# Komputerowe-Projektowanie-Lekow/pmarlo

Measured on AMD Instinct MI355X. Metric: frames/sec featurize->TICA->k-means->T-matrix, 1Mx64 synth; ITS rel-err, higher is better.
Workload: dtype f64; 1 GPU; synthetic 1000000 frames x 64 f32 features per GPU (AR(1) latents), TICA->10, k=500 (10 Lloyd iterations), lag=10, row-normalised T; frames_per_gpu=1000000, features=64, tica_dim=10, k=500, lag=10, kmeans_iters=10, parallelism=shards1

## Files before the change

### include/msmhip.h

```cpp
#ifndef MSMHIP_H
#define MSMHIP_H

#include <stddef.h>
#include <stdint.h>

#ifdef __cplusplus
extern "C" {
#endif

typedef struct msm_ctx msm_ctx;
typedef struct msm_event msm_event;
typedef struct msm_graph msm_graph;

typedef enum {
    MSM_OK = 0,
    MSM_ERR_INVALID = 1,
    MSM_ERR_HIP = 2,
    MSM_ERR_NOMEM = 3,
    MSM_ERR_UNSUPPORTED = 4,
    MSM_ERR_NOCONV = 5
} msm_status;

typedef enum { MSM_F32 = 0, MSM_F64 = 1 } msm_dtype;


msm_status msm_ctx_create(int device, void* hip_stream, msm_ctx** out);
void msm_ctx_destroy(msm_ctx* ctx);
const char* msm_last_error(const msm_ctx* ctx);
msm_status msm_device_info(msm_ctx* ctx, char* arch, size_t arch_len,
                           int* n_cu, size_t* total_mem);
const char* msm_version(void);

msm_status msm_malloc(msm_ctx* ctx, size_t bytes, void** d_out);
msm_status msm_free(msm_ctx* ctx, void* d_ptr);
msm_status msm_memcpy_h2d(msm_ctx* ctx, void* d_dst, const void* h_src, size_t bytes);
msm_status msm_memcpy_d2h(msm_ctx* ctx, void* h_dst, const void* d_src, size_t bytes);
msm_status msm_memcpy_d2d(msm_ctx* ctx, void* d_dst, const void* d_src, size_t bytes);
msm_status msm_memset(msm_ctx* ctx, void* d_dst, int value, size_t bytes);
msm_status msm_sync(msm_ctx* ctx);

msm_status msm_event_create(msm_ctx* ctx, msm_event** out);
void msm_event_destroy(msm_event* ev);
msm_status msm_event_record(msm_ctx* ctx, msm_event* ev);
msm_status msm_event_elapsed_ms(msm_event* start, msm_event* stop, float* h_ms);

msm_status msm_graph_begin(msm_ctx* ctx);
msm_status msm_graph_end(msm_ctx* ctx, msm_graph** out);
msm_status msm_graph_launch(msm_ctx* ctx, msm_graph* g);
void msm_graph_destroy(msm_graph* g);


msm_status msm_featurize_distances(msm_ctx* ctx, const float* d_xyz, int64_t n, int A,
                                   const int32_t* d_pairs, int P, float* d_out, int64_t ld, int col_off);
msm_status msm_featurize_contacts(msm_ctx* ctx, const float* d_xyz, int64_t n, int A,
                                  const int32_t* d_pairs, int P, float rcut, float* d_out,
                                  int64_t ld, int col_off);
msm_status msm_featurize_rg(msm_ctx* ctx, const float* d_xyz, int64_t n, int A, float* d_out,
                            int64_t ld, int col_off);
msm_status msm_featurize_angles(msm_ctx* ctx, const float* d_xyz, int64_t n, int A,
                                const int32_t* d_triplets, int Tn, float* d_out, int64_t ld, int col_off);
msm_status msm_featurize_dihedrals(msm_ctx* ctx, const float* d_xyz, int64_t n, int A,
                                   const int32_t* d_quads, int Q, int mode, float* d_out, int64_t ld,
                                   int col_off);

msm_status msm_featurize_sasa(msm_ctx* ctx, const float* d_xyz, int64_t n, int A, const float* d_radii,
                              const float* d_points, int P, float* d_out);
msm_status msm_hbond_presence(msm_ctx* ctx, const float* d_xyz, int64_t n, int A, const int32_t* d_triplets,
                              int Tn, float dist_cutoff, float angle_cutoff, uint64_t* d_counts);
msm_status msm_dssp(msm_ctx* ctx, const float* d_xyz, int64_t n, int A, const int32_t* d_backbone,
                    const int32_t* d_chain, const uint8_t* d_proline, int R, uint8_t* d_codes);


msm_status msm_count_transitions(msm_ctx* ctx, const int32_t* d_labels, int64_t n,
                                 const int64_t* h_seg_start, const int64_t* h_seg_stop,
                                 int n_seg, int lag, int stride, int k,
                                 int64_t* d_counts, int64_t* d_pairs);

msm_status msm_count_transitions_weighted(msm_ctx* ctx, const int32_t* d_labels,
                                          const double* d_weights, int64_t n,
                                          const int64_t* h_seg_start, const int64_t* h_seg_stop,
                                          int n_seg, int lag, int stride, int k,
                                          double* d_counts, int64_t* d_pairs);

msm_status msm_count_transitions_lagscan(msm_ctx* ctx, const int32_t* d_labels, int64_t n,
                                         const int64_t* h_seg_start, const int64_t* h_seg_stop,
                                         int n_seg, const int32_t* h_lags, int n_lag, int k,
                                         int64_t* d_counts, int64_t* d_pairs);

msm_status msm_state_counts(msm_ctx* ctx, const int32_t* d_labels, int64_t n, int k,
                            int64_t* d_visits);

msm_status msm_run_lengths(msm_ctx* ctx, const int32_t* d_labels, int64_t n, int k, int64_t* d_stats,
                           int32_t* d_run_state, int64_t* d_run_len, int64_t capacity, int64_t* d_n_runs);


msm_status msm_column_moments_partial(msm_ctx* ctx, const void* d_x, msm_dtype dtype, int64_t n, int F,
                                      int64_t ld, const double* d_shift, double* d_sums,
                                      double* d_shift_out);
msm_status msm_moments_finalize(msm_ctx* ctx, const double* d_sums, const double* d_shift, int F,
                                int ddof, double* d_mean, double* d_std, double* d_count);
msm_status msm_column_minmax(msm_ctx* ctx, const void* d_x, msm_dtype dtype, int64_t n, int F, int64_t ld,
                             double* d_min, double* d_max, int64_t* d_counts);
msm_status msm_column_moments(msm_ctx* ctx, const void* d_x, msm_dtype dtype, int64_t n, int F,
                              int64_t ld, int ddof, double* d_mean, double* d_std, double* d_count);

msm_status msm_standardise_params(msm_ctx* ctx, const double* d_sums, const double* d_shift, int F,
                                  double n_rows, int with_std, double* d_mean, double* d_scale,
                                  double* d_inv_scale);

msm_status msm_lagged_moments(msm_ctx* ctx, const void* d_x, msm_dtype dtype, int64_t n, int F, int64_t ld,
                              const int64_t* h_seg_start, const int64_t* h_seg_stop, int n_seg, int lag,
                              const double* d_shift, int assume_finite, double* d_moments);

msm_status msm_lagged_moments_reversible(msm_ctx* ctx, const void* d_x, msm_dtype dtype, int64_t n, int F, int64_t ld,
                                         const int64_t* h_seg_start, const int64_t* h_seg_stop, int n_seg, int lag,
                                         const double* d_shift, int assume_finite, double* d_moments);

msm_status msm_lagged_moments_onesided(msm_ctx* ctx, const void* d_x, msm_dtype dtype, int64_t n, int F,
                                       int64_t ld, const int64_t* h_seg_start, const int64_t* h_seg_stop,
                                       int n_seg, int lag, const double* d_shift, int assume_finite,
                                       double* d_moments);

msm_status msm_onesided_tica_eigenvalues(msm_ctx* ctx, const double* d_moments, int F, double clip,
                                         double* d_eigvals);

msm_status msm_moments_from_lagged(msm_ctx* ctx, const void* d_x, msm_dtype dtype, int64_t n, int F, int64_t ld,
                                   const int64_t* h_seg_start, const int64_t* h_seg_stop, int n_seg, int lag,
                                   const double* d_shift, const double* d_moments, double* d_sums);

msm_status msm_tica_solve(msm_ctx* ctx, const double* d_moments, const double* d_scale, int F,
                          double epsilon, int kinetic_map, double* d_eigvals, double* d_coeffs,
                          double* d_mean, int* d_rank);

msm_status msm_project(msm_ctx* ctx, const void* d_x, msm_dtype dtype, int64_t n, int F, int64_t ld,
                       const double* d_mu, const double* d_inv_sigma, const double* d_mean2,
                       const double* d_w, int d, int64_t ldw, double* d_y, int64_t ldy, double* d_absmax);

msm_status msm_project_finite(msm_ctx* ctx, const void* d_x, msm_dtype dtype, int64_t n, int F, int64_t ld,
                              const double* d_mu, const double* d_inv_sigma, const double* d_mean2,
                              const double* d_w, int d, int64_t ldw, double* d_y, int64_t ldy, double* d_absmax);

msm_status msm_eigh(msm_ctx* ctx, const double* d_a, int n, double* d_w, double* d_v, int* d_sweeps);


msm_status msm_kmeans_assign(msm_ctx* ctx, const void* d_x, msm_dtype dtype, int64_t n, int d,
                             int64_t ld, const double* d_centers, int k,
                             const double* d_mean, const double* d_std,
                             int32_t* d_labels, double* d_mindist);

msm_status msm_kmeans_fit(msm_ctx* ctx, const void* d_x, msm_dtype dtype, int64_t n, int d, int64_t ld,
                          const double* d_mean, const double* d_std, int k, uint64_t seed,
                          int init_centers, int max_iter, double tol2, double* d_centers,
                          double* d_state);
msm_status msm_kmeans_init_plusplus(msm_ctx* ctx, const void* d_x, msm_dtype dtype, int64_t n, int d, int64_t ld,
                                    const double* d_mean, const double* d_std, int k, uint64_t seed, double n_total,
                                    double* d_centers, const double* d_state, int64_t* d_picked);
msm_status msm_kmeans_fit_begin(msm_ctx* ctx, const void* d_x, msm_dtype dtype, int64_t n, int d,
                                int64_t ld, const double* d_mean, const double* d_std, int k,
                                uint64_t seed, int init_centers, double n_total, double tol2,
                                double* d_centers, double* d_state, int absmax_ready);
msm_status msm_kmeans_accumulate(msm_ctx* ctx, const void* d_x, msm_dtype dtype, int64_t n, int d,
                                 int64_t ld, const double* d_centers, int k, const double* d_mean,
                                 const double* d_std, const double* d_state, int64_t* d_sums,
                                 int64_t* d_counts);
msm_status msm_kmeans_update(msm_ctx* ctx, int64_t* d_sums, int64_t* d_counts, int k, int d,
                             double* d_centers, double* d_state, int clear);

msm_status msm_kmeans_image_bytes(int64_t n, int d, size_t* out_bytes);
msm_status msm_kmeans_pack(msm_ctx* ctx, const void* d_x, msm_dtype dtype, int64_t n, int d, int64_t ld,
                           const double* d_mean, const double* d_std, void* d_image);
msm_status msm_kmeans_assign_packed(msm_ctx* ctx, const void* d_x, msm_dtype dtype, int64_t n, int d,
                                    int64_t ld, const double* d_centers, int k, const double* d_mean,
                                    const double* d_std, const void* d_image, int32_t* d_labels,
                                    double* d_mindist);
msm_status msm_kmeans_accumulate_packed(msm_ctx* ctx, const void* d_x, msm_dtype dtype, int64_t n, int d,
                                        int64_t ld, const double* d_centers, int k, const double* d_mean,
                                        const double* d_std, const void* d_image, const double* d_state,
                                        int64_t* d_sums, int64_t* d_counts);
msm_status msm_kmeans_accumulate_delta(msm_ctx* ctx, const void* d_x, msm_dtype dtype, int64_t n, int d,
                                       int64_t ld, const double* d_centers, int k, const double* d_mean,
                                       const double* d_std, const void* d_image, const double* d_state,
                                       int32_t* d_prev_labels, int64_t* d_sums, int64_t* d_counts);
msm_status msm_kmeans_lloyd_pass(msm_ctx* ctx, const void* d_x, msm_dtype dtype, int64_t n, int d, int64_t ld,
                                 double* d_centers, int k, const double* d_mean, const double* d_std,
                                 const void* d_image, double* d_state, int32_t* d_prev_labels, int64_t* d_sums,
                                 int64_t* d_counts);
msm_status msm_kmeans_filter_scanned(msm_ctx* ctx, uint64_t* h_out, int reset);
msm_status msm_mfma_bf16_probe(msm_ctx* ctx, const uint16_t* h_a, const uint16_t* h_b, const float* h_c,
                               float* h_d, int n_tiles);

msm_status msm_sum_f64(msm_ctx* ctx, const double* d_v, int64_t n, double* d_out);


msm_status msm_transition_matrix(msm_ctx* ctx, const void* d_counts, int counts_are_f64, int k, int mode,
                                 double alpha, double epsilon, double* d_T, int32_t* d_active,
                                 int32_t* d_inv_map, int32_t* d_n_active, double* d_rowsum,
                                 double* d_diag_mass);

msm_status msm_embed_full(msm_ctx* ctx, const double* d_T_active, const double* d_pi_active,
                          const int32_t* d_inv_map, int k, double* d_T_full, double* d_pi_full);

size_t msm_spectrum_workspace_bytes(int n_max, int p, int batch);
msm_status msm_spectrum(msm_ctx* ctx, const double* d_T, int64_t t_stride, int ld, const int32_t* d_n,
                        int n_max, int batch, int p, int n_iter, int init, uint64_t seed, int n_watch,
                        void* d_workspace, double* d_ritz, double* d_pi, int64_t pi_stride,
                        double* d_change, int32_t* d_status, int n_its, const double* d_lags,
                        double* d_its_eig, double* d_its_ts, double freeze_tol, double* d_vecs, int n_vecs);
msm_status msm_matrix_power(msm_ctx* ctx, const double* d_T, int64_t t_stride, int ld, const int32_t* d_n, int n_max,
                            int batch, int n_squarings, double* d_scratch, double* d_out);
msm_status msm_spectrum_powered(msm_ctx* ctx, const double* d_T, const double* d_T_power, int64_t t_stride, int ld,
                                const int32_t* d_n, int n_max, int batch, int p, int n_iter, int init, uint64_t seed,
                                int n_watch, void* d_workspace, double* d_ritz, double* d_pi, int64_t pi_stride,
                                double* d_change, int32_t* d_status, int n_its, const double* d_lags,
                                double* d_its_eig, double* d_its_ts, double freeze_tol, double* d_vecs, int n_vecs);

msm_status msm_reversible_mle(msm_ctx* ctx, const double* d_counts, int n, int ld, double maxerr, int maxiter,
                              double* d_T, int ldt, double* d_pi, int* h_iterations, double* h_err);

msm_status msm_sample_transition_matrices(msm_ctx* ctx, const void* d_counts, int counts_are_f64, int k,
                                          const int32_t* d_active, const int32_t* d_n_active, double alpha,
                                          uint64_t seed, int first_sample, int n_samples, double* d_T,
                                          int64_t t_stride, int ld);

msm_status msm_philox4x32(msm_ctx* ctx, uint64_t key, const uint32_t counter[4], uint32_t* d_out);

msm_status msm_gemm_f64(msm_ctx* ctx, int m, int n, int k, const double* d_A, int64_t lda,
                        const double* d_B, int64_t ldb, double* d_C, int64_t ldc);
msm_status msm_ck_test(msm_ctx* ctx, const double* d_T1, int64_t ld1, const double* d_Tk,
                       int64_t tk_stride, int64_t ldk, int n, const int32_t* h_factors, int n_factors,
                       const double* d_rowcounts, int64_t rc_stride, double* d_mse, double* d_noise);

msm_status msm_diff_norms(msm_ctx* ctx, const double* d_P, int64_t ldp, const double* d_Q, int64_t ldq, int n, int m,
                          double* d_out);

msm_status msm_order_statistics(msm_ctx* ctx, const double* d_x, int64_t stride, int64_t n, const int64_t* h_ranks,
                                int n_ranks, double* h_out);

msm_status msm_weighted_stats(msm_ctx* ctx, const double* d_x, int64_t stride, int64_t n,
                              const double* d_w, double* d_out6);
msm_status msm_hist2d(msm_ctx* ctx, const double* d_x, int64_t sx, const double* d_y, int64_t sy,
                      int64_t n, const double* d_w, double w_absmax, const double* d_xedges, int nx,
                      const double* d_yedges, int ny, double* d_hist);
msm_status msm_smooth_sparse_bins(msm_ctx* ctx, const double* d_hist, int nx, int ny,
                                  double min_count, double* d_out, int32_t* d_n_smoothed);
msm_status msm_scale_to_total(msm_ctx* ctx, double* d_v, int n, double total);
msm_status msm_fes_finalize(msm_ctx* ctx, const double* d_hist, int n_cells, double kT,
                            double* d_F, int32_t* d_status);
msm_status msm_kde2d(msm_ctx* ctx, const double* d_x, int64_t sx, const double* d_y, int64_t sy,
                     int64_t n, const double* d_w, double w_scale, const double* d_xcenters, int nx,
                     const double* d_ycenters, int ny, double bw_x, double bw_y, int periodic, double* d_density);

msm_status msm_clip_or_wrap(msm_ctx* ctx, const double* d_x, int64_t stride, int64_t n, double lo, double hi, int mode,
                            double* d_out);

msm_status msm_gather_f64(msm_ctx* ctx, const double* d_table, int m, const int32_t* d_idx, int64_t n, double* d_out);

msm_status msm_solve_f64(msm_ctx* ctx, int n, int nrhs, double* d_A, int64_t lda, double* d_B,
                         int64_t ldb, int32_t* d_info);
msm_status msm_reactive_flux(msm_ctx* ctx, const double* d_T, int64_t ldt, const double* d_pi,
                             const int32_t* d_role, int n, double* d_qplus, double* d_qminus,
                             double* d_gross, double* d_net, double* d_totals, int32_t* d_info);
msm_status msm_lump_macro(msm_ctx* ctx, const double* d_T, int64_t ldt, const double* d_pi,
                          const int32_t* d_macro, int n, int n_macro, double* d_T_macro,
                          double* d_pi_macro);
msm_status msm_macro_mfpt(msm_ctx* ctx, const double* d_T, int64_t ldt, int n, double* d_mfpt,
                          int32_t* d_info);

msm_status msm_silhouette(msm_ctx* ctx, const double* d_x, int64_t n, int d, int64_t ld,
                          const int64_t* h_offsets, int k, double* d_samples, double* d_score);

msm_status msm_grid_cells(msm_ctx* ctx, const void* d_x, msm_dtype dtype, int64_t n, int F, int64_t ld,
                          const double* d_edges, int bins, int32_t* d_flat);
msm_status msm_first_occurrence(msm_ctx* ctx, const int32_t* d_flat, int64_t n, int n_cells,
                                int64_t* d_first);
msm_status msm_relabel(msm_ctx* ctx, const int32_t* d_flat, int64_t n, const int32_t* d_map, int n_cells,
                       int32_t* d_labels);


typedef struct msm_comm msm_comm;
#define MSM_COMM_ID_BYTES 128
msm_status msm_comm_unique_id(void* out_id, size_t bytes);
msm_status msm_comm_init(msm_ctx* ctx, int rank, int world, const void* id, size_t id_bytes, msm_comm** out);
void msm_comm_destroy(msm_comm* comm);
msm_status msm_comm_info(msm_comm* comm, int* rank, int* world, uint64_t* n_collectives);
msm_status msm_allreduce_i64(msm_comm* comm, int64_t* d_buf, size_t count);
msm_status msm_allreduce_i64_from(msm_comm* comm, const int64_t* d_src, int64_t* d_dst, size_t count);
msm_status msm_allreduce_f64(msm_comm* comm, double* d_buf, size_t count);
msm_status msm_allreduce_min_f64(msm_comm* comm, double* d_buf, size_t count);
msm_status msm_allreduce_max_f64(msm_comm* comm, double* d_buf, size_t count);
msm_status msm_broadcast(msm_comm* comm, void* d_buf, size_t bytes, int root);
msm_status msm_rcp_f64(msm_ctx* ctx, const double* d_src, size_t n, double* d_dst);

#ifdef __cplusplus
}
#endif
#endif
```

### pmarlo_amd/_lib.py

```python

from __future__ import annotations

import ctypes as C
from pathlib import Path

__all__ = ["lib", "load", "LIB_PATH", "check", "MsmError", "DECLARED_SYMBOLS"]

LIB_PATH = Path(__file__).resolve().parent / "csrc" / "libmsmhip.so"

MSM_OK, MSM_ERR_INVALID, MSM_ERR_HIP, MSM_ERR_NOMEM, MSM_ERR_UNSUPPORTED, MSM_ERR_NOCONV = range(6)
MSM_F32, MSM_F64 = 0, 1


class MsmError(RuntimeError):
    """A HIP-side failure reported through the C ABI."""


_vp = C.c_void_p
_i32 = C.c_int
_i64 = C.c_int64
_sz = C.c_size_t
_f64 = C.c_double
_pp = C.POINTER(C.c_void_p)

_PROTOTYPES: dict[str, tuple] = {
    "msm_version": (C.c_char_p, []),
    "msm_ctx_create": (_i32, [_i32, _vp, _pp]),
    "msm_ctx_destroy": (None, [_vp]),
    "msm_last_error": (C.c_char_p, [_vp]),
    "msm_device_info": (_i32, [_vp, C.c_char_p, _sz, C.POINTER(_i32), C.POINTER(_sz)]),
    "msm_malloc": (_i32, [_vp, _sz, _pp]),
    "msm_free": (_i32, [_vp, _vp]),
    "msm_memcpy_h2d": (_i32, [_vp, _vp, _vp, _sz]),
    "msm_memcpy_d2h": (_i32, [_vp, _vp, _vp, _sz]),
    "msm_memcpy_d2d": (_i32, [_vp, _vp, _vp, _sz]),
    "msm_memset": (_i32, [_vp, _vp, _i32, _sz]),
    "msm_sync": (_i32, [_vp]),
    "msm_event_create": (_i32, [_vp, _pp]),
    "msm_event_destroy": (None, [_vp]),
    "msm_event_record": (_i32, [_vp, _vp]),
    "msm_event_elapsed_ms": (_i32, [_vp, _vp, C.POINTER(C.c_float)]),
    "msm_graph_begin": (_i32, [_vp]),
    "msm_graph_end": (_i32, [_vp, _pp]),
    "msm_graph_launch": (_i32, [_vp, _vp]),
    "msm_graph_destroy": (None, [_vp]),
    "msm_featurize_distances": (_i32, [_vp, _vp, _i64, _i32, _vp, _i32, _vp, _i64, _i32]),
    "msm_featurize_contacts": (_i32, [_vp, _vp, _i64, _i32, _vp, _i32, C.c_float, _vp, _i64, _i32]),
    "msm_featurize_rg": (_i32, [_vp, _vp, _i64, _i32, _vp, _i64, _i32]),
    "msm_featurize_angles": (_i32, [_vp, _vp, _i64, _i32, _vp, _i32, _vp, _i64, _i32]),
    "msm_featurize_dihedrals": (_i32, [_vp, _vp, _i64, _i32, _vp, _i32, _i32, _vp, _i64, _i32]),
    "msm_featurize_sasa": (_i32, [_vp, _vp, _i64, _i32, _vp, _vp, _i32, _vp]),
    "msm_hbond_presence": (_i32, [_vp, _vp, _i64, _i32, _vp, _i32, C.c_float, C.c_float, _vp]),
    "msm_dssp": (_i32, [_vp, _vp, _i64, _i32, _vp, _vp, _vp, _i32, _vp]),
    "msm_count_transitions": (_i32, [_vp, _vp, _i64, _vp, _vp, _i32, _i32, _i32, _i32, _vp, _vp]),
    "msm_count_transitions_weighted": (
        _i32, [_vp, _vp, _vp, _i64, _vp, _vp, _i32, _i32, _i32, _i32, _vp, _vp]),
    "msm_count_transitions_lagscan": (_i32, [_vp, _vp, _i64, _vp, _vp, _i32, _vp, _i32, _i32, _vp, _vp]),
    "msm_state_counts": (_i32, [_vp, _vp, _i64, _i32, _vp]),
    "msm_column_moments_partial": (_i32, [_vp, _vp, _i32, _i64, _i32, _i64, _vp, _vp, _vp]),
    "msm_moments_finalize": (_i32, [_vp, _vp, _vp, _i32, _i32, _vp, _vp, _vp]),
    "msm_column_moments": (_i32, [_vp, _vp, _i32, _i64, _i32, _i64, _i32, _vp, _vp, _vp]),
    "msm_column_minmax": (_i32, [_vp, _vp, _i32, _i64, _i32, _i64, _vp, _vp, _vp]),
    "msm_standardise_params": (_i32, [_vp, _vp, _vp, _i32, _f64, _i32, _vp, _vp, _vp]),
    "msm_lagged_moments": (_i32, [_vp, _vp, _i32, _i64, _i32, _i64, _vp, _vp, _i32, _i32, _vp, _i32, _vp]),
    "msm_tica_solve": (_i32, [_vp, _vp, _vp, _i32, _f64, _i32, _vp, _vp, _vp, _vp]),
    "msm_lagged_moments_reversible": (_i32, [_vp, _vp, _i32, _i64, _i32, _i64, _vp, _vp, _i32, _i32, _vp, _i32, _vp]),
    "msm_lagged_moments_onesided": (_i32, [_vp, _vp, _i32, _i64, _i32, _i64, _vp, _vp, _i32, _i32, _vp, _i32, _vp]),
    "msm_onesided_tica_eigenvalues": (_i32, [_vp, _vp, _i32, _f64, _vp]),
    "msm_moments_from_lagged": (_i32, [_vp, _vp, _i32, _i64, _i32, _i64, _vp, _vp, _i32, _i32, _vp, _vp, _vp]),
    "msm_project": (_i32, [_vp, _vp, _i32, _i64, _i32, _i64, _vp, _vp, _vp, _vp, _i32, _i64, _vp, _i64, _vp]),
    "msm_project_finite": (_i32, [_vp, _vp, _i32, _i64, _i32, _i64, _vp, _vp, _vp, _vp, _i32, _i64, _vp, _i64, _vp]),
    "msm_eigh": (_i32, [_vp, _vp, _i32, _vp, _vp, _vp]),
    "msm_kmeans_assign": (_i32, [_vp, _vp, _i32, _i64, _i32, _i64, _vp, _i32, _vp, _vp, _vp, _vp]),
    "msm_kmeans_fit": (_i32, [_vp, _vp, _i32, _i64, _i32, _i64, _vp, _vp, _i32, C.c_uint64, _i32, _i32, _f64, _vp, _vp]),
    "msm_kmeans_fit_begin": (
        _i32, [_vp, _vp, _i32, _i64, _i32, _i64, _vp, _vp, _i32, C.c_uint64, _i32, _f64, _f64, _vp, _vp, _i32]),
    "msm_kmeans_accumulate": (_i32, [_vp, _vp, _i32, _i64, _i32, _i64, _vp, _i32, _vp, _vp, _vp, _vp, _vp]),
    "msm_kmeans_update": (_i32, [_vp, _vp, _vp, _i32, _i32, _vp, _vp, _i32]),
    "msm_comm_unique_id": (_i32, [_vp, _sz]),
    "msm_comm_init": (_i32, [_vp, _i32, _i32, _vp, _sz, _pp]),
    "msm_comm_destroy": (None, [_vp]),
    "msm_comm_info": (_i32, [_vp, C.POINTER(_i32), C.POINTER(_i32), C.POINTER(C.c_uint64)]),
    "msm_allreduce_i64": (_i32, [_vp, _vp, _sz]),
    "msm_allreduce_i64_from": (_i32, [_vp, _vp, _vp, _sz]),
    "msm_allreduce_f64": (_i32, [_vp, _vp, _sz]),
    "msm_allreduce_min_f64": (_i32, [_vp, _vp, _sz]),
    "msm_allreduce_max_f64": (_i32, [_vp, _vp, _sz]),
    "msm_broadcast": (_i32, [_vp, _vp, _sz, _i32]),
    "msm_rcp_f64": (_i32, [_vp, _vp, _sz, _vp]),
    "msm_kmeans_image_bytes": (_i32, [_i64, _i32, C.POINTER(_sz)]),
    "msm_kmeans_pack": (_i32, [_vp, _vp, _i32, _i64, _i32, _i64, _vp, _vp, _vp]),
    "msm_kmeans_assign_packed": (_i32, [_vp, _vp, _i32, _i64, _i32, _i64, _vp, _i32, _vp, _vp, _vp, _vp, _vp]),
    "msm_kmeans_accumulate_packed": (_i32, [_vp, _vp, _i32, _i64, _i32, _i64, _vp, _i32, _vp, _vp, _vp, _vp, _vp, _vp]),
    "msm_kmeans_lloyd_pass": (_i32, [_vp, _vp, _i32, _i64, _i32, _i64, _vp, _i32, _vp, _vp, _vp, _vp, _vp, _vp, _vp]),
    "msm_kmeans_accumulate_delta": (_i32, [_vp, _vp, _i32, _i64, _i32, _i64, _vp, _i32, _vp, _vp, _vp, _vp, _vp, _vp,
                                           _vp]),
    "msm_kmeans_filter_scanned": (_i32, [_vp, C.POINTER(C.c_uint64), _i32]),
    "msm_kmeans_init_plusplus": (_i32, [_vp, _vp, _i32, _i64, _i32, _i64, _vp, _vp, _i32, C.c_uint64, _f64, _vp, _vp, _vp]),
    "msm_mfma_bf16_probe": (_i32, [_vp, _vp, _vp, _vp, _vp, _i32]),
    "msm_run_lengths": (_i32, [_vp, _vp, _i64, _i32, _vp, _vp, _vp, _i64, _vp]),
    "msm_sum_f64": (_i32, [_vp, _vp, _i64, _vp]),
    "msm_transition_matrix": (_i32, [_vp, _vp, _i32, _i32, _i32, _f64, _f64, _vp, _vp, _vp, _vp, _vp, _vp]),
    "msm_embed_full": (_i32, [_vp, _vp, _vp, _vp, _i32, _vp, _vp]),
    "msm_spectrum_workspace_bytes": (_sz, [_i32, _i32, _i32]),
    "msm_spectrum": (_i32, [_vp, _vp, _i64, _i32, _vp, _i32, _i32, _i32, _i32, _i32, C.c_uint64, _i32, _vp, _vp, _vp,
                            _i64, _vp, _vp, _i32, _vp, _vp, _vp, _f64, _vp, _i32]),
    "msm_matrix_power": (_i32, [_vp, _vp, _i64, _i32, _vp, _i32, _i32, _i32, _vp, _vp]),
    "msm_spectrum_powered": (_i32, [_vp, _vp, _vp, _i64, _i32, _vp, _i32, _i32, _i32, _i32, _i32, C.c_uint64, _i32, _vp, _vp,
                                    _vp, _i64, _vp, _vp, _i32, _vp, _vp, _vp, _f64, _vp, _i32]),
    "msm_sample_transition_matrices": (_i32, [_vp, _vp, _i32, _i32, _vp, _vp, _f64, C.c_uint64, _i32, _i32, _vp, _i64,
                                              _i32]),
    "msm_reversible_mle": (_i32, [_vp, _vp, _i32, _i32, _f64, _i32, _vp, _i32, _vp, _vp, _vp]),
    "msm_philox4x32": (_i32, [_vp, C.c_uint64, _vp, _vp]),
    "msm_gemm_f64": (_i32, [_vp, _i32, _i32, _i32, _vp, _i64, _vp, _i64, _vp, _i64]),
    "msm_diff_norms": (_i32, [_vp, _vp, _i64, _vp, _i64, _i32, _i32, _vp]),
    "msm_gather_f64": (_i32, [_vp, _vp, _i32, _vp, _i64, _vp]),
    "msm_clip_or_wrap": (_i32, [_vp, _vp, _i64, _i64, _f64, _f64, _i32, _vp]),
    "msm_order_statistics": (_i32, [_vp, _vp, _i64, _i64, _vp, _i32, _vp]),
    "msm_weighted_stats": (_i32, [_vp, _vp, _i64, _i64, _vp, _vp]),
    "msm_hist2d": (_i32, [_vp, _vp, _i64, _vp, _i64, _i64, _vp, _f64, _vp, _i32, _vp, _i32, _vp]),
    "msm_smooth_sparse_bins": (_i32, [_vp, _vp, _i32, _i32, _f64, _vp, _vp]),
    "msm_scale_to_total": (_i32, [_vp, _vp, _i32, _f64]),
    "msm_fes_finalize": (_i32, [_vp, _vp, _i32, _f64, _vp, _vp]),
    "msm_kde2d": (_i32, [_vp, _vp, _i64, _vp, _i64, _i64, _vp, _f64, _vp, _i32, _vp, _i32, _f64, _f64, _i32, _vp]),
    "msm_solve_f64": (_i32, [_vp, _i32, _i32, _vp, _i64, _vp, _i64, _vp]),
    "msm_reactive_flux": (_i32, [_vp, _vp, _i64, _vp, _vp, _i32, _vp, _vp, _vp, _vp, _vp, _vp]),
    "msm_lump_macro": (_i32, [_vp, _vp, _i64, _vp, _vp, _i32, _i32, _vp, _vp]),
    "msm_macro_mfpt": (_i32, [_vp, _vp, _i64, _i32, _vp, _vp]),
    "msm_silhouette": (_i32, [_vp, _vp, _i64, _i32, _i64, _vp, _i32, _vp, _vp]),
    "msm_grid_cells": (_i32, [_vp, _vp, _i32, _i64, _i32, _i64, _vp, _i32, _vp]),
    "msm_first_occurrence": (_i32, [_vp, _vp, _i64, _i32, _vp]),
    "msm_relabel": (_i32, [_vp, _vp, _i64, _vp, _i32, _vp]),
    "msm_ck_test": (_i32, [_vp, _vp, _i64, _vp, _i64, _i64, _i32, _vp, _i32, _vp, _i64, _vp, _vp]),
}

DECLARED_SYMBOLS = tuple(_PROTOTYPES)

_lib = None


def load() -> C.CDLL:
    global _lib
    if _lib is not None:
        return _lib
    if not LIB_PATH.exists():
        raise ImportError(
            f"{LIB_PATH} is missing: build it with `python -m pmarlo_amd.csrc.build` "
            "(hipcc, gfx950).  pmarlo_amd has no CPU fallback."
        )
    handle = C.CDLL(str(LIB_PATH))
    for name, (res, args) in _PROTOTYPES.items():
        fn = getattr(handle, name)
        fn.restype = res
        fn.argtypes = args
    _lib = handle
    return handle


class _LazyLib:
    def __getattr__(self, name):
        return getattr(load(), name)


lib = _LazyLib()

_EXC = {
    MSM_ERR_INVALID: ValueError,
    MSM_ERR_HIP: MsmError,
    MSM_ERR_NOMEM: MemoryError,
    MSM_ERR_UNSUPPORTED: NotImplementedError,
    MSM_ERR_NOCONV: MsmError,
}


def check(status: int, ctx_handle=None) -> None:
    if status == MSM_OK:
        return
    msg = ""
    if ctx_handle:
        raw = load().msm_last_error(ctx_handle)
        msg = raw.decode("utf-8", "replace") if raw else ""
    exc = _EXC.get(status, MsmError)
    raise exc(msg or f"libmsmhip call failed with status {status}")
```

### pmarlo_amd/csrc/kmeans.hip

```cpp
#include "common.h"

#include <algorithm>
#include <cstdlib>

namespace {

constexpr int kThreads = 256;

template <typename T>
__device__ __forceinline__ double load_as_f64(const T* p) { return (double)(*p); }

struct FitState {
    double scale;
    double inv_scale;
    double absmax;
    double shift2;
    double tol2;
    double done;
    double n_iter;
    double inertia;
};

__device__ __forceinline__ long long to_fixed(double v, double scale) { return __double2ll_rn(v * scale); }

// ... 448 lines not shown
            const int kt16 = (kt + 15) & ~15;
            if (!single_tile) {
                __syncthreads();
                stage_tile(k0, kt, kt16);
                KSTAMP(5);
            }
            const int n_tiles = kt16 / 16;
            for (int jt = 0; jt < n_tiles; jt += 2) {
                const int jb = min(jt + 1, n_tiles - 1);
                v4f64 acca[NF], accb[NF];
#pragma unroll
                for (int u = 0; u < NF; ++u) { acca[u] = (v4f64){0.0, 0.0, 0.0, 0.0}; accb[u] = acca[u]; }
                if constexpr (KS <= 4) {
#pragma unroll
                    for (int s = 0; s < KS; ++s) {
                        const double afa = cs[jt * TS + s * 64 + lane];
#pragma unroll
                        for (int u = 0; u < NF; ++u)
                            acca[u] = __builtin_amdgcn_mfma_f64_16x16x4f64(afa, zb[u][s], acca[u], 0, 0, 0);
                    }
#pragma unroll
                    for (int s = 0; s < KS; ++s) {
                        const double afb = cs[jb * TS + s * 64 + lane];
#pragma unroll
                        for (int u = 0; u < NF; ++u)
                            accb[u] = __builtin_amdgcn_mfma_f64_16x16x4f64(afb, zb[u][s], accb[u], 0, 0, 0);
                    }
                } else {
                    double fa = cs[jt * TS + lane], fb = cs[jb * TS + lane];
#pragma unroll
                    for (int s = 0; s < KS; ++s) {
                        double na = fa, nb = fb;
                        if (s + 1 < KS) {
                            na = cs[jt * TS + (s + 1) * 64 + lane];
                            nb = cs[jb * TS + (s + 1) * 64 + lane];
                        }
#pragma unroll
                        for (int u = 0; u < NF; ++u) {
                            acca[u] = __builtin_amdgcn_mfma_f64_16x16x4f64(fa, zb[u][s], acca[u], 0, 0, 0);
                            accb[u] = __builtin_amdgcn_mfma_f64_16x16x4f64(fb, zb[u][s], accb[u], 0, 0, 0);
                        }
                        fa = na;
                        fb = nb;
                    }
                }
                if constexpr (!fold) {
#pragma unroll
                    for (int r = 0; r < 4; ++r) {
                        const double ha = chalf[jt * 16 + g + 4 * r], hb = chalf[jb * 16 + g + 4 * r];
#pragma unroll
                        for (int u = 0; u < NF; ++u) { acca[u][r] -= ha; accb[u][r] -= hb; }
                    }
                }
                __builtin_amdgcn_sched_barrier(0);
                if constexpr (KS > 4) asm volatile("s_nop 15\n\ts_nop 3" ::: "memory");
                double ma[NF], mb[NF];
#pragma unroll
                for (int u = 0; u < NF; ++u) ma[u] = max_f64(max_f64(acca[u][0], acca[u][1]), max_f64(acca[u][2], acca[u][3]));
                asm volatile("s_nop 7" ::: "memory");
                __builtin_amdgcn_sched_barrier(0);
#pragma unroll
                for (int u = 0; u < NF; ++u) {
                    mb[u] = max_f64(max_f64(accb[u][0], accb[u][1]), max_f64(accb[u][2], accb[u][3]));
                    const double m = max_f64(ma[u], mb[u]);
                    const bool better = m > best[u];
                    best[u] = better ? m : best[u];
                    const int code = kGlobalRecovery ? (((k0 >> 4) + jt) << 1) | (jb == jt ? 1 : 0) : jt;
                    bpair[u] = better ? code : bpair[u];
                }
            }
            KSTAMP(2);
            if constexpr (!kGlobalRecovery) {
#pragma unroll
            for (int u = 0; u < NF; ++u) {
                double M = best[u];
                M = fmax(M, __shfl_xor(M, 16, 64));
                M = fmax(M, __shfl_xor(M, 32, 64));
                const unsigned long long tied = __ballot(best[u] == M) >> j16;
                unsigned pending = (unsigned)(tied & 1) | (unsigned)((tied >> 15) & 2) | (unsigned)((tied >> 30) & 4) |
                                   (unsigned)((tied >> 45) & 8);
                int found = 0x7fffffff;
                while (__any(pending != 0)) {
                    const int gs = pending ? __builtin_ctz(pending) : 0;
                    const int pj = __shfl(bpair[u], j16 + 16 * gs, 64);
                    const int ta = pj, tb = min(pj + 1, n_tiles - 1);
                    const int crow = gs + 4 * g;
                    const double* ca = cs + ta * TS + crow;
                    const double* cb = cs + tb * TS + crow;
                    double da = 0.0, db = 0.0;
#pragma unroll
                    for (int s = 0; s < KS; ++s)
#pragma unroll
                        for (int gp = 0; gp < 4; ++gp) {
                            const double zv = __shfl(zb[u][s], j16 + 16 * gp, 64);
                            da = fma(ca[s * 64 + gp * 16], zv, da);
                            db = fma(cb[s * 64 + gp * 16], zv, db);
                        }
                    if constexpr (!fold) {
                        da -= chalf[ta * 16 + crow];
                        db -= chalf[tb * 16 + crow];
                    }
                    int cand = 0x7fffffff;
                    if (pending) {
                        if (db == M) cand = k0 + tb * 16 + crow;
                        if (da == M) cand = k0 + ta * 16 + crow;
                    }
                    cand = min(cand, __shfl_xor(cand, 16, 64));
                    cand = min(cand, __shfl_xor(cand, 32, 64));
                    found = min(found, cand);
                    pending &= pending - 1;
                }
                if (found < k) { bm[u] = M; bidx[u] = found; }
            }
            }
        }
        if constexpr (kGlobalRecovery) {
#pragma unroll
            for (int u = 0; u < NF; ++u) {
                double M = best[u];
                M = fmax(M, __shfl_xor(M, 16, 64));
                M = fmax(M, __shfl_xor(M, 32, 64));
                const unsigned long long tied = __ballot(best[u] == M) >> j16;
                unsigned pending = (unsigned)(tied & 1) | (unsigned)((tied >> 15) & 2) | (unsigned)((tied >> 30) & 4) |
                                   (unsigned)((tied >> 45) & 8);
                int found = 0x7fffffff;
                const T* row = x + (fok[u] ? fidx[u] : 0) * ld;
                while (__any(pending != 0)) {
                    const int gs = pending ? __builtin_ctz(pending) : 0;
                    const int pj = __shfl(bpair[u], j16 + 16 * gs, 64);
                    const int ta = pj >> 1, tb = ta + ((pj & 1) ? 0 : 1);
                    const int crow = gs + 4 * g;
                    const int ia = ta * 16 + crow, ib = tb * 16 + crow;
                    const double* ca = centers + (size_t)min(ia, k - 1) * d;
                    const double* cb = centers + (size_t)min(ib, k - 1) * d;
                    double da = 0.0, db = 0.0;
                    int f = 0;
                    for (; f + 8 <= d; f += 8) {
                        double v[8], va[8], vb[8];
#pragma unroll
                        for (int q = 0; q < 8; ++q) {
                            v[q] = load_as_f64(row + f + q);
                            va[q] = ca[f + q];
                            vb[q] = cb[f + q];
                        }
#pragma unroll
                        for (int q = 0; q < 8; ++q) {
                            double z = v[q];
                            if (mean) z = (z - mean[f + q]) / stdv[f + q];
                            da = fma(va[q], z, da);
                            db = fma(vb[q], z, db);
                        }
                    }
                    for (; f < d; ++f) {
                        double v = load_as_f64(row + f);
                        if (mean) v = (v - mean[f]) / stdv[f];
                        da = fma(ca[f], v, da);
                        db = fma(cb[f], v, db);
                    }
                    da -= chalf_g[min(ia, k - 1)];
                    db -= chalf_g[min(ib, k - 1)];
                    int cand = 0x7fffffff;
                    if (pending) {
                        if (ib < k && db == M) cand = ib;
                        if (ia < k && da == M) cand = ia;
                    }
                    cand = min(cand, __shfl_xor(cand, 16, 64));
                    cand = min(cand, __shfl_xor(cand, 32, 64));
                    found = min(found, cand);
                    pending &= pending - 1;
                }
                if (found < k) { bm[u] = M; bidx[u] = found; }
            }
        }
        KSTAMP(3);
#pragma unroll
        for (int u = 0; u < NF; ++u) {
            if (!fok[u]) continue;
            if constexpr (ACCUM) {
                const int old = labels ? labels[fidx[u]] : -1;
                if (!labels || old != bidx[u]) {
                    unsigned long long* base = lds_acc ? lsum : sums;
                    unsigned long long* srow = base + (size_t)bidx[u] * d;
#pragma unroll
                    for (int s = 0; s < KS; ++s) {
                        const int f = 4 * s + g;
                        if (f < d) {
                            const unsigned long long fx = (unsigned long long)to_fixed(zb[u][s], scale);
                            atomicAdd(&srow[f], fx);
                            if (old >= 0) atomicAdd(&base[(size_t)old * d + f], 0ull - fx);
                        }
                    }
                    if (g == 0) {
                        atomicAdd((lds_acc ? lcnt : counts) + bidx[u], 1ull);
                        if (old >= 0) atomicAdd((lds_acc ? lcnt : counts) + old, ~0ull);
                        if (labels) labels[fidx[u]] = bidx[u];
                    }
                }
            } else {
                if (g == 0) {
                    labels[fidx[u]] = bidx[u];
                    if (mindist) {
                        const T* row = x + fidx[u] * ld;
                        double zsq = 0.0;
                        for (int f = 0; f < d; ++f) {
                            double v = load_as_f64(row + f);
                            if (mean) v = (v - mean[f]) / stdv[f];
                            zsq = fma(v, v, zsq);
                        }
                        const double md = -2.0 * bm[u] + zsq;
                        mindist[fidx[u]] = md > 0.0 ? md : 0.0;
                    }
                }
            }
        }
        KSTAMP(4);
    }
    KSTAMP(7);
    if constexpr (ACCUM) {
        if (lds_acc) {
            __syncthreads();
            KSTAMP(5);
            for (int i = tid; i < k * d; i += kMT)
                if (lsum[i]) atomicAdd(&sums[i], lsum[i]);
            for (int i = tid; i < k; i += kMT)
                if (lcnt[i]) atomicAdd(&counts[i], lcnt[i]);
        }
    }
    KSTAMP(6);
    KSTAMP_FLUSH
}

template <typename T, int KS, bool ACCUM>
msm_status launch_mfma(msm_ctx* ctx, const T* x, int64_t n, int d, int64_t ld, const double* centers, int k,
                       const double* mean, const double* stdv, int32_t* labels, double* mindist, const FitState* st,
                       unsigned long long* sums, unsigned long long* counts) {
    constexpr int NF = KS <= 16 ? 2 : 1;
    constexpr int kMT = KS <= 4 ? kMTNarrow : kMTWide;
    constexpr int TS = KS * 64 + 1;
    const size_t acc_bytes = ACCUM ? (size_t)k * (d + 1) * sizeof(unsigned long long) : 0;
    const int lds_acc = ACCUM && acc_bytes <= 64 * 1024;
    const size_t tile_budget = 150 * 1024 - (lds_acc ? acc_bytes : 0);
    int tile_k = (int)(tile_budget / ((TS + 16) * sizeof(double))) * 16;
    const int k16 = (k + 15) & ~15;
    if (tile_k > k16) tile_k = k16;
    if (tile_k < 16) tile_k = 16;
    if (tile_k < k16 && tile_k >= 32) tile_k &= ~31;
    const size_t lds = (size_t)(tile_k / 16) * (TS + 16) * sizeof(double) + (lds_acc ? acc_bytes : 0);
    const int64_t n_units = (n + 16 * NF - 1) / (16 * NF);
    const int waves = kMT / 64;
    const int grid = (int)std::min<int64_t>((n_units + waves - 1) / waves, (int64_t)ctx->n_cu);
    const bool multi = k > tile_k;
    const bool foldm = (d & 3) != 0;
    auto kern = multi ? (foldm ? kmeans_mfma_kernel<T, KS, NF, kMT, ACCUM, true, true>
                               : kmeans_mfma_kernel<T, KS, NF, kMT, ACCUM, false, true>)
                      : (foldm ? kmeans_mfma_kernel<T, KS, NF, kMT, ACCUM, true, false>
                               : kmeans_mfma_kernel<T, KS, NF, kMT, ACCUM, false, false>);
    double* chalf_g = nullptr;
    double* tile_img = nullptr;
    if (multi) {
        const size_t n_tiles_all = (size_t)k16 / 16;
        const size_t img_doubles = (n_tiles_all * TS + 1) & ~(size_t)1;
        msm_status rs = msm_reserve_aux(ctx, (img_doubles + k16) * sizeof(double));
        if (rs != MSM_OK) return rs;
        tile_img = (double*)ctx->aux;
        chalf_g = tile_img + img_doubles;
        if (foldm)
            hipLaunchKernelGGL((pack_tiles_kernel<KS, true>), dim3((unsigned)n_tiles_all), dim3(64), 0, ctx->stream, centers,
                               k, d, tile_img, chalf_g);
        else
            hipLaunchKernelGGL((pack_tiles_kernel<KS, false>), dim3((unsigned)n_tiles_all), dim3(64), 0, ctx->stream, centers,
                               k, d, tile_img, chalf_g);
    } else if (KS > 8) {
        msm_status rs = msm_reserve_aux(ctx, (size_t)k * sizeof(double));
        if (rs != MSM_OK) return rs;
        chalf_g = (double*)ctx->aux;
        hipLaunchKernelGGL(chalf_kernel, dim3((k + 255) / 256), dim3(256), 0, ctx->stream, centers, k, d, chalf_g);
    }
    if (lds > 48 * 1024)
        MSM_HIP(ctx, hipFuncSetAttribute((const void*)kern, hipFuncAttributeMaxDynamicSharedMemorySize, (int)lds));
    hipLaunchKernelGGL(kern, dim3(grid), dim3(kMT), lds, ctx->stream, x, n, d, ld, centers, k, mean, stdv, tile_k,
                       labels, mindist, st, sums, counts, lds_acc, (const double*)chalf_g, (const double*)tile_img);
    MSM_CHECK_LAUNCH(ctx);
    return MSM_OK;
}

__global__ void mfma_bf16_probe_kernel(const uint16_t* __restrict__ A, const uint16_t* __restrict__ B,
                                       const float* __restrict__ C, float* __restrict__ D) {
    const int l = threadIdx.x, i = l & 15, q = l >> 4;
    A += (size_t)blockIdx.x * 512;
    B += (size_t)blockIdx.x * 512;
    C += (size_t)blockIdx.x * 256;
    D += (size_t)blockIdx.x * 256;
    v8bf a, b;
    for (int j = 0; j < 8; ++j) {
        a[j] = __builtin_bit_cast(__bf16, A[i * 32 + 8 * q + j]);
        b[j] = __builtin_bit_cast(__bf16, B[(8 * q + j) * 16 + i]);
    }
    v4f32 c;
    for (int r = 0; r < 4; ++r) c[r] = C[(4 * q + r) * 16 + i];
    c = __builtin_amdgcn_mfma_f32_16x16x32_bf16(a, b, c, 0, 0, 0);
    for (int r = 0; r < 4; ++r) D[(4 * q + r) * 16 + i] = c[r];
}

bool filter_enabled() {
    static const bool on = [] {
        const char* e = getenv("MSM_KMEANS_FILTER");
        return !(e && e[0] == '0');
    }();
    return on;
}

size_t filter_image_bytes(int64_t n, int d) { return (size_t)((n + 63) & ~(int64_t)63) * 16 * filter_rowq(filter_nm(d)); }

template <typename T>
msm_status launch_pack(msm_ctx* ctx, const T* x, int64_t n, int d, int64_t ld, const double* mean, const double* stdv,
                       uint4* image) {
    const unsigned grid = (unsigned)((n + 255) / 256);
    const int dense = ld == d && ((uintptr_t)x & 15) == 0;
#define MSM_PACK_CASE(D)                                                                                              \
    case D:                                                                                                           \
        hipLaunchKernelGGL((kmeans_pack_kernel<T, D>), dim3(grid), dim3(256), 0, ctx->stream, x, n, ld, mean, stdv, image, \
                           dense);                                                                                    \
        break
    switch (d) {
        MSM_PACK_CASE(1); MSM_PACK_CASE(2); MSM_PACK_CASE(3); MSM_PACK_CASE(4); MSM_PACK_CASE(5);
        MSM_PACK_CASE(6); MSM_PACK_CASE(7); MSM_PACK_CASE(8); MSM_PACK_CASE(9); MSM_PACK_CASE(10);
        default: return msm_fail(ctx, MSM_ERR_UNSUPPORTED, "k-means frame images need d <= %d (got %d)", kFilterMaxD, d);
    }
#undef MSM_PACK_CASE
    MSM_CHECK_LAUNCH(ctx);
    return MSM_OK;
}

msm_status filter_stats_buffer(msm_ctx* ctx, unsigned long long** out) {
    static_assert(sizeof(unsigned long long) == 8, "");
    if (!ctx->km_stats) {
        if (ctx->capturing) { *out = nullptr; return MSM_OK; }
        MSM_HIP(ctx, hipMalloc(&ctx->km_stats, 16));
        MSM_HIP(ctx, hipMemsetAsync(ctx->km_stats, 0, 16, ctx->stream));
    }
    *out = (unsigned long long*)ctx->km_stats;
    return MSM_OK;
}

template <typename T, int NM, bool ACCUM>
msm_status launch_filter_nm(msm_ctx* ctx, const T* x, int64_t n, int d, int64_t ld, const double* centers, int k,
                            const double* mean, const double* stdv, const uint4* image, int32_t* labels, double* mindist,
                            const FitState* st, unsigned long long* sums, unsigned long long* counts, double* upd_centers) {
    constexpr int NF = 4;
    const size_t lds = filter_lds_bytes(k, d, ACCUM);
    msm_status rs;
    const int64_t n_units = (n + 16 * NF - 1) / (16 * NF);
    constexpr int kWaves = filter_waves(NM);
    const int grid = (int)std::min<int64_t>((n_units + kWaves - 1) / kWaves, (int64_t)ctx->n_cu);
    unsigned long long* stats = nullptr;
    rs = filter_stats_buffer(ctx, &stats);
    if (rs != MSM_OK) return rs;
    auto kern = mean ? kmeans_filter_kernel<T, NM, NF, ACCUM, true> : kmeans_filter_kernel<T, NM, NF, ACCUM, false>;
    if (lds > 48 * 1024)
        MSM_HIP(ctx, hipFuncSetAttribute((const void*)kern, hipFuncAttributeMaxDynamicSharedMemorySize, (int)lds));
    hipLaunchKernelGGL(kern, dim3(grid), dim3(64 * kWaves), lds, ctx->stream, x, n, d, ld, k, mean, stdv, image, centers,
                       labels, mindist, st, sums, counts, stats, stats ? upd_centers : nullptr,
                       stats ? (unsigned int*)(stats + 1) : nullptr);
    MSM_CHECK_LAUNCH(ctx);
    return MSM_OK;
}

template <typename T, bool ACCUM>
msm_status launch_filter(msm_ctx* ctx, const T* x, int64_t n, int d, int64_t ld, const double* centers, int k,
                         const double* mean, const double* stdv, const uint4* image, int32_t* labels, double* mindist,
                         const FitState* st, unsigned long long* sums, unsigned long long* counts, double* upd_centers) {
    if (filter_nm(d) == 1)
        return launch_filter_nm<T, 1, ACCUM>(ctx, x, n, d, ld, centers, k, mean, stdv, image, labels, mindist, st, sums,
                                             counts, upd_centers);
    return launch_filter_nm<T, 2, ACCUM>(ctx, x, n, d, ld, centers, k, mean, stdv, image, labels, mindist, st, sums, counts,
                                         upd_centers);
}

bool filter_fits(int k, int d, bool accum) { return filter_enabled() && d <= kFilterMaxD && filter_lds_bytes(k, d, accum) != 0; }

template <typename T, bool ACCUM>
msm_status dispatch_mfma(msm_ctx* ctx, const T* x, int64_t n, int d, int64_t ld, const double* centers, int k,
                         const double* mean, const double* stdv, int32_t* labels, double* mindist, const FitState* st,
                         unsigned long long* sums, unsigned long long* counts, const void* image = nullptr,
                         double* upd_centers = nullptr, bool* folded = nullptr) {
    if (folded) *folded = false;
    if (filter_fits(k, d, ACCUM)) {
        if (!image) {
            msm_status rs = msm_reserve_km_image(ctx, filter_image_bytes(n, d));
            if (rs != MSM_OK) return rs;
            rs = launch_pack<T>(ctx, x, n, d, ld, mean, stdv, (uint4*)ctx->km_image);
            if (rs != MSM_OK) return rs;
            image = ctx->km_image;
        }
        if (upd_centers && !(ACCUM && (int64_t)k * d <= kUpdateWide && (ctx->km_stats || !ctx->capturing))) upd_centers = nullptr;
        if (folded) *folded = upd_centers != nullptr;
        return launch_filter<T, ACCUM>(ctx, x, n, d, ld, centers, k, mean, stdv, (const uint4*)image, labels, mindist, st,
                                       sums, counts, upd_centers);
    }
#define MSM_MFMA_CASE(KSV) \
    if (d <= 4 * KSV)      \
        return launch_mfma<T, KSV, ACCUM>(ctx, x, n, d, ld, centers, k, mean, stdv, labels, mindist, st, sums, counts)
    MSM_MFMA_CASE(1);
    MSM_MFMA_CASE(2);
    MSM_MFMA_CASE(3);
    MSM_MFMA_CASE(4);
    MSM_MFMA_CASE(6);
    MSM_MFMA_CASE(8);
    MSM_MFMA_CASE(12);
    MSM_MFMA_CASE(16);
    MSM_MFMA_CASE(24);
    MSM_MFMA_CASE(32);
    MSM_MFMA_CASE(48);
    MSM_MFMA_CASE(64);
#undef MSM_MFMA_CASE
    return msm_fail(ctx, MSM_ERR_UNSUPPORTED, "k-means: d=%d > 256 not supported", d);
}

}

extern "C" {

static msm_status kmeans_assign_impl(msm_ctx* ctx, const void* d_x, msm_dtype dtype, int64_t n, int d, int64_t ld,
                                     const double* d_centers, int k, const double* d_mean, const double* d_std,
                                     const void* d_image, int32_t* d_labels, double* d_mindist) {
    if (!ctx) return MSM_ERR_INVALID;
    MSM_REQUIRE(ctx, n >= 0 && d >= 1 && k >= 1, "msm_kmeans_assign: need n >= 0, d >= 1, k >= 1");
    MSM_REQUIRE(ctx, ld >= d, "msm_kmeans_assign: ld (%lld) < d (%d)", (long long)ld, d);
    MSM_REQUIRE(ctx, (d_mean == nullptr) == (d_std == nullptr),
                "msm_kmeans_assign: mean and std must both be given or both be NULL");
    MSM_REQUIRE(ctx, dtype == MSM_F32 || dtype == MSM_F64, "msm_kmeans_assign: bad dtype");
    if (n == 0) return MSM_OK;
    MSM_REQUIRE(ctx, d_x && d_centers && d_labels, "msm_kmeans_assign: NULL pointer");
    if (dtype == MSM_F32)
        return dispatch_mfma<float, false>(ctx, (const float*)d_x, n, d, ld, d_centers, k, d_mean, d_std, d_labels,
                                           d_mindist, nullptr, nullptr, nullptr, d_image);
    return dispatch_mfma<double, false>(ctx, (const double*)d_x, n, d, ld, d_centers, k, d_mean, d_std, d_labels,
                                        d_mindist, nullptr, nullptr, nullptr, d_image);
}

msm_status msm_kmeans_assign(msm_ctx* ctx, const void* d_x, msm_dtype dtype, int64_t n, int d, int64_t ld,
                             const double* d_centers, int k, const double* d_mean, const double* d_std,
                             int32_t* d_labels, double* d_mindist) {
    return kmeans_assign_impl(ctx, d_x, dtype, n, d, ld, d_centers, k, d_mean, d_std, nullptr, d_labels, d_mindist);
}

msm_status msm_kmeans_assign_packed(msm_ctx* ctx, const void* d_x, msm_dtype dtype, int64_t n, int d, int64_t ld,
                                    const double* d_centers, int k, const double* d_mean, const double* d_std,
                                    const void* d_image, int32_t* d_labels, double* d_mindist) {
    return kmeans_assign_impl(ctx, d_x, dtype, n, d, ld, d_centers, k, d_mean, d_std, d_image, d_labels, d_mindist);
}

msm_status msm_kmeans_image_bytes(int64_t n, int d, size_t* out_bytes) {
    if (!out_bytes || n < 0 || d < 1) return MSM_ERR_INVALID;
    *out_bytes = d <= kFilterMaxD ? filter_image_bytes(n, d) : 0;
    return MSM_OK;
}

msm_status msm_kmeans_pack(msm_ctx* ctx, const void* d_x, msm_dtype dtype, int64_t n, int d, int64_t ld,
                           const double* d_mean, const double* d_std, void* d_image) {
    if (!ctx) return MSM_ERR_INVALID;
    MSM_REQUIRE(ctx, n >= 0 && d >= 1 && d <= kFilterMaxD && ld >= d, "msm_kmeans_pack: need 1 <= d <= %d, ld >= d",
                kFilterMaxD);
    MSM_REQUIRE(ctx, (d_mean == nullptr) == (d_std == nullptr), "msm_kmeans_pack: mean/std must come together");
    MSM_REQUIRE(ctx, dtype == MSM_F32 || dtype == MSM_F64, "msm_kmeans_pack: bad dtype");
    if (n == 0) return MSM_OK;
    MSM_REQUIRE(ctx, d_x && d_image, "msm_kmeans_pack: NULL pointer");
    MSM_REQUIRE(ctx, ((uintptr_t)d_image & 15) == 0, "msm_kmeans_pack: the image must be 16-byte aligned");
    if (dtype == MSM_F32) return launch_pack<float>(ctx, (const float*)d_x, n, d, ld, d_mean, d_std, (uint4*)d_image);
    return launch_pack<double>(ctx, (const double*)d_x, n, d, ld, d_mean, d_std, (uint4*)d_image);
}

msm_status msm_kmeans_filter_scanned(msm_ctx* ctx, uint64_t* h_out, int reset) {
    if (!ctx || !h_out) return MSM_ERR_INVALID;
    *h_out = 0;
    if (!ctx->km_stats) return MSM_OK;
    MSM_HIP(ctx, hipStreamSynchronize(ctx->stream));
    MSM_HIP(ctx, hipMemcpy(h_out, ctx->km_stats, 8, hipMemcpyDeviceToHost));
    if (reset) MSM_HIP(ctx, hipMemset(ctx->km_stats, 0, 8));
    return MSM_OK;
}

msm_status msm_mfma_bf16_probe(msm_ctx* ctx, const uint16_t* h_a, const uint16_t* h_b, const float* h_c, float* h_d,
                               int n_tiles) {
    if (!ctx) return MSM_ERR_INVALID;
    MSM_REQUIRE(ctx, n_tiles >= 1 && h_a && h_b && h_c && h_d, "msm_mfma_bf16_probe: bad arguments");
    const size_t na = (size_t)n_tiles * 512 * sizeof(uint16_t), nc = (size_t)n_tiles * 256 * sizeof(float);
    msm_status rs = msm_reserve_scratch(ctx, 2 * na + 2 * nc);
    if (rs != MSM_OK) return rs;
    unsigned char* base = (unsigned char*)ctx->scratch;
    uint16_t* d_a = (uint16_t*)base;
    uint16_t* d_b = (uint16_t*)(base + na);
    float* d_c = (float*)(base + 2 * na);
    float* d_d = (float*)(base + 2 * na + nc);
    MSM_HIP(ctx, hipMemcpyAsync(d_a, h_a, na, hipMemcpyHostToDevice, ctx->stream));
    MSM_HIP(ctx, hipMemcpyAsync(d_b, h_b, na, hipMemcpyHostToDevice, ctx->stream));
    MSM_HIP(ctx, hipMemcpyAsync(d_c, h_c, nc, hipMemcpyHostToDevice, ctx->stream));
    hipLaunchKernelGGL(mfma_bf16_probe_kernel, dim3((unsigned)n_tiles), dim3(64), 0, ctx->stream, d_a, d_b, d_c, d_d);
    MSM_CHECK_LAUNCH(ctx);
    MSM_HIP(ctx, hipMemcpyAsync(h_d, d_d, nc, hipMemcpyDeviceToHost, ctx->stream));
    MSM_HIP(ctx, hipStreamSynchronize(ctx->stream));
    return MSM_OK;
}

msm_status msm_kmeans_fit_begin(msm_ctx* ctx, const void* d_x, msm_dtype dtype, int64_t n, int d, int64_t ld,
                                const double* d_mean, const double* d_std, int k, uint64_t seed, int init_centers,
                                double n_total, double tol2, double* d_centers, double* d_state, int absmax_ready) {
    if (!ctx) return MSM_ERR_INVALID;
    MSM_REQUIRE(ctx, n >= 1 && d >= 1 && d <= 256 && k >= 1 && ld >= d, "msm_kmeans_fit_begin: bad shape");
    MSM_REQUIRE(ctx, !absmax_ready || !d_mean, "msm_kmeans_fit_begin: a precomputed max |x| excludes whitening");
    MSM_REQUIRE(ctx, !init_centers || n >= k, "msm_kmeans_fit_begin: fewer frames (%lld) than centres (%d)",
                (long long)n, k);
    MSM_REQUIRE(ctx, (d_mean == nullptr) == (d_std == nullptr), "msm_kmeans_fit_begin: mean/std must come together");
    MSM_REQUIRE(ctx, d_x && d_centers && d_state, "msm_kmeans_fit_begin: NULL pointer");
    MSM_REQUIRE(ctx, dtype == MSM_F32 || dtype == MSM_F64, "msm_kmeans_fit_begin: bad dtype");
    MSM_REQUIRE(ctx, n_total >= (double)n && tol2 >= 0.0, "msm_kmeans_fit_begin: bad n_total / tol2");
    unsigned long long* bits = (unsigned long long*)(d_state + 2);
    if (!absmax_ready) {
        MSM_HIP(ctx, hipMemsetAsync(bits, 0, sizeof(unsigned long long), ctx->stream));
        const int grid = (int)std::min<int64_t>((n * d + kThreads * 8 - 1) / (kThreads * 8), (int64_t)ctx->n_cu * 8);
        if (dtype == MSM_F32)
            hipLaunchKernelGGL(absmax_kernel<float>, dim3(grid), dim3(kThreads), 0, ctx->stream, (const float*)d_x, n, d,
                               ld, d_mean, d_std, bits);
        else
            hipLaunchKernelGGL(absmax_kernel<double>, dim3(grid), dim3(kThreads), 0, ctx->stream, (const double*)d_x, n,
                               d, ld, d_mean, d_std, bits);
        MSM_CHECK_LAUNCH(ctx);
    }
    if (!init_centers) {
        hipLaunchKernelGGL(fit_scale_kernel, dim3(1), dim3(64), 0, ctx->stream, bits, n_total, tol2, (FitState*)d_state);
        MSM_CHECK_LAUNCH(ctx);
    }
    if (init_centers) {
        const int g2 = msm_ceil_div((int64_t)k * d, 256);
        if (dtype == MSM_F32)
            hipLaunchKernelGGL(init_centers_kernel<float>, dim3(g2), dim3(256), 0, ctx->stream, (const float*)d_x, n, d,
                               ld, d_mean, d_std, k, (unsigned long long)seed, d_centers, bits, n_total, tol2,
                               (FitState*)d_state);
        else
            hipLaunchKernelGGL(init_centers_kernel<double>, dim3(g2), dim3(256), 0, ctx->stream, (const double*)d_x, n,
                               d, ld, d_mean, d_std, k, (unsigned long long)seed, d_centers, bits, n_total, tol2,
                               (FitState*)d_state);
        MSM_CHECK_LAUNCH(ctx);
    }
    return MSM_OK;
}

static msm_status kmeans_accumulate_impl(msm_ctx* ctx, const void* d_x, msm_dtype dtype, int64_t n, int d, int64_t ld,
                                         const double* d_centers, int k, const double* d_mean, const double* d_std,
                                         const void* d_image, const double* d_state, int64_t* d_sums, int64_t* d_counts,
                                         int32_t* d_prev_labels = nullptr, double* d_update_centers = nullptr,
                                         bool* folded = nullptr) {
    if (folded) *folded = false;
    if (!ctx) return MSM_ERR_INVALID;
    MSM_REQUIRE(ctx, n >= 0 && d >= 1 && k >= 1 && ld >= d, "msm_kmeans_accumulate: bad shape");
    MSM_REQUIRE(ctx, (d_mean == nullptr) == (d_std == nullptr), "msm_kmeans_accumulate: mean/std must come together");
    MSM_REQUIRE(ctx, dtype == MSM_F32 || dtype == MSM_F64, "msm_kmeans_accumulate: bad dtype");
    if (n == 0) return MSM_OK;
    MSM_REQUIRE(ctx, d_x && d_centers && d_state && d_sums && d_counts, "msm_kmeans_accumulate: NULL pointer");
    if (dtype == MSM_F32)
        return dispatch_mfma<float, true>(ctx, (const float*)d_x, n, d, ld, d_centers, k, d_mean, d_std, d_prev_labels,
                                          nullptr, (const FitState*)d_state, (unsigned long long*)d_sums,
                                          (unsigned long long*)d_counts, d_image, d_update_centers, folded);
    return dispatch_mfma<double, true>(ctx, (const double*)d_x, n, d, ld, d_centers, k, d_mean, d_std, d_prev_labels,
                                       nullptr, (const FitState*)d_state, (unsigned long long*)d_sums,
                                       (unsigned long long*)d_counts, d_image, d_update_centers, folded);
}

msm_status msm_kmeans_lloyd_pass(msm_ctx* ctx, const void* d_x, msm_dtype dtype, int64_t n, int d, int64_t ld,
                                 double* d_centers, int k, const double* d_mean, const double* d_std, const void* d_image,
                                 double* d_state, int32_t* d_prev_labels, int64_t* d_sums, int64_t* d_counts) {
    bool folded = false;
    msm_status rs = kmeans_accumulate_impl(ctx, d_x, dtype, n, d, ld, d_centers, k, d_mean, d_std, d_image, d_state, d_sums,
                                           d_counts, d_prev_labels, d_centers, &folded);
    if (rs != MSM_OK || folded) return rs;
    return msm_kmeans_update(ctx, d_sums, d_counts, k, d, d_centers, d_state, 0);
}

msm_status msm_kmeans_accumulate_delta(msm_ctx* ctx, const void* d_x, msm_dtype dtype, int64_t n, int d, int64_t ld,
                                       const double* d_centers, int k, const double* d_mean, const double* d_std,
                                       const void* d_image, const double* d_state, int32_t* d_prev_labels,
                                       int64_t* d_sums, int64_t* d_counts) {
    if (!ctx) return MSM_ERR_INVALID;
    MSM_REQUIRE(ctx, d_prev_labels || n == 0, "msm_kmeans_accumulate_delta: NULL label buffer");
    return kmeans_accumulate_impl(ctx, d_x, dtype, n, d, ld, d_centers, k, d_mean, d_std, d_image, d_state, d_sums,
                                  d_counts, d_prev_labels);
}

msm_status msm_kmeans_accumulate(msm_ctx* ctx, const void* d_x, msm_dtype dtype, int64_t n, int d, int64_t ld,
                                 const double* d_centers, int k, const double* d_mean, const double* d_std,
                                 const double* d_state, int64_t* d_sums, int64_t* d_counts) {
    return kmeans_accumulate_impl(ctx, d_x, dtype, n, d, ld, d_centers, k, d_mean, d_std, nullptr, d_state, d_sums,
                                  d_counts);
}

msm_status msm_kmeans_accumulate_packed(msm_ctx* ctx, const void* d_x, msm_dtype dtype, int64_t n, int d, int64_t ld,
                                        const double* d_centers, int k, const double* d_mean, const double* d_std,
                                        const void* d_image, const double* d_state, int64_t* d_sums,
                                        int64_t* d_counts) {
    return kmeans_accumulate_impl(ctx, d_x, dtype, n, d, ld, d_centers, k, d_mean, d_std, d_image, d_state, d_sums,
                                  d_counts);
}

msm_status msm_kmeans_update(msm_ctx* ctx, int64_t* d_sums, int64_t* d_counts, int k, int d, double* d_centers,
                             double* d_state, int clear) {
    if (!ctx) return MSM_ERR_INVALID;
    MSM_REQUIRE(ctx, k >= 1 && d >= 1, "msm_kmeans_update: bad shape");
    MSM_REQUIRE(ctx, d_sums && d_counts && d_centers && d_state, "msm_kmeans_update: NULL pointer");
    if ((int64_t)k * d > kUpdateWide) {
        const int nb = std::min(k, ctx->n_cu);
        const int cpb = (k + nb - 1) / nb;
        const int nblocks = (k + cpb - 1) / cpb;
        msm_status rs = msm_reserve_aux(ctx, (size_t)nblocks * sizeof(double));
        if (rs != MSM_OK) return rs;
        hipLaunchKernelGGL(kmeans_update_wide_kernel, dim3(nblocks), dim3(1024), 0, ctx->stream, (unsigned long long*)d_sums,
                           (unsigned long long*)d_counts, k, d, cpb, d_centers, (const FitState*)d_state, clear,
                           (double*)ctx->aux);
        MSM_CHECK_LAUNCH(ctx);
        hipLaunchKernelGGL(kmeans_update_finish_kernel, dim3(1), dim3(64), 0, ctx->stream, (const double*)ctx->aux, nblocks,
                           (FitState*)d_state);
        MSM_CHECK_LAUNCH(ctx);
        return MSM_OK;
    }
    hipLaunchKernelGGL(kmeans_update_kernel, dim3(1), dim3(1024), 0, ctx->stream, (unsigned long long*)d_sums,
                       (unsigned long long*)d_counts, k, d, d_centers, (FitState*)d_state, clear);
    MSM_CHECK_LAUNCH(ctx);
    return MSM_OK;
}

msm_status msm_kmeans_fit(msm_ctx* ctx, const void* d_x, msm_dtype dtype, int64_t n, int d, int64_t ld,
                          const double* d_mean, const double* d_std, int k, uint64_t seed, int init_centers,
                          int max_iter, double tol2, double* d_centers, double* d_state) {
    if (!ctx) return MSM_ERR_INVALID;
    MSM_REQUIRE(ctx, max_iter >= 0, "msm_kmeans_fit: max_iter must be >= 0");
    msm_status rs = msm_kmeans_fit_begin(ctx, d_x, dtype, n, d, ld, d_mean, d_std, k, seed, init_centers, (double)n,
                                         tol2, d_centers, d_state, 0);
    if (rs != MSM_OK) return rs;
    const size_t acc_bytes = ((size_t)k * (d + 1) * sizeof(unsigned long long) + 15) & ~(size_t)15;
    rs = msm_reserve_scratch(ctx, acc_bytes + (size_t)n * sizeof(int32_t));
    if (rs != MSM_OK) return rs;
    int64_t* sums = (int64_t*)ctx->scratch;
    int64_t* counts = sums + (size_t)k * d;
    int32_t* prev = (int32_t*)((char*)ctx->scratch + acc_bytes);
    MSM_HIP(ctx, hipMemsetAsync(sums, 0, acc_bytes, ctx->stream));
    MSM_HIP(ctx, hipMemsetAsync(prev, 0xFF, (size_t)n * sizeof(int32_t), ctx->stream));
    const void* image = nullptr;
    if (max_iter > 0 && filter_fits(k, d, true)) {
        rs = msm_reserve_km_image(ctx, filter_image_bytes(n, d));
        if (rs != MSM_OK) return rs;
        rs = msm_kmeans_pack(ctx, d_x, dtype, n, d, ld, d_mean, d_std, ctx->km_image);
        if (rs != MSM_OK) return rs;
        image = ctx->km_image;
    }
    for (int it = 0; it < max_iter; ++it) {
        rs = msm_kmeans_lloyd_pass(ctx, d_x, dtype, n, d, ld, d_centers, k, d_mean, d_std, image, d_state, prev, sums, counts);
        if (rs != MSM_OK) return rs;
    }
    return MSM_OK;
}

msm_status msm_sum_f64(msm_ctx* ctx, const double* d_v, int64_t n, double* d_out) {
    if (!ctx) return MSM_ERR_INVALID;
    MSM_REQUIRE(ctx, n >= 0 && d_out && (d_v || n == 0), "msm_sum_f64: bad arguments");
    const int nb = (int)std::min<int64_t>(256, std::max<int64_t>(1, n / 4096));
    msm_status rs = msm_reserve_scratch(ctx, (size_t)nb * sizeof(double));
    if (rs != MSM_OK) return rs;
    hipLaunchKernelGGL(sum_partial_kernel, dim3(nb), dim3(1024), 0, ctx->stream, d_v, n, (double*)ctx->scratch);
    MSM_CHECK_LAUNCH(ctx);
    hipLaunchKernelGGL(sum_final_kernel, dim3(1), dim3(64), 0, ctx->stream, (const double*)ctx->scratch, nb, d_out);
    MSM_CHECK_LAUNCH(ctx);
    return MSM_OK;
}

}
```

### pmarlo_amd/csrc/kmeans_filter.h

```cpp
#pragma once

typedef __bf16 v8bf __attribute__((ext_vector_type(8)));
typedef float v4f32 __attribute__((ext_vector_type(4)));

#ifdef MSM_KMF_WAVES
__host__ __device__ constexpr int filter_waves(int) { return MSM_KMF_WAVES; }
#else
__host__ __device__ constexpr int filter_waves(int nm) { return nm == 1 ? 16 : 12; }
#endif
constexpr int kFilterMaxD = 10;
constexpr double kFilterTiny = 1e-14, kFilterHi = 1e18;
constexpr float kPickEps = 20.0f * 5.9604644775390625e-08f;
constexpr float kPickFloor = 1e-30f;
constexpr float kUp20 = 1.0f + 9.5367431640625e-07f;

__host__ __device__ constexpr int filter_nm(int d) { return 6 * d + 4 <= 32 ? 1 : 2; }
__host__ __device__ constexpr int filter_rowq(int nm) { return nm == 1 ? 4 : 5; }
__host__ __device__ constexpr double filter_kappa(int nm) { return (nm == 1 ? 44.0 : 80.0) * 5.9604644775390625e-08; }

__device__ __forceinline__ unsigned bf16_rn(float f) {
    unsigned u = __float_as_uint(f);
    u += 0x7FFFu + ((u >> 16) & 1u);
    return u >> 16;
}
__device__ __forceinline__ float bf16_f32(unsigned h) { return __uint_as_float(h << 16); }
__device__ __forceinline__ unsigned bf16_up(float f) {
    unsigned h = bf16_rn(f);
    if (bf16_f32(h) < f) ++h;
    return h;
}
__device__ __forceinline__ void bf16_split3(double v, unsigned (&out)[3]) {
    float r = (float)v;
#pragma unroll
    for (int t = 0; t < 3; ++t) {
        out[t] = bf16_rn(r);
        r -= bf16_f32(out[t]);
    }
}
__device__ __forceinline__ int filter_part_c(int t) { return t == 1 || t == 3 ? 1 : (t == 4 ? 2 : 0); }
__device__ __forceinline__ int filter_part_x(int t) { return t == 2 || t == 3 ? 1 : (t == 5 ? 2 : 0); }

template <int NM>
__host__ __device__ constexpr int filter_slot(int t, int f, int d) {
    if (NM == 1) return t * d + f;
    constexpr int lo8[6] = {0, 8, 24, 32, 16, 40};
    constexpr int hi2[6] = {48, 50, 54, 56, 52, 58};
    return f < 8 ? lo8[t] + f : hi2[t] + (f - 8);
}
template <int NM>
__host__ __device__ constexpr int filter_slot_h(int d) { return NM == 1 ? 6 * d : 60; }
template <int NM>
__host__ __device__ constexpr int filter_slot_norm() { return 32 * NM - 1; }
template <int NM>
__device__ __forceinline__ int filter_piece(int q, int m) {
    if (NM == 1) return q;
    return m == 0 ? (q < 3 ? 0 : 1) : q + 1;
}

__device__ __forceinline__ float max3_f32(float a, float b, float c) { return __builtin_fmaxf(__builtin_fmaxf(a, b), c); }
__device__ __forceinline__ float med3_f32(float a, float b, float c) { return __builtin_amdgcn_fmed3f(a, b, c); }
__device__ __forceinline__ float hw_max_f32(float a, float b) {
    float r;
    asm("v_max_f32 %0, %1, %2" : "=v"(r) : "v"(a), "v"(b));
    return r;
}

template <typename T, int D>
__global__ __launch_bounds__(256) void kmeans_pack_kernel(const T* __restrict__ x, int64_t n, int64_t ld,
                                                         const double* __restrict__ mean,
                                                         const double* __restrict__ stdv, uint4* __restrict__ image,
                                                         int dense) {
    constexpr int NM = filter_nm(D);
    constexpr int RQ = filter_rowq(NM);
    constexpr int kOutStride = 5;
    constexpr int kInBytes = 256 * D * (int)sizeof(T);
    constexpr int kOutBytes = 256 * kOutStride * 16;
    __shared__ __attribute__((aligned(16))) unsigned char stage[kOutBytes > kInBytes ? kOutBytes : kInBytes];
    const int64_t t0 = (int64_t)blockIdx.x * 256;
    const int64_t t = t0 + threadIdx.x;
    const int rows = (int)(n - t0 < 256 ? n - t0 : 256);
    const int64_t n_pad = (n + 63) & ~(int64_t)63;
    const int rows_out = (int)(n_pad - t0 < 256 ? n_pad - t0 : 256);
    double v[D];
    if (dense) {
        const unsigned char* src = reinterpret_cast<const unsigned char*>(x + t0 * D);
        const int nbytes = rows * D * (int)sizeof(T);
        for (int b = threadIdx.x * 16; b + 16 <= nbytes; b += 256 * 16)
            *reinterpret_cast<uint4*>(stage + b) = *reinterpret_cast<const uint4*>(src + b);
        if (threadIdx.x < (nbytes & 15) / (int)sizeof(T)) {
            const int e = (nbytes & ~15) / (int)sizeof(T) + threadIdx.x;
            reinterpret_cast<T*>(stage)[e] = reinterpret_cast<const T*>(src)[e];
        }
        __syncthreads();
        const T* row = reinterpret_cast<const T*>(stage) + threadIdx.x * D;
#pragma unroll
        for (int f = 0; f < D; ++f) v[f] = threadIdx.x < rows ? (double)row[f] : 0.0;
        __syncthreads();
    } else {
        const T* row = x + (t < n ? t : n - 1) * ld;
#pragma unroll
        for (int f = 0; f < D; ++f) v[f] = load_as_f64(row + f);
    }
    unsigned part[D][3];
    double q = 0.0, tiny = 0.0;
    bool ok = t < n;
#pragma unroll
    for (int f = 0; f < D; ++f) {
        if (mean) v[f] = (v[f] - mean[f]) / stdv[f];
        ok = ok && fabs(v[f]) <= kFilterHi;
    }
#pragma unroll
    for (int f = 0; f < D; ++f) {
        const double a = fabs(v[f]);
        const bool keep = ok && a >= kFilterTiny;
        if (ok && !keep) tiny += a;
        const double w = keep ? v[f] : 0.0;
        q = fma(w, w, q);
        bf16_split3(w, part[f]);
    }
    const unsigned xn = ok ? bf16_up((float)((sqrt(q) + tiny / filter_kappa(NM)) * (1.0 + 9.5367431640625e-07))) : 0x7F80u;
    unsigned slots[8 * RQ];
#pragma unroll
    for (int s = 0; s < 8 * RQ; ++s) slots[s] = 0;
    if constexpr (NM == 1) {
#pragma unroll
        for (int tt = 0; tt < 6; ++tt)
#pragma unroll
            for (int f = 0; f < D; ++f) slots[tt * D + f] = part[f][tt == 2 || tt == 3 ? 1 : (tt == 5 ? 2 : 0)];
        slots[6 * D] = slots[6 * D + 1] = slots[6 * D + 2] = 0x3F80u;
        slots[31] = xn;
    } else {
#pragma unroll
        for (int f = 0; f < D; ++f) {
            if (f < 8) {
                slots[f] = part[f][0];
                slots[8 + f] = part[f][1];
                slots[16 + f] = part[f][2];
            } else {
                const int g = f - 8;
                slots[24 + g] = slots[26 + g] = slots[28 + g] = part[f][0];
                slots[30 + g] = part[f][1];
                slots[32 + g] = part[f][1];
                slots[34 + g] = part[f][2];
            }
        }
        slots[36] = slots[37] = slots[38] = 0x3F80u;
        slots[39] = xn;
    }
    uint4* mine = reinterpret_cast<uint4*>(stage) + threadIdx.x * kOutStride;
#pragma unroll
    for (int c = 0; c < RQ; ++c)
        mine[c] = make_uint4(slots[8 * c + 0] | (slots[8 * c + 1] << 16), slots[8 * c + 2] | (slots[8 * c + 3] << 16),
                             slots[8 * c + 4] | (slots[8 * c + 5] << 16), slots[8 * c + 6] | (slots[8 * c + 7] << 16));
    __syncthreads();
    uint4* dst = image + t0 * RQ;
    for (int c = threadIdx.x; c < rows_out * RQ; c += 256)
        dst[c] = reinterpret_cast<const uint4*>(stage)[(c / RQ) * kOutStride + (c % RQ)];
}

template <int NM>
struct FilterShape {
    static constexpr int DP = NM == 1 ? 4 : 10;
    static constexpr int RF = NM == 1 ? 8 : 12;
    static constexpr int kTileBytes = NM * 1024 + 16 * RF * 4 + 16 * 8;
};

constexpr int kStageRegs = (16 * kFilterMaxD + 63) / 64;
__device__ __forceinline__ int stage_row(int i, int d) { return (int)(((float)i + 0.5f) * (1.0f / (float)d)); }
template <int DP>
__device__ __forceinline__ void filter_stage_fetch(int tile, int lane, const double* __restrict__ centers, int k, int d,
                                                   double (&c)[kStageRegs], double (&rc)[DP]) {
#pragma unroll
    for (int u = 0; u < kStageRegs; ++u) {
        const int i = lane + 64 * u;
        const int r = stage_row(i, d), j = tile * 16 + r;
        c[u] = (i < 16 * d && j < k) ? centers[(size_t)tile * 16 * d + i] : 0.0;
    }
    const int jr = tile * 16 + lane;
#pragma unroll
    for (int f = 0; f < DP; ++f) rc[f] = (lane < 16 && jr < k && f < d) ? centers[(size_t)jr * d + f] : 0.0;
}
template <int NM>
__device__ __forceinline__ void filter_stage_build(int tile, int lane, unsigned short* simg, const double (&c)[kStageRegs],
                                                   const double (&rc)[FilterShape<NM>::DP], int k, int d,
                                                   float* __restrict__ tab, double* __restrict__ hs, int* __restrict__ any_bad) {
    using S = FilterShape<NM>;
    constexpr double kappa = filter_kappa(NM);
    for (int i = lane; i < NM * 64 * 4; i += 64) reinterpret_cast<unsigned*>(simg)[i] = 0u;
    for (int i = lane; i < 16 * S::RF; i += 64) tab[(size_t)tile * 16 * S::RF + i] = 0.0f;
    __builtin_amdgcn_fence(__ATOMIC_ACQ_REL, "wavefront");
    auto slot_addr = [&](int i, int sl) {
        const int m = sl >> 5, qq = (sl & 31) >> 3, e = sl & 7;
        return ((m * 64) + qq * 16 + i) * 8 + e;
    };
#pragma unroll
    for (int u = 0; u < kStageRegs; ++u) {
        const int i = lane + 64 * u;
        const int r = stage_row(i, d), f = i - r * d, j = tile * 16 + r;
        if (i < 16 * d && j < k) {
            tab[(size_t)j * S::RF + f] = (float)c[u];
            if (fabs(c[u]) >= kFilterTiny) {
                unsigned cp[3];
                bf16_split3(c[u], cp);
#pragma unroll
                for (int t = 0; t < 6; ++t) simg[slot_addr(r, filter_slot<NM>(t, f, d))] = (unsigned short)cp[filter_part_c(t)];
            }
        }
    }
    __builtin_amdgcn_fence(__ATOMIC_ACQ_REL, "wavefront");
    int bad_row = 0;
    if (lane < 16) {
        const int j = tile * 16 + lane;
        float* row = tab + (size_t)j * S::RF;
        double h = __builtin_inf();
        if (j < k) {
            double a = 0.0, akeep = 0.0, tiny = 0.0;
            bool ok = true;
#pragma unroll
            for (int f = 0; f < S::DP; ++f) {
                const double cf = rc[f];
                a = fma(cf, cf, a);
                const double ac = fabs(cf);
                ok = ok && ac <= kFilterHi;
                if (ac >= kFilterTiny) akeep = fma(cf, cf, akeep);
                else tiny += ac;
            }
            h = 0.5 * a;
            if (!ok) bad_row = 1;
            unsigned hsp[3];
            bf16_split3(-(h - kappa * h), hsp);
            const int sh = filter_slot_h<NM>(d);
            simg[slot_addr(lane, sh)] = (unsigned short)hsp[0];
            simg[slot_addr(lane, sh + 1)] = (unsigned short)hsp[1];
            simg[slot_addr(lane, sh + 2)] = (unsigned short)hsp[2];
            simg[slot_addr(lane, filter_slot_norm<NM>())] =
                (unsigned short)bf16_up((float)((kappa * sqrt(akeep) + tiny) * (1.0 + 9.5367431640625e-07)));
            row[S::DP] = (float)h;
            row[S::DP + 1] = (float)(sqrt(a) * (1.0 + 9.5367431640625e-07));
        } else {
            simg[slot_addr(lane, filter_slot_h<NM>(d))] = 0xFF7F;
            row[S::DP] = 3.0e38f;
            row[S::DP + 1] = -3.0e38f;
        }
        hs[j] = h;
    }
    const bool bad = __any(bad_row != 0);
    if (bad && lane == 0) atomicOr(any_bad, 1);
}

typedef unsigned v2u32 __attribute__((ext_vector_type(2)));
template <typename Op>
__device__ __forceinline__ unsigned xrow_reduce_u32(unsigned x, Op op) {
    v2u32 r = __builtin_amdgcn_permlane16_swap(x, x, false, false);
    x = op(r[0], r[1]);
    r = __builtin_amdgcn_permlane32_swap(x, x, false, false);
    return op(r[0], r[1]);
}
__device__ __forceinline__ float xrow_max_f32(float x) {
    return __uint_as_float(xrow_reduce_u32(__float_as_uint(x), [](unsigned a, unsigned b) {
        return __float_as_uint(hw_max_f32(__uint_as_float(a), __uint_as_float(b)));
    }));
}
__device__ __forceinline__ int xrow_min_i32(int x) {
    return (int)xrow_reduce_u32((unsigned)x, [](unsigned a, unsigned b) { return (unsigned)min((int)a, (int)b); });
}
template <typename Op>
__device__ __forceinline__ unsigned row_reduce_u32(unsigned x, Op op) {
    x = op(x, (unsigned)__builtin_amdgcn_update_dpp(0, (int)x, 0xB1, 0xF, 0xF, false));
    x = op(x, (unsigned)__builtin_amdgcn_update_dpp(0, (int)x, 0x4E, 0xF, 0xF, false));
    x = op(x, (unsigned)__builtin_amdgcn_update_dpp(0, (int)x, 0x141, 0xF, 0xF, false));
    x = op(x, (unsigned)__builtin_amdgcn_update_dpp(0, (int)x, 0x140, 0xF, 0xF, false));
    return x;
}
__device__ __forceinline__ float wave_max_f32(float x) {
    const unsigned r = row_reduce_u32(__float_as_uint(x), [](unsigned a, unsigned b) {
        return __float_as_uint(hw_max_f32(__uint_as_float(a), __uint_as_float(b)));
    });
    return xrow_max_f32(__uint_as_float(r));
}
__device__ __forceinline__ int wave_min_i32(int x) {
    return xrow_min_i32((int)row_reduce_u32((unsigned)x, [](unsigned a, unsigned b) { return (unsigned)min((int)a, (int)b); }));
}
__device__ __forceinline__ double wave_max_f64(double x) {
    auto mx = [](double a, double b) {
        double r;
        asm volatile("v_max_f64 %0, %1, %2" : "=v"(r) : "v"(a), "v"(b));
        return r;
    };
    auto dpp = [&](double v, auto ctrl) {
        const long long bits = __double_as_longlong(v);
        const int lo = __builtin_amdgcn_update_dpp(0, (int)bits, decltype(ctrl)::value, 0xF, 0xF, false);
        const int hi = __builtin_amdgcn_update_dpp(0, (int)(bits >> 32), decltype(ctrl)::value, 0xF, 0xF, false);
        return __longlong_as_double((long long)(((unsigned long long)(unsigned)hi << 32) | (unsigned)lo));
    };
    x = mx(x, dpp(x, std::integral_constant<int, 0xB1>{}));
    x = mx(x, dpp(x, std::integral_constant<int, 0x4E>{}));
    x = mx(x, dpp(x, std::integral_constant<int, 0x141>{}));
    x = mx(x, dpp(x, std::integral_constant<int, 0x140>{}));
#pragma unroll
    for (int step = 0; step < 2; ++step) {
        const unsigned lo = (unsigned)__double_as_longlong(x), hi = (unsigned)(__double_as_longlong(x) >> 32);
        v2u32 rl, rh;
        if (step == 0) {
            rl = __builtin_amdgcn_permlane16_swap(lo, lo, false, false);
            rh = __builtin_amdgcn_permlane16_swap(hi, hi, false, false);
        } else {
            rl = __builtin_amdgcn_permlane32_swap(lo, lo, false, false);
            rh = __builtin_amdgcn_permlane32_swap(hi, hi, false, false);
        }
        x = mx(__longlong_as_double((long long)(((unsigned long long)rh[0] << 32) | rl[0])),
               __longlong_as_double((long long)(((unsigned long long)rh[1] << 32) | rl[1])));
    }
    return x;
}

template <typename T, int DP, bool WHITEN>
__device__ __forceinline__ void filter_load_frame(const T* __restrict__ x, int64_t ld, int d, bool vec_rows,
                                                  const double* __restrict__ mean, const double* __restrict__ stdv,
                                                  int64_t t, double (&z)[DP]) {
    const T* row = x + t * ld;
    if (vec_rows) {
        const double2* r2 = reinterpret_cast<const double2*>(row);
#pragma unroll
        for (int f2 = 0; f2 < DP / 2; ++f2) {
            const double2 v = r2[f2];
            z[2 * f2] = v.x;
            z[2 * f2 + 1] = v.y;
        }
    } else {
#pragma unroll
        for (int f = 0; f < DP; ++f) {
            const double v = load_as_f64(row + (f < d ? f : d - 1));
            z[f] = f < d ? v : 0.0;
        }
    }
    if constexpr (WHITEN) {
#pragma unroll
        for (int f = 0; f < DP; ++f) {
            const int fc = f < d ? f : d - 1;
            const double w = (z[f] - mean[fc]) / stdv[fc];
            z[f] = f < d ? w : 0.0;
        }
    }
}

template <int MT>
__device__ __forceinline__ void filter_close_iteration(const unsigned long long* sums, const unsigned long long* counts, int k,
                                                       int d, double* centers, FitState* st) {
    __shared__ double red[16];
    const int tid = threadIdx.x;
    const double inv_scale = st->inv_scale;
    for (int v0 = 0; v0 < 1024; v0 += MT) {
        const int v = v0 + tid;
        if (v < 1024) {
            double acc = 0.0;
            constexpr int CH = 4;
            for (int i0 = v; i0 < k * d; i0 += 1024 * CH) {
                long long cnt[CH], sm[CH];
                double old[CH];
#pragma unroll
                for (int c = 0; c < CH; ++c) {
                    const int i = i0 + c * 1024;
                    cnt[c] = 0;
                    if (i < k * d) {
                        cnt[c] = (long long)__hip_atomic_load(&counts[i / d], __ATOMIC_RELAXED, __HIP_MEMORY_SCOPE_AGENT);
                        sm[c] = (long long)__hip_atomic_load(&sums[i], __ATOMIC_RELAXED, __HIP_MEMORY_SCOPE_AGENT);
                        old[c] = centers[i];
                    }
                }
#pragma unroll
                for (int c = 0; c < CH; ++c)
                    if (cnt[c] > 0) {
                        const double c_new = (double)sm[c] * inv_scale / (double)cnt[c];
                        const double dlt = c_new - old[c];
                        acc = fma(dlt, dlt, acc);
                        centers[i0 + c * 1024] = c_new;
                    }
            }
            for (int off = 32; off > 0; off >>= 1) acc += __shfl_down(acc, off, 64);
            if ((v & 63) == 0) red[v >> 6] = acc;
        }
    }
    __syncthreads();
    if (tid == 0) {
        double t = 0.0;
        for (int i = 0; i < 16; ++i) t += red[i];
        st->shift2 = t;
        st->n_iter += 1.0;
        if (t <= st->tol2) st->done = 1.0;
    }
}

template <typename T, int NM, int NF, bool ACCUM, bool WHITEN>
__global__ __launch_bounds__(64 * filter_waves(NM)) void kmeans_filter_kernel(
    const T* __restrict__ x, int64_t n, int d, int64_t ld, int k, const double* __restrict__ mean,
    const double* __restrict__ stdv, const uint4* __restrict__ image, const double* __restrict__ centers,
    int32_t* __restrict__ labels,
    double* __restrict__ mindist, const FitState* __restrict__ st, unsigned long long* __restrict__ sums,
    unsigned long long* __restrict__ counts, unsigned long long* __restrict__ n_scanned, double* upd_centers,
    unsigned int* __restrict__ ticket) {
    using S = FilterShape<NM>;
    constexpr int kFilterWaves = filter_waves(NM);
    constexpr int kMT = 64 * kFilterWaves, DP = S::DP, RF = S::RF, RQ = filter_rowq(NM);
    static_assert(NF == 4, "one frame group per lane quarter: a unit is 64 frames, one per lane in the candidate pick");
    extern __shared__ __attribute__((aligned(16))) unsigned char smem_raw[];
    if constexpr (ACCUM) {
        if (st->done != 0.0) return;
    }
    const int k16 = (k + 15) & ~15;
    const int n_tiles = ((k16 / 16) + 1) & ~1;
    uint4* img = reinterpret_cast<uint4*>(smem_raw);
    float* tab = reinterpret_cast<float*>(img + (size_t)n_tiles * NM * 64);
    double* hs = reinterpret_cast<double*>(tab + (size_t)n_tiles * 16 * RF);
    unsigned long long* lsum = reinterpret_cast<unsigned long long*>(hs + (size_t)n_tiles * 16);
    unsigned long long* lcnt = lsum + (ACCUM ? (size_t)k * d : 0);
    __shared__ int unit_ctr;
    __shared__ int any_bad;
    const int tid = threadIdx.x, lane = tid & 63, wave = __builtin_amdgcn_readfirstlane(tid >> 6);
    const int j16 = lane & 15, q = lane >> 4;
    const double scale = ACCUM ? st->scale : 0.0;
    if (tid == 0) {
        unit_ctr = kFilterWaves;
        any_bad = 0;
    }
    KSTAMP_INIT
    if constexpr (ACCUM) {
        for (int i = tid; i < k * (d + 1); i += kMT) lsum[i] = 0ull;
    }
    __syncthreads();
    constexpr int kUnit = 16 * NF;
    const int64_t n_units = (n + kUnit - 1) / kUnit;
    const int64_t units_per_block = (n_units + gridDim.x - 1) / gridDim.x;
    const int64_t u_begin = (int64_t)blockIdx.x * units_per_block;
    const int64_t u_end = min(n_units, u_begin + units_per_block);
    int voff[NM];
#pragma unroll
    for (int m = 0; m < NM; ++m) voff[m] = j16 * RQ + filter_piece<NM>(q, m);

    int64_t unit = u_begin + wave;
    v8bf b[NF][NM];
    auto load_images = [&](int64_t un) {
        const uint4* ub = image + un * (kUnit * RQ);
#pragma unroll
        for (int u = 0; u < NF; ++u)
#pragma unroll
            for (int m = 0; m < NM; ++m) b[u][m] = __builtin_bit_cast(v8bf, ub[voff[m] + u * 16 * RQ]);
    };
    if (unit < u_end) load_images(unit);

    for (int t = wave; t < n_tiles; t += 2 * kFilterWaves) {
        const int t2 = t + kFilterWaves;
        double c0[kStageRegs], c1[kStageRegs], r0[DP], r1[DP];
        filter_stage_fetch<DP>(t, lane, centers, k, d, c0, r0);
        if (t2 < n_tiles) filter_stage_fetch<DP>(t2, lane, centers, k, d, c1, r1);
        filter_stage_build<NM>(t, lane, reinterpret_cast<unsigned short*>(img + (size_t)t * NM * 64), c0, r0, k, d, tab, hs,
                               &any_bad);
        if (t2 < n_tiles)
            filter_stage_build<NM>(t2, lane, reinterpret_cast<unsigned short*>(img + (size_t)t2 * NM * 64), c1, r1, k, d, tab, hs,
                                   &any_bad);
    }
    __syncthreads();
    const bool all_scan = any_bad != 0;
    KSTAMP(0);

    unsigned long long my_scans = 0;
    const bool vec_rows = sizeof(T) == 8 && d == DP && ((ld * sizeof(T)) & 15) == 0 && (((uintptr_t)x) & 15) == 0;
    const int iters = n_tiles / 2;
    constexpr int kNone = 0x7fffffff;

    auto load_frame = [&](int64_t t, double (&z)[DP]) { filter_load_frame<T, DP, WHITEN>(x, ld, d, vec_rows, mean, stdv, t, z); };
    auto score64 = [&](const double* crow, int c, const double (&z)[DP]) {
        double a = 0.0;
#pragma unroll
        for (int f = 0; f < DP; ++f)
            if (f < d) a = fma(crow[f], z[f], a);
        return a - hs[c];
    };
    auto write_label = [&](int64_t t, int bidx, double bm, const double (&z)[DP]) {
        labels[t] = bidx;
        if (mindist) {
            double zsq = 0.0;
#pragma unroll
            for (int f = 0; f < DP; ++f) zsq = fma(z[f], z[f], zsq);
            const double md = -2.0 * bm + zsq;
            mindist[t] = md > 0.0 ? md : 0.0;
        }
    };
    auto commit_scan = [&](int64_t t, int sbi, double sbest, const double (&zz)[DP], int old_s) {
        if constexpr (ACCUM) {
            if (!labels || old_s != sbi) {
#pragma unroll
                for (int f = 0; f < DP; ++f) {
                    if (f < d && lane == f) {
                        const unsigned long long fx = (unsigned long long)to_fixed(zz[f], scale);
                        atomicAdd(&lsum[(size_t)sbi * d + f], fx);
                        if (old_s >= 0) atomicAdd(&lsum[(size_t)old_s * d + f], 0ull - fx);
                    }
                }
                if (lane == 0) {
                    atomicAdd(&lcnt[sbi], 1ull);
                    if (old_s >= 0) atomicAdd(&lcnt[old_s], ~0ull);
                    if (labels) labels[t] = sbi;
                }
            }
        } else {
            if (lane == 0) write_label(t, sbi, sbest, zz);
        }
    };
    auto scan_frame = [&](int64_t t) {
        double zz[DP];
        load_frame(t, zz);
        double sbest = -__builtin_inf();
        int sbi = kNone;
        for (int c = lane; c < k; c += 64) {
            const double sc = score64(centers + (size_t)c * d, c, zz);
            if (sc > sbest) { sbest = sc; sbi = c; }
        }
#pragma unroll
        for (int off = 1; off < 64; off <<= 1) {
            const double ob = __shfl_xor(sbest, off, 64);
            const int oi = __shfl_xor(sbi, off, 64);
            if (ob > sbest || (ob == sbest && oi < sbi)) { sbest = ob; sbi = oi; }
        }
        if (sbi >= k) { sbi = 0; sbest = -__builtin_inf(); }
        int old_s = -1;
        if constexpr (ACCUM) {
            if (labels) old_s = labels[t];
        }
        commit_scan(t, sbi, sbest, zz, old_s);
#ifdef MSM_KMF_DIAG_COUNT
        if (MSM_KMF_DIAG_COUNT == 1) ++my_scans;
#else
        ++my_scans;
#endif
    };

    while (unit < u_end) {
        int nt = 0;
        if (lane == 0) nt = atomicAdd(&unit_ctr, 1);
        const int64_t nxt = u_begin + __builtin_amdgcn_readfirstlane(nt);
        KSTAMP_VM(1);
        float b1[NF], b2[NF];
        int bp[NF];
#pragma unroll
        for (int u = 0; u < NF; ++u) { b1[u] = -__builtin_inff(); b2[u] = -__builtin_inff(); bp[u] = 0; }
#ifdef MSM_KMF_DIAG_NOTILE
        for (int it = 0; it < (iters < 9 ? iters : 9); ++it) {
#else
        for (int it = 0; it < iters; ++it) {
#endif
            const int jt = 2 * it;
            v8bf aa[NM], ab[NM];
#pragma unroll
            for (int m = 0; m < NM; ++m) {
                aa[m] = __builtin_bit_cast(v8bf, img[((jt + 0) * NM + m) * 64 + lane]);
                ab[m] = __builtin_bit_cast(v8bf, img[((jt + 1) * NM + m) * 64 + lane]);
            }
            v4f32 acca[NF], accb[NF];
#pragma unroll
            for (int u = 0; u < NF; ++u) {
                acca[u] = __builtin_amdgcn_mfma_f32_16x16x32_bf16(aa[0], b[u][0], (v4f32){0.f, 0.f, 0.f, 0.f}, 0, 0, 0);
                accb[u] = __builtin_amdgcn_mfma_f32_16x16x32_bf16(ab[0], b[u][0], (v4f32){0.f, 0.f, 0.f, 0.f}, 0, 0, 0);
            }
            if constexpr (NM == 2) {
#pragma unroll
                for (int u = 0; u < NF; ++u) {
                    acca[u] = __builtin_amdgcn_mfma_f32_16x16x32_bf16(aa[1], b[u][1], acca[u], 0, 0, 0);
                    accb[u] = __builtin_amdgcn_mfma_f32_16x16x32_bf16(ab[1], b[u][1], accb[u], 0, 0, 0);
                }
            }
#pragma unroll
            for (int u = 0; u < NF; ++u) {
                float m = max3_f32(b2[u], acca[u][0], acca[u][1]);
                m = max3_f32(m, acca[u][2], acca[u][3]);
                m = max3_f32(m, accb[u][0], accb[u][1]);
                m = max3_f32(m, accb[u][2], accb[u][3]);
                const bool better = m > b1[u];
                b2[u] = med3_f32(b1[u], b2[u], m);
                b1[u] = hw_max_f32(b1[u], m);
                bp[u] = better ? jt : bp[u];
            }
        }
        KSTAMP(2);
        bool guard[NF];
#pragma unroll
        for (int u = 0; u < NF; ++u) guard[u] = q == 3 && __builtin_bit_cast(unsigned short, b[u][NM - 1][7]) == 0x7F80;
        if (nxt < u_end) load_images(nxt);
        const int64_t f0 = unit * kUnit + lane;
        const bool fok = f0 < n;
        const int64_t fr = fok ? f0 : n - 1;
        int old = -1;
        if constexpr (ACCUM) {
            if (labels) old = labels[fr];
        }
        double z[DP];
        load_frame(fr, z);
        int cd = kNone;
        float Ru = __builtin_inff();
#ifdef MSM_KMF_DIAG_NOCROSS
        cd = bp[0] | (q << 16);
        Ru = b2[0] + b1[1] + b1[2] + b1[3] + b2[1] + b2[2] + b2[3] + (guard[0] | guard[1] | guard[2] | guard[3] ? 1.f : 0.f) + (float)(bp[1] + bp[2] + bp[3]);
#else
#pragma unroll
        for (int u = 0; u < NF; ++u) {
            const float M1 = xrow_max_f32(b1[u]);
            const int code_u = xrow_min_i32(b1[u] == M1 ? ((q << 16) | bp[u]) : kNone);
            const int gs = code_u >> 16;
            float r = q == gs ? b2[u] : b1[u];
            if (guard[u]) r = __builtin_inff();
            const float R_u = xrow_max_f32(r);
            cd = q == u ? code_u : cd;
            Ru = q == u ? R_u : Ru;
        }
#endif
        KSTAMP(3);
        const int gs = cd >> 16, pstar = cd & 0xffff;
        const int base = min(pstar * 16 + 4 * gs, n_tiles * 16 - 20);
        float pz[DP];
        float qz = 0.f;
#pragma unroll
        for (int f = 0; f < DP; ++f) {
            pz[f] = (float)z[f];
            qz = __builtin_fmaf(pz[f], pz[f], qz);
        }
        const bool z_bad = !(qz < __builtin_inff());
        const float zn = hw_max_f32(__builtin_amdgcn_sqrtf(qz) * kUp20, 1.0f);
        float s1 = -__builtin_inff(), s2 = -__builtin_inff(), sbmax = 0.f;
        int i1 = 0;
#ifndef MSM_KMF_DIAG_NOPICK
        const float* p_row = tab + (size_t)base * RF;
#pragma unroll
        for (int c = 0; c < 8; ++c) {
            const float4* r4 = reinterpret_cast<const float4*>(p_row + ((c & 3) + 16 * (c >> 2)) * RF);
            float a = 0.f, h, cn;
            if constexpr (NM == 1) {
                const float4 r0 = r4[0], r1 = r4[1];
                a = __builtin_fmaf(r0.x, pz[0], a);
                a = __builtin_fmaf(r0.y, pz[1], a);
                a = __builtin_fmaf(r0.z, pz[2], a);
                a = __builtin_fmaf(r0.w, pz[3], a);
                h = r1.x;
                cn = r1.y;
            } else {
                const float4 r0 = r4[0], r1 = r4[1], r2 = r4[2];
                a = __builtin_fmaf(r0.x, pz[0], a);
                a = __builtin_fmaf(r0.y, pz[1], a);
                a = __builtin_fmaf(r0.z, pz[2], a);
                a = __builtin_fmaf(r0.w, pz[3], a);
                a = __builtin_fmaf(r1.x, pz[4], a);
                a = __builtin_fmaf(r1.y, pz[5], a);
                a = __builtin_fmaf(r1.z, pz[6], a);
                a = __builtin_fmaf(r1.w, pz[7], a);
                a = __builtin_fmaf(r2.x, pz[8], a);
                a = __builtin_fmaf(r2.y, pz[9], a);
                h = r2.z;
                cn = r2.w;
            }
            const float s = a - h;
            sbmax = hw_max_f32(sbmax, __builtin_fmaf(zn, cn, h));
            const bool better = s > s1;
            s2 = med3_f32(s1, s2, s);
            s1 = hw_max_f32(s1, s);
            i1 = better ? c : i1;
        }
#endif
        const float e = __builtin_fmaf(kPickEps, sbmax, kPickFloor);
        const int jw = base + (i1 & 3) + 16 * (i1 >> 2);
        const bool certified = !all_scan && !z_bad && cd != kNone && jw < k && s1 - s2 > 2.0f * e && s1 - e > Ru;
        const int lab = jw;
#if defined(MSM_KMF_DIAG_NOSCAN) || defined(MSM_KMF_DIAG_NOQUEUE)
        unsigned long long todo = 0;
#else
        unsigned long long todo = __ballot(fok && !certified);
#endif
        KSTAMP(4);
#ifdef MSM_KMF_DIAG_NOCOMMIT
        if (fok && certified && cd == 12345) {
#else
        if (fok && certified) {
#endif
            if constexpr (ACCUM) {
                if (!labels || old != lab) {
#pragma unroll
                    for (int f = 0; f < DP; ++f) {
                        if (f < d) {
                            const unsigned long long fx = (unsigned long long)to_fixed(z[f], scale);
                            atomicAdd(&lsum[(size_t)lab * d + f], fx);
                            if (old >= 0) atomicAdd(&lsum[(size_t)old * d + f], 0ull - fx);
                        }
                    }
                    atomicAdd(&lcnt[lab], 1ull);
                    if (old >= 0) atomicAdd(&lcnt[old], ~0ull);
                    if (labels) labels[f0] = lab;
                }
            } else {
                if (mindist) write_label(f0, lab, score64(centers + (size_t)lab * d, lab, z), z);
                else labels[f0] = lab;
            }
        }
        KSTAMP(5);
        while (todo) {
            const int jf = __builtin_ctzll(todo);
            todo &= todo - 1;
            const int64_t t = ((int64_t)__builtin_amdgcn_readlane((int)(f0 >> 32), jf) << 32) |
                              (unsigned)__builtin_amdgcn_readlane((int)f0, jf);
            const bool plain = all_scan || __builtin_amdgcn_readlane((int)(z_bad || !(Ru < __builtin_inff())), jf) != 0;
            if (plain) {
                scan_frame(t);
                continue;
            }
            float zf[DP];
#pragma unroll
            for (int f = 0; f < DP; ++f) zf[f] = __int_as_float(__builtin_amdgcn_readlane(__float_as_int(pz[f]), jf));
            const float znj = __int_as_float(__builtin_amdgcn_readlane(__float_as_int(zn), jf));
            float t1 = -__builtin_inff(), t2 = -__builtin_inff(), t3 = -__builtin_inff(), sbl = 0.f;
            int c1 = 0, c2 = 0;
            for (int c = lane; c < n_tiles * 16; c += 64) {
                const float4* r4 = reinterpret_cast<const float4*>(tab + (size_t)c * RF);
                float a = 0.f, h, cn;
                if constexpr (NM == 1) {
                    const float4 r0 = r4[0], r1 = r4[1];
                    a = __builtin_fmaf(r0.x, zf[0], a);
                    a = __builtin_fmaf(r0.y, zf[1], a);
                    a = __builtin_fmaf(r0.z, zf[2], a);
                    a = __builtin_fmaf(r0.w, zf[3], a);
                    h = r1.x;
                    cn = r1.y;
                } else {
                    const float4 r0 = r4[0], r1 = r4[1], r2 = r4[2];
                    a = __builtin_fmaf(r0.x, zf[0], a);
                    a = __builtin_fmaf(r0.y, zf[1], a);
                    a = __builtin_fmaf(r0.z, zf[2], a);
                    a = __builtin_fmaf(r0.w, zf[3], a);
                    a = __builtin_fmaf(r1.x, zf[4], a);
                    a = __builtin_fmaf(r1.y, zf[5], a);
                    a = __builtin_fmaf(r1.z, zf[6], a);
                    a = __builtin_fmaf(r1.w, zf[7], a);
                    a = __builtin_fmaf(r2.x, zf[8], a);
                    a = __builtin_fmaf(r2.y, zf[9], a);
                    h = r2.z;
                    cn = r2.w;
                }
                const float sc = a - h;
                sbl = hw_max_f32(sbl, __builtin_fmaf(znj, cn, h));
                if (sc > t1) { t3 = t2; t2 = t1; c2 = c1; t1 = sc; c1 = c; }
                else if (sc > t2) { t3 = t2; t2 = sc; c2 = c; }
                else t3 = hw_max_f32(t3, sc);
            }
            double rowa[DP], rowb[DP];
            {
                const double* ca = centers + (size_t)(c1 < k ? c1 : 0) * d;
                const double* cb = centers + (size_t)(c2 < k ? c2 : 0) * d;
#pragma unroll
                for (int f = 0; f < DP; ++f) {
                    rowa[f] = f < d ? ca[f] : 0.0;
                    rowb[f] = f < d ? cb[f] : 0.0;
                }
            }
            const float top = wave_max_f32(t1), sbw = wave_max_f32(sbl);
            const float band = top - 2.0f * __builtin_fmaf(kPickEps, sbw, kPickFloor);
            const unsigned long long in1 = __ballot(t1 >= band);
            if (__any(t3 >= band) || in1 == 0ull) {
                scan_frame(t);
                continue;
            }
            double zz[DP];
#pragma unroll
            for (int f = 0; f < DP; ++f) {
                const long long bits = __double_as_longlong(z[f]);
                zz[f] = __longlong_as_double((long long)(((unsigned long long)(unsigned)__builtin_amdgcn_readlane((int)(bits >> 32), jf) << 32) |
                                                         (unsigned)__builtin_amdgcn_readlane((int)bits, jf)));
            }
            const int old_t = __builtin_amdgcn_readlane(old, jf);
            int sbi;
            double sbest = 0.0;
            const bool two = __any(t2 >= band) || __builtin_popcountll(in1) > 1;
            if (!two && !(mindist && !ACCUM)) {
                sbi = __builtin_amdgcn_readlane(c1, __builtin_ctzll(in1));
            } else {
                double m1 = -__builtin_inf();
                int i1b = kNone;
                auto chain = [&](const double (&row)[DP], int c) {
                    double a = 0.0;
#pragma unroll
                    for (int f = 0; f < DP; ++f) a = fma(row[f], zz[f], a);
                    return a - hs[c];
                };
                if (t1 >= band && c1 < k) { m1 = chain(rowa, c1); i1b = c1; }
                if (t2 >= band && c2 < k) {
                    const double m2 = chain(rowb, c2);
                    if (m2 > m1 || (m2 == m1 && c2 < i1b)) { m1 = m2; i1b = c2; }
                }
                sbest = wave_max_f64(m1);
                sbi = wave_min_i32(m1 == sbest ? i1b : kNone);
                if (sbi >= k) {
                    scan_frame(t);
                    continue;
                }
            }
            commit_scan(t, sbi, sbest, zz, old_t);
#ifdef MSM_KMF_DIAG_COUNT
            if (MSM_KMF_DIAG_COUNT == 2 && two) ++my_scans;
#else
            ++my_scans;
#endif
        }
        KSTAMP(6);
        unit = nxt;
    }
    KSTAMP(7);
    if (n_scanned && lane == 0 && my_scans) atomicAdd(n_scanned, my_scans);
    if constexpr (ACCUM) {
        __syncthreads();
        for (int i = tid; i < k * d; i += kMT)
            if (lsum[i]) atomicAdd(&sums[i], lsum[i]);
        for (int i = tid; i < k; i += kMT)
            if (lcnt[i]) atomicAdd(&counts[i], lcnt[i]);
        if (upd_centers) {
            __shared__ int is_last;
            asm volatile("s_waitcnt vmcnt(0)" ::: "memory");
            __syncthreads();
            if (tid == 0) {
                const unsigned t = __hip_atomic_fetch_add(ticket, 1u, __ATOMIC_RELAXED, __HIP_MEMORY_SCOPE_AGENT);
                is_last = t == gridDim.x - 1;
                if (is_last) __hip_atomic_store(ticket, 0u, __ATOMIC_RELAXED, __HIP_MEMORY_SCOPE_AGENT);
            }
            __syncthreads();
            if (is_last) filter_close_iteration<kMT>(sums, counts, k, d, upd_centers, const_cast<FitState*>(st));
        }
    }
    KSTAMP_FLUSH
}

static inline size_t filter_lds_bytes(int k, int d, bool accum) {
    if (d > kFilterMaxD) return 0;
    const int nm = filter_nm(d);
    const int k16 = (k + 15) & ~15;
    const int n_tiles = ((k16 / 16) + 1) & ~1;
    const size_t tile_bytes = nm == 1 ? FilterShape<1>::kTileBytes : FilterShape<2>::kTileBytes;
    const size_t total = (size_t)n_tiles * tile_bytes + (accum ? (size_t)k * (d + 1) * sizeof(unsigned long long) : 0);
    const size_t cap = 160 * 1024 - 64;
    return total <= cap ? total : 0;
}
```

### pmarlo_amd/device.py

```python

from __future__ import annotations

import ctypes as C
import os
import sys
from typing import Iterable, Sequence

import numpy as np

from . import _lib
from ._lib import check, lib

__all__ = ["Engine", "DeviceArray", "get_engine", "segments_to_bounds"]


def _dtype_code(dtype: np.dtype) -> int:
    dtype = np.dtype(dtype)
    if dtype == np.float32:
        return _lib.MSM_F32
    if dtype == np.float64:
        return _lib.MSM_F64
    raise TypeError(f"feature matrices must be float32 or float64, got {dtype}")


# ... 283 lines not shown
        width = P + Tn + (Q if dihedral_mode == 0 else 2 * Q)
        out = out if out is not None else self.empty((n, width), np.float32)
        ld = out.shape[1]
        if P:
            check(lib.msm_featurize_distances(self.handle, xyz.ptr, n, A, dp.ptr, P, out.ptr, ld, 0), self.handle)
        if Tn:
            check(lib.msm_featurize_angles(self.handle, xyz.ptr, n, A, dt.ptr, Tn, out.ptr, ld, P), self.handle)
        if Q:
            check(lib.msm_featurize_dihedrals(self.handle, xyz.ptr, n, A, dq.ptr, Q, int(dihedral_mode), out.ptr, ld,
                                              P + Tn), self.handle)
        self.sync()
        return out

    def featurize_distances_into(self, xyz: DeviceArray, pairs: DeviceArray, out: DeviceArray, col0: int = 0) -> DeviceArray:
        n, A, _ = xyz.shape
        check(lib.msm_featurize_distances(self.handle, xyz.ptr, n, A, pairs.ptr, pairs.shape[0], out.ptr, out.shape[1],
                                          int(col0)), self.handle)
        return out

    @staticmethod
    def _seg_ptrs(starts: np.ndarray, stops: np.ndarray):
        starts = np.ascontiguousarray(starts, np.int64)
        stops = np.ascontiguousarray(stops, np.int64)
        if starts.shape != stops.shape:
            raise ValueError("segment starts/stops differ in length")
        return starts, stops

    def count_transitions(self, labels: DeviceArray, k: int, lag: int, *, starts=None, stops=None,
                          stride: int = 1, out: DeviceArray | None = None,
                          pairs: DeviceArray | None = None) -> tuple[DeviceArray, DeviceArray]:
        n = labels.size
        if starts is None:
            starts, stops = segments_to_bounds(None, n)
        starts, stops = self._seg_ptrs(starts, stops)
        out = out if out is not None else self.empty((k, k), np.int64)
        pairs = pairs if pairs is not None else self.empty((1,), np.int64)
        check(lib.msm_count_transitions(self.handle, labels.ptr, n, starts.ctypes.data, stops.ctypes.data,
                                        len(starts), int(lag), int(stride), int(k), out.ptr, pairs.ptr),
              self.handle)
        return out, pairs

    def count_transitions_weighted(self, labels: DeviceArray, weights: DeviceArray, k: int, lag: int, *,
                                   starts=None, stops=None, stride: int = 1,
                                   out: DeviceArray | None = None, pairs: DeviceArray | None = None):
        n = labels.size
        if weights.size != n or weights.dtype != np.float64:
            raise ValueError("weights must be float64 with one entry per label")
        if starts is None:
            starts, stops = segments_to_bounds(None, n)
        starts, stops = self._seg_ptrs(starts, stops)
        out = out if out is not None else self.empty((k, k), np.float64)
        pairs = pairs if pairs is not None else self.empty((1,), np.int64)
        check(lib.msm_count_transitions_weighted(self.handle, labels.ptr, weights.ptr, n, starts.ctypes.data,
                                                 stops.ctypes.data, len(starts), int(lag), int(stride),
                                                 int(k), out.ptr, pairs.ptr), self.handle)
        return out, pairs

    def count_transitions_lagscan(self, labels: DeviceArray, k: int, lags: Sequence[int], *, starts=None,
                                  stops=None, out: DeviceArray | None = None,
                                  pairs: DeviceArray | None = None):
        n = labels.size
        lags_arr = np.ascontiguousarray(lags, np.int32)
        if starts is None:
            starts, stops = segments_to_bounds(None, n)
        starts, stops = self._seg_ptrs(starts, stops)
        L = len(lags_arr)
        out = out if out is not None else self.empty((L, k, k), np.int64)
        pairs = pairs if pairs is not None else self.empty((L,), np.int64)
        check(lib.msm_count_transitions_lagscan(self.handle, labels.ptr, n, starts.ctypes.data,
                                                stops.ctypes.data, len(starts), lags_arr.ctypes.data, L,
                                                int(k), out.ptr, pairs.ptr), self.handle)
        return out, pairs

    def state_counts(self, labels: DeviceArray, k: int, out: DeviceArray | None = None) -> DeviceArray:
        out = out if out is not None else self.empty((k,), np.int64)
        check(lib.msm_state_counts(self.handle, labels.ptr, labels.size, int(k), out.ptr), self.handle)
        return out

    def run_lengths(self, labels: DeviceArray, k: int):
        n = labels.size
        stats = self.empty((4, int(k)), np.int64)
        rs, rl = self.empty((max(n, 1),), np.int32), self.empty((max(n, 1),), np.int64)
        cnt = self.empty((1,), np.int64)
        check(lib.msm_run_lengths(self.handle, labels.ptr, n, int(k), stats.ptr, rs.ptr, rl.ptr, n, cnt.ptr), self.handle)
        r = int(cnt.to_host()[0])
        return stats.to_host(), rs.to_host()[:r], rl.to_host()[:r]

    def column_moments(self, x: DeviceArray, ddof: int = 0):
        n, F = x.shape
        mean, std, cnt = (self.empty((F,), np.float64) for _ in range(3))
        check(lib.msm_column_moments(self.handle, x.ptr, _dtype_code(x.dtype), n, F, F, int(ddof), mean.ptr,
                                     std.ptr, cnt.ptr), self.handle)
        return mean, std, cnt

    def column_minmax(self, x: DeviceArray):
        n, F = x.shape
        mn, mx, cnt = self.empty((F,), np.float64), self.empty((F,), np.float64), self.empty((2,), np.int64)
        check(lib.msm_column_minmax(self.handle, x.ptr, _dtype_code(x.dtype), n, F, F, mn.ptr, mx.ptr, cnt.ptr), self.handle)
        return mn, mx, cnt

    def column_moments_partial(self, x: DeviceArray, shift: DeviceArray | None = None,
                               sums: DeviceArray | None = None):
        n, F = x.shape
        sums = sums if sums is not None else self.empty((3 * F,), np.float64)
        shift_out = self.empty((F,), np.float64) if shift is None else None
        check(lib.msm_column_moments_partial(self.handle, x.ptr, _dtype_code(x.dtype), n, F, F,
                                             shift.ptr if shift is not None else None, sums.ptr,
                                             shift_out.ptr if shift_out is not None else None), self.handle)
        return sums, (shift_out if shift_out is not None else shift)

    def moments_finalize(self, sums: DeviceArray, shift: DeviceArray, F: int, ddof: int = 0):
        mean, std, cnt = (self.empty((F,), np.float64) for _ in range(3))
        check(lib.msm_moments_finalize(self.handle, sums.ptr, shift.ptr, F, int(ddof), mean.ptr, std.ptr,
                                       cnt.ptr), self.handle)
        return mean, std, cnt

    def standardise_params(self, sums: DeviceArray, shift: DeviceArray, F: int, n_rows: float, with_std: bool = True,
                           out=None):
        mean, scale, inv = out if out is not None else tuple(self.empty((F,), np.float64) for _ in range(3))
        check(lib.msm_standardise_params(self.handle, sums.ptr, shift.ptr, F, float(n_rows), int(bool(with_std)),
                                         mean.ptr, scale.ptr, inv.ptr), self.handle)
        return mean, scale, inv

    def lagged_moments(self, x: DeviceArray, lag: int, shift: DeviceArray, *, starts=None, stops=None,
                       assume_finite: bool = False, out: DeviceArray | None = None,
                       one_sided: bool = False, symmetric: bool = False) -> DeviceArray:
        if one_sided and symmetric:
            raise ValueError("one_sided and symmetric moments exclude each other")
        n, F = x.shape
        if starts is None:
            starts, stops = segments_to_bounds(None, n)
        starts, stops = self._seg_ptrs(starts, stops)
        out = out if out is not None else self.empty((2 * F * F + 2 * F + 1,), np.float64)
        fn = (lib.msm_lagged_moments_onesided if one_sided
              else lib.msm_lagged_moments_reversible if symmetric else lib.msm_lagged_moments)
        check(fn(self.handle, x.ptr, _dtype_code(x.dtype), n, F, F, starts.ctypes.data, stops.ctypes.data, len(starts),
                 int(lag), shift.ptr, int(bool(assume_finite)), out.ptr), self.handle)
        return out

    def onesided_tica_eigenvalues(self, moments: DeviceArray, F: int, clip: float = 1e-12) -> DeviceArray:
        out = self.empty((F,), np.float64)
        check(lib.msm_onesided_tica_eigenvalues(self.handle, moments.ptr, int(F), float(clip), out.ptr), self.handle)
        return out

    def moments_from_lagged(self, x: DeviceArray, lag: int, shift: DeviceArray, moments: DeviceArray, *, starts=None,
                            stops=None, out: DeviceArray | None = None) -> DeviceArray:
        n, F = x.shape
        if starts is None:
            starts, stops = segments_to_bounds(None, n)
        starts, stops = self._seg_ptrs(starts, stops)
        out = out if out is not None else self.empty((3 * F,), np.float64)
        check(lib.msm_moments_from_lagged(self.handle, x.ptr, _dtype_code(x.dtype), n, F, F, starts.ctypes.data,
                                          stops.ctypes.data, len(starts), int(lag), shift.ptr, moments.ptr, out.ptr),
              self.handle)
        return out

    def tica_solve(self, moments: DeviceArray, F: int, *, scale: DeviceArray | None = None,
                   epsilon: float = 1e-6, kinetic_map: bool = True, out=None):
        if out is not None:
            eig, W, mean, rank = out
        else:
            eig = self.empty((F,), np.float64)
            W = self.empty((F, F), np.float64)
            mean = self.empty((F,), np.float64)
            rank = self.empty((1,), np.int32)
        check(lib.msm_tica_solve(self.handle, moments.ptr, scale.ptr if scale is not None else None, F,
                                 float(epsilon), int(bool(kinetic_map)), eig.ptr, W.ptr, mean.ptr, rank.ptr),
              self.handle)
        return eig, W, mean, rank

    def project(self, x: DeviceArray, mu: DeviceArray, inv_sigma: DeviceArray, W: DeviceArray, d: int, *,
                mean2: DeviceArray | None = None, out: DeviceArray | None = None,
                absmax: DeviceArray | None = None, assume_finite: bool = False) -> DeviceArray:
        n, F = x.shape
        ldw = W.shape[1]
        out = out if out is not None else self.empty((n, d), np.float64)
        fn = lib.msm_project_finite if assume_finite else lib.msm_project
        check(fn(self.handle, x.ptr, _dtype_code(x.dtype), n, F, F, mu.ptr, inv_sigma.ptr,
                 mean2.ptr if mean2 is not None else None, W.ptr, int(d), ldw, out.ptr,
                 out.shape[1], absmax.ptr if absmax is not None else None), self.handle)
        return out

    def eigh(self, a: DeviceArray, want_vectors: bool = True):
        n = a.shape[0]
        w = self.empty((n,), np.float64)
        v = self.empty((n, n), np.float64) if want_vectors else None
        sweeps = self.empty((1,), np.int32)
        check(lib.msm_eigh(self.handle, a.ptr, n, w.ptr, v.ptr if v is not None else None, sweeps.ptr),
              self.handle)
        return w, v, sweeps

    def kmeans_assign(self, x: DeviceArray, centers: DeviceArray, *, mean: DeviceArray | None = None,
                      std: DeviceArray | None = None, labels: DeviceArray | None = None,
                      mindist: DeviceArray | None = None, image: DeviceArray | None = None) -> DeviceArray:
        n, d = x.shape
        k, dc = centers.shape
        if dc != d:
            raise ValueError(f"centres have {dc} features, data has {d}")
        if centers.dtype != np.float64:
            raise TypeError("centres must be float64")
        labels = labels if labels is not None else self.empty((n,), np.int32)
        check(lib.msm_kmeans_assign_packed(self.handle, x.ptr, _dtype_code(x.dtype), n, d, d, centers.ptr, k,
                                           mean.ptr if mean is not None else None,
                                           std.ptr if std is not None else None,
                                           image.ptr if image is not None else None, labels.ptr,
                                           mindist.ptr if mindist is not None else None), self.handle)
        return labels


    FIT_STATE_FIELDS = ("scale", "inv_scale", "absmax", "shift2", "tol2", "done", "n_iter", "inertia")

    def kmeans_fit(self, x: DeviceArray, k: int, *, seed: int = 0, max_iter: int = 50, tol2: float = 0.0,
                   mean: DeviceArray | None = None, std: DeviceArray | None = None,
                   centers: DeviceArray | None = None) -> tuple[DeviceArray, DeviceArray]:
        n, d = x.shape
        init = centers is None
        centers = centers if centers is not None else self.empty((k, d), np.float64)
        state = self.zeros((8,), np.float64)
        check(lib.msm_kmeans_fit(self.handle, x.ptr, _dtype_code(x.dtype), n, d, d,
                                 mean.ptr if mean is not None else None, std.ptr if std is not None else None,
                                 int(k), int(seed) & (2**64 - 1), int(init), int(max_iter), float(tol2), centers.ptr,
                                 state.ptr), self.handle)
        return centers, state

    def kmeans_init_plusplus(self, x: DeviceArray, k: int, *, seed: int = 0, mean: DeviceArray | None = None,
                             std: DeviceArray | None = None, n_total: int | None = None,
                             centers: DeviceArray | None = None, return_picked: bool = False):
        n, d = x.shape
        n_total = n if n_total is None else int(n_total)
        centers, state = self.kmeans_fit_begin(x, k, seed=seed, n_total=n_total, tol2=0.0, mean=mean, std=std,
                                               centers=centers, init_centers=False)
        picked = self.empty((k,), np.int64) if return_picked else None
        check(lib.msm_kmeans_init_plusplus(self.handle, x.ptr, _dtype_code(x.dtype), n, d, d,
                                           mean.ptr if mean is not None else None, std.ptr if std is not None else None,
                                           int(k), int(seed) & (2**64 - 1), float(n_total), centers.ptr, state.ptr,
                                           picked.ptr if picked is not None else None), self.handle)
        return (centers, picked) if return_picked else centers

    def kmeans_fit_minibatch(self, x: DeviceArray, k: int, *, seed: int = 0, batch_size: int = 100, max_iter: int = 5,
                             init: str = "kmeans++", centers: DeviceArray | None = None,
                             max_batches: int = 4096) -> tuple[DeviceArray, DeviceArray]:
        n, d = x.shape
        if batch_size < 1 or max_iter < 0:
            raise ValueError("batch_size must be >= 1 and max_iter >= 0")
        given = centers is not None
        n_terms = n * max(1, int(max_iter))
        centers, state = self.kmeans_fit_begin(x, k, seed=seed, n_total=n_terms, tol2=0.0, centers=centers,
                                               init_centers=not given and init != "kmeans++")
        if not given and init == "kmeans++":
            check(lib.msm_kmeans_init_plusplus(self.handle, x.ptr, _dtype_code(x.dtype), n, d, d, None, None, int(k),
                                               int(seed) & (2**64 - 1), float(n_terms), centers.ptr, state.ptr, None),
                  self.handle)
        nb = max(1, min(int(max_batches), -(-n // int(batch_size))))
        sums, counts = self.zeros((k * d,), np.int64), self.zeros((k,), np.int64)
        item = x.dtype.itemsize
        for _ in range(int(max_iter)):
            for b in range(nb):
                rows = (n - b + nb - 1) // nb
                if rows <= 0:
                    continue
                check(lib.msm_kmeans_accumulate(self.handle, x.ptr + b * d * item, _dtype_code(x.dtype), rows, d, nb * d,
                                                centers.ptr, k, None, None, state.ptr, sums.ptr, counts.ptr), self.handle)
                check(lib.msm_kmeans_update(self.handle, sums.ptr, counts.ptr, k, d, centers.ptr, state.ptr, 0), self.handle)
        return centers, state

    def kmeans_fit_begin(self, x: DeviceArray, k: int, *, seed: int, n_total: int, tol2: float,
                         mean: DeviceArray | None = None, std: DeviceArray | None = None,
                         centers: DeviceArray | None = None, init_centers: bool = True,
                         state: DeviceArray | None = None, absmax_ready: bool = False):
        n, d = x.shape
        centers = centers if centers is not None else self.empty((k, d), np.float64)
        state = state if state is not None else self.zeros((8,), np.float64)
        check(lib.msm_kmeans_fit_begin(self.handle, x.ptr, _dtype_code(x.dtype), n, d, d,
                                       mean.ptr if mean is not None else None,
                                       std.ptr if std is not None else None, int(k), int(seed) & (2**64 - 1),
                                       int(bool(init_centers)), float(n_total), float(tol2), centers.ptr, state.ptr,
                                       int(bool(absmax_ready))), self.handle)
        return centers, state

    def kmeans_accumulate(self, x: DeviceArray, centers: DeviceArray, state: DeviceArray, sums: DeviceArray,
                          counts: DeviceArray, *, mean: DeviceArray | None = None, std: DeviceArray | None = None,
                          image: DeviceArray | None = None, prev_labels: DeviceArray | None = None):
        n, d = x.shape
        k = centers.shape[0]
        if prev_labels is not None:
            check(lib.msm_kmeans_accumulate_delta(self.handle, x.ptr, _dtype_code(x.dtype), n, d, d, centers.ptr, k,
                                                  mean.ptr if mean is not None else None,
                                                  std.ptr if std is not None else None,
                                                  image.ptr if image is not None else None, state.ptr,
                                                  prev_labels.ptr, sums.ptr, counts.ptr), self.handle)
            return
        check(lib.msm_kmeans_accumulate_packed(self.handle, x.ptr, _dtype_code(x.dtype), n, d, d, centers.ptr, k,
                                               mean.ptr if mean is not None else None,
                                               std.ptr if std is not None else None,
                                               image.ptr if image is not None else None, state.ptr, sums.ptr,
                                               counts.ptr), self.handle)

    def kmeans_image_bytes(self, n: int, d: int) -> int:
        out = C.c_size_t(0)
        check(lib.msm_kmeans_image_bytes(int(n), int(d), C.byref(out)), self.handle)
        return int(out.value)

    def kmeans_pack(self, x: DeviceArray, *, mean: DeviceArray | None = None, std: DeviceArray | None = None,
                    image: DeviceArray | None = None) -> DeviceArray | None:
        n, d = x.shape
        nbytes = self.kmeans_image_bytes(n, d)
        if nbytes == 0:
            return None
        image = image if image is not None else self.empty((nbytes,), np.uint8)
        if image.nbytes < nbytes:
            raise ValueError(f"image buffer holds {image.nbytes} bytes, {nbytes} needed")
        check(lib.msm_kmeans_pack(self.handle, x.ptr, _dtype_code(x.dtype), n, d, d,
                                  mean.ptr if mean is not None else None, std.ptr if std is not None else None,
                                  image.ptr), self.handle)
        return image

    def kmeans_filter_scanned(self, reset: bool = False) -> int:
        out = C.c_uint64(0)
        check(lib.msm_kmeans_filter_scanned(self.handle, C.byref(out), int(reset)), self.handle)
        return int(out.value)

    def mfma_bf16_probe(self, a_bits: np.ndarray, b_bits: np.ndarray, c: np.ndarray) -> np.ndarray:
        a = np.ascontiguousarray(a_bits, np.uint16)
        b = np.ascontiguousarray(b_bits, np.uint16)
        cc = np.ascontiguousarray(c, np.float32)
        t = a.shape[0]
        if a.shape != (t, 16, 32) or b.shape != (t, 32, 16) or cc.shape != (t, 16, 16):
            raise ValueError("mfma_bf16_probe: shapes must be [t,16,32], [t,32,16], [t,16,16]")
        out = np.empty((t, 16, 16), np.float32)
        check(lib.msm_mfma_bf16_probe(self.handle, a.ctypes.data, b.ctypes.data, cc.ctypes.data, out.ctypes.data, t),
              self.handle)
        return out

    def kmeans_lloyd_pass(self, x: DeviceArray, centers: DeviceArray, state: DeviceArray, sums: DeviceArray,
                          counts: DeviceArray, *, mean: DeviceArray | None = None, std: DeviceArray | None = None,
                          image: DeviceArray | None = None, prev_labels: DeviceArray | None = None):
        n, d = x.shape
        k = centers.shape[0]
        check(lib.msm_kmeans_lloyd_pass(self.handle, x.ptr, _dtype_code(x.dtype), n, d, d, centers.ptr, k,
                                        mean.ptr if mean is not None else None, std.ptr if std is not None else None,
                                        image.ptr if image is not None else None, state.ptr,
                                        prev_labels.ptr if prev_labels is not None else None, sums.ptr, counts.ptr),
              self.handle)

    def kmeans_update(self, sums: DeviceArray, counts: DeviceArray, centers: DeviceArray, state: DeviceArray,
                      clear: bool = True):
        k, d = centers.shape
        check(lib.msm_kmeans_update(self.handle, sums.ptr, counts.ptr, k, d, centers.ptr, state.ptr, int(clear)),
              self.handle)

    def sum_f64(self, v: DeviceArray, out: DeviceArray | None = None) -> DeviceArray:
        out = out if out is not None else self.empty((1,), np.float64)
        check(lib.msm_sum_f64(self.handle, v.ptr, v.size, out.ptr), self.handle)
        return out


    def transition_matrix(self, counts: DeviceArray, *, mode: int = 0, alpha: float = 1e-3,
                          epsilon: float = 1e-12) -> dict:
        k = counts.shape[0]
        if counts.dtype not in (np.dtype(np.int64), np.dtype(np.float64)):
            raise TypeError("counts must be int64 or float64")
        T = self.empty((k, k), np.float64)
        rowsum = self.empty((k,), np.float64)
        out = {"T": T, "rowsum": rowsum}
        if mode == 0:
            dm = self.empty((1,), np.float64)
            check(lib.msm_transition_matrix(self.handle, counts.ptr, int(counts.dtype == np.float64), k, 0, 0.0, 0.0,
                                            T.ptr, None, None, None, rowsum.ptr, dm.ptr), self.handle)
            out["diag_mass"] = dm
        else:
            active, inv = self.empty((k,), np.int32), self.empty((k,), np.int32)
            na = self.empty((1,), np.int32)
            check(lib.msm_transition_matrix(self.handle, counts.ptr, int(counts.dtype == np.float64), k, 1,
                                            float(alpha), float(epsilon), T.ptr, active.ptr, inv.ptr, na.ptr,
                                            rowsum.ptr, None), self.handle)
            out.update(active=active, inv_map=inv, n_active=na)
        return out

    def row_normalise_into(self, counts: DeviceArray, T: DeviceArray, rowsum: DeviceArray, diag_mass: DeviceArray):
        k = counts.shape[0]
        check(lib.msm_transition_matrix(self.handle, counts.ptr, int(counts.dtype == np.float64), k, 0, 0.0, 0.0,
                                        T.ptr, None, None, None, rowsum.ptr, diag_mass.ptr), self.handle)

    def rcp(self, src: DeviceArray, dst: DeviceArray) -> None:
        check(lib.msm_rcp_f64(self.handle, src.ptr, src.size, dst.ptr), self.handle)

    def embed_full(self, T_active: DeviceArray, inv_map: DeviceArray, pi_active: DeviceArray | None = None):
        k = T_active.shape[0]
        T_full = self.empty((k, k), np.float64)
        pi_full = self.empty((k,), np.float64)
        check(lib.msm_embed_full(self.handle, T_active.ptr, pi_active.ptr if pi_active is not None else None,
                                 inv_map.ptr, k, T_full.ptr, pi_full.ptr), self.handle)
        return T_full, pi_full

    def silhouette(self, x_sorted: DeviceArray, offsets) -> tuple[float, DeviceArray]:
        n, d = x_sorted.shape
        off = np.ascontiguousarray(offsets, np.int64)
        samples = self.empty((n,), np.float64)
        score = self.empty((1,), np.float64)
        check(lib.msm_silhouette(self.handle, x_sorted.ptr, n, d, d, off.ctypes.data, len(off) - 1, samples.ptr, score.ptr),
              self.handle)
        return float(score.to_host()[0]), samples

    def grid_cells(self, x: DeviceArray, edges: np.ndarray) -> DeviceArray:
        n, F = x.shape
        e = np.ascontiguousarray(edges, np.float64)
        if e.shape[0] != F:
            raise ValueError("edges must have one row per feature")
        flat = self.empty((n,), np.int32)
        dt = _lib.MSM_F32 if x.dtype == np.float32 else _lib.MSM_F64
        ed = self.to_device(e)
        check(lib.msm_grid_cells(self.handle, x.ptr, dt, n, F, F, ed.ptr, e.shape[1] - 1, flat.ptr), self.handle)
        self.sync()
        return flat

    def first_occurrence(self, flat: DeviceArray, n_cells: int) -> np.ndarray:
        first = self.empty((int(n_cells),), np.int64)
        check(lib.msm_first_occurrence(self.handle, flat.ptr, flat.size, int(n_cells), first.ptr), self.handle)
        return first.to_host()

    def relabel(self, flat: DeviceArray, cell_map: np.ndarray) -> DeviceArray:
        m = self.to_device(np.ascontiguousarray(cell_map, np.int32))
        labels = self.empty((flat.size,), np.int32)
        check(lib.msm_relabel(self.handle, flat.ptr, flat.size, m.ptr, m.size, labels.ptr), self.handle)
        self.sync()
        return labels

    def solve(self, A: DeviceArray, B: DeviceArray) -> int:
        n = A.shape[0]
        nrhs = 1 if len(B.shape) == 1 else B.shape[1]
        info = self.empty((1,), np.int32)
        check(lib.msm_solve_f64(self.handle, n, nrhs, A.ptr, A.shape[1], B.ptr, nrhs, info.ptr), self.handle)
        return int(info.to_host()[0])

    def reactive_flux(self, T: DeviceArray, pi: DeviceArray, role: np.ndarray, want_flux: bool = True) -> dict:
        n = T.shape[0]
        rd = self.to_device(np.ascontiguousarray(role, np.int32))
        qp, qm = self.empty((n,), np.float64), self.empty((n,), np.float64)
        info = self.empty((2,), np.int32)
        gross = net = tot = None
        if want_flux:
            gross, net, tot = self.empty((n, n), np.float64), self.empty((n, n), np.float64), self.empty((4,), np.float64)
        check(lib.msm_reactive_flux(self.handle, T.ptr, n, pi.ptr, rd.ptr, n, qp.ptr, qm.ptr,
                                    gross.ptr if gross is not None else None, net.ptr if net is not None else None,
                                    tot.ptr if tot is not None else None, info.ptr), self.handle)
        return {"qplus": qp, "qminus": qm, "gross": gross, "net": net, "totals": tot, "info": info.to_host()}

    def lump_macro(self, T: DeviceArray, pi: DeviceArray, macro: np.ndarray, n_macro: int):
        n = T.shape[0]
        md = self.to_device(np.ascontiguousarray(macro, np.int32))
        Tm, pm = self.empty((n_macro, n_macro), np.float64), self.empty((n_macro,), np.float64)
        check(lib.msm_lump_macro(self.handle, T.ptr, n, pi.ptr, md.ptr, n, int(n_macro), Tm.ptr, pm.ptr), self.handle)
        return Tm, pm

    def macro_mfpt(self, T: DeviceArray):
        n = T.shape[0]
        out = self.empty((n, n), np.float64)
        info = self.empty((n,), np.int32)
        check(lib.msm_macro_mfpt(self.handle, T.ptr, n, n, out.ptr, info.ptr), self.handle)
        return out, info.to_host()

    def weighted_stats(self, x: DeviceArray, col: int = 0, weights: DeviceArray | None = None) -> np.ndarray:
        if len(x.shape) == 1:
            n, stride, off = x.shape[0], 1, 0
        else:
            n, stride, off = x.shape[0], x.shape[1], int(col)
        out = self.empty((6,), np.float64)
        check(lib.msm_weighted_stats(self.handle, x.ptr + off * 8, stride, n, weights.ptr if weights is not None else None,
                                     out.ptr), self.handle)
        return out.to_host()

    def gather(self, table: DeviceArray, idx: DeviceArray) -> DeviceArray:
        out = self.empty((idx.size,), np.float64)
        check(lib.msm_gather_f64(self.handle, table.ptr, table.size, idx.ptr, idx.size, out.ptr), self.handle)
        return out

    def hist2d_xy(self, x, y, xedges: np.ndarray, yedges: np.ndarray) -> DeviceArray:
        def col(a):
            if isinstance(a, tuple):
                arr, c = a
                return arr.ptr + int(c) * 8, arr.shape[1], arr.shape[0]
            return a.ptr, 1, a.size
        (px, sx, n), (py, sy, _) = col(x), col(y)
        nx, ny = len(xedges) - 1, len(yedges) - 1
        xe = self.to_device(np.ascontiguousarray(xedges, np.float64))
        ye = self.to_device(np.ascontiguousarray(yedges, np.float64))
        h = self.empty((nx, ny), np.float64)
        check(lib.msm_hist2d(self.handle, px, sx, py, sy, n, None, 0.0, xe.ptr, nx, ye.ptr, ny, h.ptr), self.handle)
        return h

    def clip_or_wrap(self, x: DeviceArray, lo: float, hi: float, *, wrap: bool, col: int = 0) -> DeviceArray:
        if len(x.shape) == 1:
            n, stride, off = x.shape[0], 1, 0
        else:
            n, stride, off = x.shape[0], x.shape[1], int(col)
        out = self.empty((n,), np.float64)
        check(lib.msm_clip_or_wrap(self.handle, x.ptr + off * 8, stride, n, float(lo), float(hi), 2 if wrap else 1,
                                   out.ptr), self.handle)
        return out

    def order_statistics(self, x: DeviceArray, ranks, col: int = 0) -> np.ndarray:
        if len(x.shape) == 1:
            n, stride, off = x.shape[0], 1, 0
        else:
            n, stride, off = x.shape[0], x.shape[1], int(col)
        r = np.ascontiguousarray(ranks, dtype=np.int64).ravel()
        out = np.empty(r.size, dtype=np.float64)
        check(lib.msm_order_statistics(self.handle, x.ptr + off * 8, stride, n, r.ctypes.data, r.size, out.ctypes.data),
              self.handle)
        return out

    def hist2d(self, x: DeviceArray, cols, xedges: np.ndarray, yedges: np.ndarray,
               weights: DeviceArray | None = None, w_absmax: float = 0.0) -> DeviceArray:
        n, d = x.shape
        nx, ny = len(xedges) - 1, len(yedges) - 1
        xe, ye = self.to_device(np.ascontiguousarray(xedges, np.float64)), self.to_device(np.ascontiguousarray(yedges, np.float64))
        h = self.empty((nx, ny), np.float64)
        check(lib.msm_hist2d(self.handle, x.ptr + int(cols[0]) * 8, d, x.ptr + int(cols[1]) * 8, d, n,
                             weights.ptr if weights is not None else None, float(w_absmax), xe.ptr, nx, ye.ptr, ny, h.ptr),
              self.handle)
        return h

    def smooth_sparse_bins(self, hist: DeviceArray, min_count: float) -> tuple[DeviceArray, int]:
        nx, ny = hist.shape
        out = self.empty((nx, ny), np.float64)
        cnt = self.empty((1,), np.int32)
        check(lib.msm_smooth_sparse_bins(self.handle, hist.ptr, nx, ny, float(min_count), out.ptr, cnt.ptr), self.handle)
        return out, int(cnt.to_host()[0])

    def scale_to_total(self, v: DeviceArray, total: float) -> None:
        check(lib.msm_scale_to_total(self.handle, v.ptr, v.size, float(total)), self.handle)

    def fes_finalize(self, hist: DeviceArray, kT: float) -> tuple[DeviceArray, int]:
        F = self.empty(hist.shape, np.float64)
        st = self.empty((1,), np.int32)
        check(lib.msm_fes_finalize(self.handle, hist.ptr, hist.size, float(kT), F.ptr, st.ptr), self.handle)
        return F, int(st.to_host()[0])

    def kde2d(self, x: DeviceArray, cols, xcenters: np.ndarray, ycenters: np.ndarray, bw_x: float, bw_y: float,
              weights: DeviceArray | None, w_scale: float, periodic: int = 0) -> DeviceArray:
        n, d = x.shape
        xc, yc = self.to_device(np.ascontiguousarray(xcenters, np.float64)), self.to_device(np.ascontiguousarray(ycenters, np.float64))
        dens = self.empty((len(xcenters), len(ycenters)), np.float64)
        check(lib.msm_kde2d(self.handle, x.ptr + int(cols[0]) * 8, d, x.ptr + int(cols[1]) * 8, d, n,
                            weights.ptr if weights is not None else None, float(w_scale), xc.ptr, len(xcenters), yc.ptr,
                            len(ycenters), float(bw_x), float(bw_y), int(periodic), dens.ptr), self.handle)
        return dens

    def gemm(self, A: DeviceArray, B: DeviceArray, out: DeviceArray | None = None) -> DeviceArray:
        m, k = A.shape
        k2, n = B.shape
        if k != k2:
            raise ValueError(f"gemm: inner dimensions differ ({k} vs {k2})")
        C = out if out is not None else self.empty((m, n), np.float64)
        check(lib.msm_gemm_f64(self.handle, m, n, k, A.ptr, k, B.ptr, n, C.ptr, n), self.handle)
        return C

    def ck_test(self, T1: DeviceArray, Tk: DeviceArray, factors, rowcounts: DeviceArray | None = None):
        n = T1.shape[0]
        fac = np.ascontiguousarray(factors, dtype=np.int32)
        F = int(fac.size)
        if tuple(Tk.shape) != (F, n, n):
            raise ValueError(f"ck_test: Tk must have shape ({F}, {n}, {n}), got {tuple(Tk.shape)}")
        mse = self.empty((max(F, 1),), np.float64)
        noise = self.empty((max(F, 1),), np.float64) if rowcounts is not None else None
        check(lib.msm_ck_test(self.handle, T1.ptr, n, Tk.ptr, n * n, n, n, fac.ctypes.data, F,
                              rowcounts.ptr if rowcounts is not None else None, n, mse.ptr,
                              noise.ptr if noise is not None else None), self.handle)
        return mse.to_host()[:F], (noise.to_host()[:F] if noise is not None else None)

    def matrix_power(self, T: DeviceArray, squarings: int, *, n: DeviceArray | None = None) -> DeviceArray:
        B = T.shape[0] if len(T.shape) == 3 else 1
        k = T.shape[-1]
        out = self.empty(T.shape, np.float64)
        tmp = self.empty(T.shape, np.float64) if squarings > 1 else None
        check(lib.msm_matrix_power(self.handle, T.ptr, k * k, k, n.ptr if n is not None else None, k, B, int(squarings),
                                   tmp.ptr if tmp is not None else None, out.ptr), self.handle)
        return out

    def spectrum(self, T: DeviceArray, *, n: DeviceArray | None = None, n_its: int = 0, lags=None,
                 p: int | None = None, want_pi: bool = True, tol: float = 1e-9, n_iter: int = 24,
                 max_launches: int = 100, seed: int = 0, allow_unconverged: bool = False, n_vecs: int = 0,
                 n_watch: int | None = None, squarings: int | None = None) -> dict:
        if squarings is None:
            squarings = int(os.environ.get("MSM_SPEC_SQUARINGS", "2")) if T.shape[-1] >= 32 else 0
        if squarings > 0:
            B = T.shape[0] if len(T.shape) == 3 else 1
            it_pow = int(os.environ.get("MSM_SPEC_NITER", -n_iter if B == 1 else max(6, (2 * n_iter) // 3)))
            try:
                return self._spectrum(T, self.matrix_power(T, squarings, n=n), it_pow, n=n, n_its=n_its, lags=lags, p=p,
                                      want_pi=want_pi, tol=tol, max_launches=max(8, max_launches // 2), seed=seed,
                                      allow_unconverged=False, n_vecs=n_vecs, n_watch=n_watch)
            except _lib.MsmError:
                pass
        return self._spectrum(T, None, n_iter, n=n, n_its=n_its, lags=lags, p=p, want_pi=want_pi, tol=tol,
                              max_launches=max_launches, seed=seed, allow_unconverged=allow_unconverged, n_vecs=n_vecs,
                              n_watch=n_watch)

    def _spectrum(self, T: DeviceArray, Tpow: DeviceArray | None, n_iter: int, *, n, n_its, lags, p, want_pi, tol,
                  max_launches, seed, allow_unconverged, n_vecs, n_watch) -> dict:
        batched = len(T.shape) == 3
        B = T.shape[0] if batched else 1
        k = T.shape[-1]
        n_vecs = int(min(n_vecs, 32, k))
        watch = int(n_watch) if n_watch is not None else max(n_its + 1, n_vecs, 1)
        if p is None:
            p = min(32, max(watch + 6, 8))
        p = int(min(p, 32, k))
        ws_bytes = int(lib.msm_spectrum_workspace_bytes(k, p, B))
        cache = getattr(self, "_spec_cache", None)
        key = (k, B, max(n_its, 1))
        m_its = max(n_its, 1)
        if cache is None or cache[0] != key or cache[1].size < ws_bytes:
            outs = self.empty((B * (129 + 2 * m_its) + (B + 1) // 2,), np.float64)
            cache = (key, self.empty((ws_bytes,), np.uint8), outs)
            self._spec_cache = cache
        _, ws, outs = cache
        o_change, o_eig, o_ts, o_status = B * 128, B * 129, B * (129 + m_its), B * (129 + 2 * m_its)
        ritz = self.wrap(outs.ptr, (B, 128), np.float64)
        change = self.wrap(outs.ptr + 8 * o_change, (B,), np.float64)
        its_eig = self.wrap(outs.ptr + 8 * o_eig, (B, m_its), np.float64)
        its_ts = self.wrap(outs.ptr + 8 * o_ts, (B, m_its), np.float64)
        status = self.wrap(outs.ptr + 8 * o_status, (B,), np.int32)
        pi = self.empty((B, k), np.float64) if want_pi else None
        vecs = self.empty((B, n_vecs, k), np.float64) if n_vecs else None
        lag_d = self.to_device(np.asarray(lags if lags is not None else np.ones(B), np.float64).reshape(B))
        launches = 0
        restart = True
        since_restart = 0
        worst = prev = float("inf")
        ramp = n_iter < 0
        n_iter_max = abs(int(n_iter))
        for launch in range(max_launches):
            n_iter = min(n_iter_max, 6 << max(0, launch - 1)) if ramp else n_iter_max
# ... 97 lines not shown
```

### pmarlo_amd/dist.py

```python

from __future__ import annotations

import ctypes as C
import os
import time
from dataclasses import dataclass
from pathlib import Path

import numpy as np

from .device import DeviceArray, Engine

__all__ = ["Comm", "NativeComm", "TorchComm", "ShardedMSM", "ShardConfig", "exchange_shapes", "exchange_aliases",
           "torch_exchange_buffers", "bootstrap_id"]


class Comm:

    world = 1
    rank = 0

    def allreduce_sum(self, name: str) -> None: ...
    def allreduce_sum_from(self, name: str, src) -> None: ...
    def allreduce_min(self, name: str) -> None: ...
# ... 52 lines not shown

    def __init__(self, engine: Engine, bufs: dict[str, DeviceArray], rank: int, world: int, uid: bytes,
                 id_file: str | os.PathLike | None = None):
        from ._lib import check, lib

        self.eng, self.b, self.rank, self.world = engine, bufs, int(rank), int(world)
        self._lib, self._check = lib, check
        handle = C.c_void_p()
        idbuf = (C.c_ubyte * 128).from_buffer_copy(uid)
        check(lib.msm_comm_init(engine.handle, self.rank, self.world, idbuf, 128, C.byref(handle)), engine.handle)
        self.handle = handle
        self._id_file = id_file
        self.timing = False
        self.events: dict[str, list] = {}

    @classmethod
    def from_env(cls, engine: Engine, bufs: dict[str, DeviceArray]) -> "NativeComm":
        rank, world = int(os.environ.get("RANK", "0")), int(os.environ.get("WORLD_SIZE", "1"))
        path = _resolve_id_path(world)
        if rank == 0:
            try:
                os.unlink(path)
            except OSError:
                pass
        self = cls(engine, bufs, rank, world, bootstrap_id(rank, world, path), id_file=path)
        if "timing" in bufs:
            self.allreduce_max("timing")
            engine.sync()
            if rank == 0:
                try:
                    os.unlink(path)
                except OSError:
                    pass
        return self

    def comm_info(self) -> tuple[int, int]:
        r, w = C.c_int32(0), C.c_int32(0)
        self._check(self._lib.msm_comm_info(self.handle, C.byref(r), C.byref(w), None), self.eng.handle)
        return int(r.value), int(w.value)

    def _timed(self, name, call):
        if not self.timing:
            return call()
        e0, e1 = self.eng.event(), self.eng.event()
        e0.record()
        call()
        e1.record()
        self.events.setdefault(name, []).append((e0, e1))

    def exchange_ms(self) -> dict[str, float]:
        return {nm: float(sum(a.elapsed_ms(b) for a, b in evs)) for nm, evs in self.events.items()}

    def close(self) -> None:
        if getattr(self, "handle", None):
            self._lib.msm_comm_destroy(self.handle)
            self.handle = None

    def __del__(self):
        try:
            self.close()
        except Exception:
            pass

    @property
    def n_collectives(self) -> int:
        n = C.c_uint64(0)
        self._check(self._lib.msm_comm_info(self.handle, None, None, C.byref(n)), self.eng.handle)
        return int(n.value)

    def allreduce_sum(self, name):
        a = self.b[name]
        fn = self._lib.msm_allreduce_i64 if a.dtype == np.int64 else self._lib.msm_allreduce_f64
        if a.dtype not in (np.dtype(np.int64), np.dtype(np.float64)):
            raise TypeError(f"exchange buffer {name!r} must be int64 or float64")
        self._timed(name, lambda: self._check(fn(self.handle, a.ptr, a.size), self.eng.handle))

    def allreduce_sum_from(self, name, src):
        a = self.b[name]
        if a.dtype != np.dtype(np.int64) or src.dtype != a.dtype or src.size != a.size:
            raise TypeError(f"exchange buffer {name!r}: the out-of-place sum takes int64 arrays of one size")
        self._timed(name, lambda: self._check(self._lib.msm_allreduce_i64_from(self.handle, src.ptr, a.ptr, a.size),
                                              self.eng.handle))

    def allreduce_min(self, name):
        a = self.b[name]
        self._timed(name, lambda: self._check(self._lib.msm_allreduce_min_f64(self.handle, a.ptr, a.size), self.eng.handle))

    def allreduce_max(self, name):
        a = self.b[name]
        self._timed(name, lambda: self._check(self._lib.msm_allreduce_max_f64(self.handle, a.ptr, a.size), self.eng.handle))

    def broadcast(self, name, src=0):
        a = self.b[name]
        self._timed(name, lambda: self._check(self._lib.msm_broadcast(self.handle, a.ptr, a.nbytes, int(src)),
                                              self.eng.handle))

    def reciprocal(self, dst, src):
        self.eng.rcp(self.b[src], self.b[dst])


class TorchComm(Comm):

    def __init__(self, tensors: dict, views: dict | None = None):
        import torch.distributed as dist

        self.dist = dist
        self.t = tensors
        self.v = views
        self.world = dist.get_world_size()
        self.rank = dist.get_rank()
        self._gather: dict = {}
        self._into_tensor = dist.get_backend() == "nccl"
        self.n_collectives = 0

    def allreduce_sum(self, name):
        t = self.t[name]
        self.n_collectives += 1
        if not t.dtype.is_floating_point:
            self.dist.all_reduce(t, op=self.dist.ReduceOp.SUM)
            return
        import torch

        buf = self._gather.get(name)
        if buf is None:
            buf = torch.empty((self.world,) + tuple(t.shape), dtype=t.dtype, device=t.device)
            self._gather[name] = buf
        if self._into_tensor:
            self.dist.all_gather_into_tensor(buf, t)
        else:
            self.dist.all_gather([buf[r] for r in range(self.world)], t)
        acc = buf[0].clone()
        for r in range(1, self.world):
            acc += buf[r]
        t.copy_(acc)

    def allreduce_sum_from(self, name, src):
        if self.v is None:
            raise RuntimeError("TorchComm needs the engine's views of the exchange buffers for an out-of-place sum")
        self.v[name].copy_from(src)
        self.n_collectives += 1
        self.dist.all_reduce(self.t[name], op=self.dist.ReduceOp.SUM)

    def allreduce_min(self, name):
        self.n_collectives += 1
        self.dist.all_reduce(self.t[name], op=self.dist.ReduceOp.MIN)

    def allreduce_max(self, name):
        self.n_collectives += 1
        self.dist.all_reduce(self.t[name], op=self.dist.ReduceOp.MAX)

    def broadcast(self, name, src=0):
        self.n_collectives += 1
        self.dist.broadcast(self.t[name], src=src)

    def reciprocal(self, dst, src):
        import torch

        torch.reciprocal(self.t[src], out=self.t[dst])


@dataclass
class ShardConfig:
    n_frames: int
    n_features: int
    tica_dim: int
    k: int
    lag: int
    kmeans_iters: int = 10
    seed: int = 0
    n_total: int | None = None
    lags: tuple | None = None
    n_atoms: int = 0
    pairs: np.ndarray | None = None

    @property
    def cluster_dim(self) -> int:
        return self.tica_dim if self.tica_dim > 0 else self.n_features


def exchange_shapes(cfg: ShardConfig) -> dict[str, tuple[tuple[int, ...], str]]:
    F, d, k = cfg.n_features, cfg.cluster_dim, cfg.k
    L = len(cfg.lags) if cfg.lags else 1
    return {
        "shift": ((F,), "float64"),
        "moments": ((2 * F * F + 2 * F + 1 + 3 * F,), "float64"),
        "fit_state": ((8,), "float64"),
        "start": ((k * d + 1,), "float64"),
        "km_acc": ((k * d + k,), "int64"),
        "counts": ((L * k * k + L,), "int64"),
    }


def exchange_aliases(cfg: ShardConfig) -> dict[str, tuple[str, int, int]]:
    F, d, k = cfg.n_features, cfg.cluster_dim, cfg.k
    L = 2 * F * F + 2 * F + 1
    return {"lagged": ("moments", 0, L), "mom_sums": ("moments", L, 3 * F),
            "fit_scale": ("fit_state", 0, 1), "fit_inv_scale": ("fit_state", 1, 1),
            "centers": ("start", 0, k * d), "start_scale": ("start", k * d, 1)}


class ShardedMSM:

    def __init__(self, engine: Engine, cfg: ShardConfig, x: DeviceArray, comm: Comm | None = None,
                 shared: dict[str, DeviceArray] | None = None, always_exchange: bool = False):
        self.eng, self.cfg = engine, cfg
        self.comm = comm
        self.always_exchange = bool(always_exchange) and comm is not None
        self.world = comm.world if comm else 1
        self.n_total = cfg.n_total if cfg.n_total is not None else cfg.n_frames * self.world
        eng = engine
        F, d, k, n = cfg.n_features, cfg.cluster_dim, cfg.k, cfg.n_frames
        self.buf = shared if shared is not None else {
            nm: eng.zeros(shape, np.dtype(dt)) for nm, (shape, dt) in exchange_shapes(cfg).items()}
        b = self.buf
        for name, (parent, first, length) in exchange_aliases(cfg).items():
            if name not in b:
                b[name] = b[parent].view((length,), offset_elems=first)
        b["centers"] = b["start"].view((k, d))
        if cfg.n_atoms > 0:
            if cfg.pairs is None or len(cfg.pairs) != F:
                raise ValueError("ShardConfig.pairs must list n_features atom pairs")
            self.xyz = x
            self.pairs_d = eng.to_device(np.ascontiguousarray(cfg.pairs, np.int32).reshape(F, 2))
            self.x = eng.empty((n, F), np.float32)
            eng.featurize_distances_into(self.xyz, self.pairs_d, self.x)
        else:
            self.xyz = None
            self.x = x
        if cfg.tica_dim > 0:
            self.mean, self.scale, self.inv_scale = (eng.empty((F,), np.float64) for _ in range(3))
            self.eig = eng.empty((F,), np.float64)
            self.W = eng.empty((F, F), np.float64)
            self.m2 = eng.empty((F,), np.float64)
            self.rank_d = eng.empty((1,), np.int32)
            self.Y = eng.empty((n, d), np.float64)
        else:
            self.Y = self.x
        self.labels = eng.empty((n,), np.int32)
        self.T = eng.empty((k, k), np.float64)
        self.rowsum = eng.empty((k,), np.float64)
        self.diag = eng.empty((1,), np.float64)
        self.km_sums = b["km_acc"].view((k * d,), np.int64)
        self.km_counts = b["km_acc"].view((k,), np.int64, offset_elems=k * d)
        multi_shard = self.comm is not None and (self.comm.world > 1 or self.always_exchange)
        self.km_local = eng.empty((k * d + k,), np.int64) if multi_shard else None
        nbytes = eng.kmeans_image_bytes(n, d)
        self.km_image = eng.empty((nbytes,), np.uint8) if nbytes else None
        self.accum_events: list = []
        self.stage_events: dict = {}
        self.time_accum = False
        self.time_stages = False
        if cfg.tica_dim > 0:
            _, first = eng.column_moments_partial(self.x)
            b["shift"].copy_from_host(first.to_host())
            if comm and (comm.world > 1 or self.always_exchange):
                comm.broadcast("shift", 0)

    @property
    def collectives_per_step(self) -> int:
        return (3 if self.cfg.tica_dim > 0 else 2) + self.cfg.kmeans_iters

    def _stamp(self, name: str):
        if self.time_stages:
            ev = self.eng.event()
            ev.record()
            self.stage_events.setdefault(name, []).append(ev)

    def step(self) -> None:
        eng, cfg, b, comm = self.eng, self.cfg, self.buf, self.comm
        multi = comm is not None and (comm.world > 1 or self.always_exchange)
        F, d, k = cfg.n_features, cfg.cluster_dim, cfg.k
        self._stamp("begin")
        if self.xyz is not None:
            eng.featurize_distances_into(self.xyz, self.pairs_d, self.x)
            self._stamp("featurize")
        if cfg.tica_dim > 0:
            eng.lagged_moments(self.x, cfg.lag, b["shift"], assume_finite=True, out=b["lagged"], symmetric=True)
            eng.moments_from_lagged(self.x, cfg.lag, b["shift"], b["lagged"], out=b["mom_sums"])
            if multi:
                comm.allreduce_sum("moments")
            eng.standardise_params(b["mom_sums"], b["shift"], F, float(self.n_total), True,
                                   out=(self.mean, self.scale, self.inv_scale))
            self._stamp("moments")
            eng.tica_solve(b["lagged"], F, scale=self.scale, epsilon=1e-6, kinetic_map=True,
                           out=(self.eig, self.W, self.m2, self.rank_d))
            self._stamp("tica_solve")
            eng.project(self.x, b["shift"], self.inv_scale, self.W, d, mean2=self.m2, out=self.Y,
                        absmax=b["fit_state"].view((1,), offset_elems=2), assume_finite=True)
            self._stamp("project")
        eng.kmeans_fit_begin(self.Y, k, seed=cfg.seed, n_total=self.n_total, tol2=0.0, centers=b["centers"],
                             state=b["fit_state"], absmax_ready=cfg.tica_dim > 0)
        if multi:
            if comm.rank != 0:
                b["centers"].fill_bytes_(0x7F)
            b["start_scale"].copy_from(b["fit_scale"])
            comm.allreduce_min("start")
            b["fit_scale"].copy_from(b["start_scale"])
            comm.reciprocal("fit_inv_scale", "fit_scale")
        acc = self.km_local if self.km_local is not None else b["km_acc"]
        acc.zero_()
        acc_sums, acc_counts = acc.view((k * d,), np.int64), acc.view((k,), np.int64, offset_elems=k * d)
        self.labels.fill_bytes_(0xFF)
        if self.km_image is not None:
            eng.kmeans_pack(self.Y, image=self.km_image)
        for _ in range(cfg.kmeans_iters):
            if self.time_accum:
                e0, e1 = eng.event(), eng.event()
                e0.record()
            if not multi:
                eng.kmeans_lloyd_pass(self.Y, b["centers"], b["fit_state"], acc_sums, acc_counts,
                                      image=self.km_image, prev_labels=self.labels)
            else:
                eng.kmeans_accumulate(self.Y, b["centers"], b["fit_state"], acc_sums, acc_counts,
                                      image=self.km_image, prev_labels=self.labels)
            if self.time_accum:
                e1.record()
                self.accum_events.append((e0, e1))
            if multi:
                comm.allreduce_sum_from("km_acc", self.km_local)
                eng.kmeans_update(self.km_sums, self.km_counts, b["centers"], b["fit_state"], clear=False)
        eng.kmeans_assign(self.Y, b["centers"], labels=self.labels, image=self.km_image)
        self._stamp("kmeans")
        if cfg.lags:
            L = len(cfg.lags)
            eng.count_transitions_lagscan(self.labels, k, cfg.lags, out=b["counts"].view((L, k, k)),
                                          pairs=b["counts"].view((L,), offset_elems=L * k * k))
            if multi:
                comm.allreduce_sum("counts")
            li = list(cfg.lags).index(cfg.lag) if cfg.lag in cfg.lags else 0
            eng.row_normalise_into(b["counts"].view((k, k), offset_elems=li * k * k), self.T, self.rowsum, self.diag)
        else:
            eng.count_transitions(self.labels, k, cfg.lag, out=b["counts"].view((k, k)),
                                  pairs=b["counts"].view((1,), offset_elems=k * k))
            if multi:
                comm.allreduce_sum("counts")
            eng.row_normalise_into(b["counts"].view((k, k)), self.T, self.rowsum, self.diag)
        self._stamp("counts")

    def lagscan_counts(self) -> np.ndarray:
        L, k = len(self.cfg.lags), self.cfg.k
        return self.buf["counts"].view((L, k, k)).to_host()


def torch_exchange_buffers(engine: Engine, cfg: ShardConfig, device) -> tuple[dict, dict]:
    import torch

    tensors, views = {}, {}
    for name, (shape, dt) in exchange_shapes(cfg).items():
        t = torch.zeros(shape, dtype=getattr(torch, dt), device=device)
        tensors[name] = t
        views[name] = engine.wrap(t.data_ptr(), shape, np.dtype(dt))
    for name, (parent, first, length) in exchange_aliases(cfg).items():
        tensors[name] = tensors[parent][first:first + length]
        views[name] = views[parent].view((length,), offset_elems=first)
    return tensors, views
```

Measured before the change: 659.4 million frames/s.

## Switch k-means filter from split-bf16 MFMA to scaled single-f16 MFMA

Replaces the multi-piece bf16 split encoding of points and centers in the k-means distance filter with a single scaled f16 encoding. The scale comes from a global absmax, so each tile needs one f16 MFMA per 16x16x32 block instead of one or two bf16 MFMAs, and the center-norm term is folded into the accumulator init. The packed image shrinks to a fixed three quads per row. The pack step now takes the absmax already computed by projection, or computes it with an extra kernel when none is given. Lower f16 precision is covered by a widened error bound (kappa) and the existing rescan fallback, which may trigger more exact rescans.

```diff
diff --git a/include/msmhip.h b/include/msmhip.h
--- a/include/msmhip.h
+++ b/include/msmhip.h
@@ -169,6 +169,8 @@
 msm_status msm_kmeans_image_bytes(int64_t n, int d, size_t* out_bytes);
 msm_status msm_kmeans_pack(msm_ctx* ctx, const void* d_x, msm_dtype dtype, int64_t n, int d, int64_t ld,
                            const double* d_mean, const double* d_std, void* d_image);
+msm_status msm_kmeans_pack_bounded(msm_ctx* ctx, const void* d_x, msm_dtype dtype, int64_t n, int d, int64_t ld,
+                                   const double* d_mean, const double* d_std, const double* d_absmax, void* d_image);
 msm_status msm_kmeans_assign_packed(msm_ctx* ctx, const void* d_x, msm_dtype dtype, int64_t n, int d,
                                     int64_t ld, const double* d_centers, int k, const double* d_mean,
                                     const double* d_std, const void* d_image, int32_t* d_labels,
@@ -188,6 +190,8 @@
 msm_status msm_kmeans_filter_scanned(msm_ctx* ctx, uint64_t* h_out, int reset);
 msm_status msm_mfma_bf16_probe(msm_ctx* ctx, const uint16_t* h_a, const uint16_t* h_b, const float* h_c,
                                float* h_d, int n_tiles);
+msm_status msm_mfma_f16_probe(msm_ctx* ctx, const uint16_t* h_a, const uint16_t* h_b, const float* h_c,
+                              float* h_d, int n_tiles);
 
 msm_status msm_sum_f64(msm_ctx* ctx, const double* d_v, int64_t n, double* d_out);
 
diff --git a/pmarlo_amd/_lib.py b/pmarlo_amd/_lib.py
--- a/pmarlo_amd/_lib.py
+++ b/pmarlo_amd/_lib.py
@@ -90,6 +90,7 @@
     "msm_rcp_f64": (_i32, [_vp, _vp, _sz, _vp]),
     "msm_kmeans_image_bytes": (_i32, [_i64, _i32, C.POINTER(_sz)]),
     "msm_kmeans_pack": (_i32, [_vp, _vp, _i32, _i64, _i32, _i64, _vp, _vp, _vp]),
+    "msm_kmeans_pack_bounded": (_i32, [_vp, _vp, _i32, _i64, _i32, _i64, _vp, _vp, _vp, _vp]),
     "msm_kmeans_assign_packed": (_i32, [_vp, _vp, _i32, _i64, _i32, _i64, _vp, _i32, _vp, _vp, _vp, _vp, _vp]),
     "msm_kmeans_accumulate_packed": (_i32, [_vp, _vp, _i32, _i64, _i32, _i64, _vp, _i32, _vp, _vp, _vp, _vp, _vp, _vp]),
     "msm_kmeans_lloyd_pass": (_i32, [_vp, _vp, _i32, _i64, _i32, _i64, _vp, _i32, _vp, _vp, _vp, _vp, _vp, _vp, _vp]),
@@ -98,6 +99,7 @@
     "msm_kmeans_filter_scanned": (_i32, [_vp, C.POINTER(C.c_uint64), _i32]),
     "msm_kmeans_init_plusplus": (_i32, [_vp, _vp, _i32, _i64, _i32, _i64, _vp, _vp, _i32, C.c_uint64, _f64, _vp, _vp, _vp]),
     "msm_mfma_bf16_probe": (_i32, [_vp, _vp, _vp, _vp, _vp, _i32]),
+    "msm_mfma_f16_probe": (_i32, [_vp, _vp, _vp, _vp, _vp, _i32]),
     "msm_run_lengths": (_i32, [_vp, _vp, _i64, _i32, _vp, _vp, _vp, _i64, _vp]),
     "msm_sum_f64": (_i32, [_vp, _vp, _i64, _vp]),
     "msm_transition_matrix": (_i32, [_vp, _vp, _i32, _i32, _i32, _f64, _f64, _vp, _vp, _vp, _vp, _vp, _vp]),
diff --git a/pmarlo_amd/csrc/kmeans.hip b/pmarlo_amd/csrc/kmeans.hip
--- a/pmarlo_amd/csrc/kmeans.hip
+++ b/pmarlo_amd/csrc/kmeans.hip
@@ -774,6 +774,24 @@
     for (int r = 0; r < 4; ++r) D[(4 * q + r) * 16 + i] = c[r];
 }
 
+__global__ void mfma_f16_probe_kernel(const uint16_t* __restrict__ A, const uint16_t* __restrict__ B,
+                                      const float* __restrict__ C, float* __restrict__ D) {
+    const int l = threadIdx.x, i = l & 15, q = l >> 4;
+    A += (size_t)blockIdx.x * 512;
+    B += (size_t)blockIdx.x * 512;
+    C += (size_t)blockIdx.x * 256;
+    D += (size_t)blockIdx.x * 256;
+    v8h a, b;
+    for (int j = 0; j < 8; ++j) {
+        a[j] = __builtin_bit_cast(_Float16, A[i * 32 + 8 * q + j]);
+        b[j] = __builtin_bit_cast(_Float16, B[(8 * q + j) * 16 + i]);
+    }
+    v4f32 c;
+    for (int r = 0; r < 4; ++r) c[r] = C[(4 * q + r) * 16 + i];
+    c = __builtin_amdgcn_mfma_f32_16x16x32_f16(a, b, c, 0, 0, 0);
+    for (int r = 0; r < 4; ++r) D[(4 * q + r) * 16 + i] = c[r];
+}
+
 bool filter_enabled() {
     static const bool on = [] {
         const char* e = getenv("MSM_KMEANS_FILTER");
@@ -782,17 +800,26 @@
     return on;
 }
 
-size_t filter_image_bytes(int64_t n, int d) { return (size_t)((n + 63) & ~(int64_t)63) * 16 * filter_rowq(filter_nm(d)); }
+size_t filter_image_bytes(int64_t n, int) { return (size_t)((n + 63) & ~(int64_t)63) * 16 * kFilterRowQ + 16; }
 
 template <typename T>
 msm_status launch_pack(msm_ctx* ctx, const T* x, int64_t n, int d, int64_t ld, const double* mean, const double* stdv,
-                       uint4* image) {
+                       const double* absmax, uint4* image) {
     const unsigned grid = (unsigned)((n + 255) / 256);
+    if (!absmax) {
+        uint4* tail = image + (size_t)((n + 63) & ~(int64_t)63) * kFilterRowQ;
+        MSM_HIP(ctx, hipMemsetAsync(tail, 0, 8, ctx->stream));
+        const int g = (int)std::min<int64_t>((n * d + 256 * 8 - 1) / (256 * 8), (int64_t)ctx->n_cu * 8);
+        hipLaunchKernelGGL(filter_absmax_kernel<T>, dim3(g), dim3(256), 0, ctx->stream, x, n, d, ld, mean, stdv,
+                           (unsigned long long*)tail);
+        MSM_CHECK_LAUNCH(ctx);
+        absmax = (const double*)tail;
+    }
     const int dense = ld == d && ((uintptr_t)x & 15) == 0;
 #define MSM_PACK_CASE(D)                                                                                              \
     case D:                                                                                                           \
-        hipLaunchKernelGGL((kmeans_pack_kernel<T, D>), dim3(grid), dim3(256), 0, ctx->stream, x, n, ld, mean, stdv, image, \
-                           dense);                                                                                    \
+        hipLaunchKernelGGL((kmeans_pack_kernel<T, D>), dim3(grid), dim3(256), 0, ctx->stream, x, n, ld, mean, stdv, absmax, \
+                           image, dense);                                                                             \
         break
     switch (d) {
         MSM_PACK_CASE(1); MSM_PACK_CASE(2); MSM_PACK_CASE(3); MSM_PACK_CASE(4); MSM_PACK_CASE(5);
@@ -815,20 +842,20 @@
     return MSM_OK;
 }
 
-template <typename T, int NM, bool ACCUM>
-msm_status launch_filter_nm(msm_ctx* ctx, const T* x, int64_t n, int d, int64_t ld, const double* centers, int k,
+template <typename T, int DP, bool ACCUM>
+msm_status launch_filter_dp(msm_ctx* ctx, const T* x, int64_t n, int d, int64_t ld, const double* centers, int k,
                             const double* mean, const double* stdv, const uint4* image, int32_t* labels, double* mindist,
                             const FitState* st, unsigned long long* sums, unsigned long long* counts, double* upd_centers) {
     constexpr int NF = 4;
     const size_t lds = filter_lds_bytes(k, d, ACCUM);
     msm_status rs;
     const int64_t n_units = (n + 16 * NF - 1) / (16 * NF);
-    constexpr int kWaves = filter_waves(NM);
+    const int kWaves = filter_waves(DP, ACCUM);
     const int grid = (int)std::min<int64_t>((n_units + kWaves - 1) / kWaves, (int64_t)ctx->n_cu);
     unsigned long long* stats = nullptr;
     rs = filter_stats_buffer(ctx, &stats);
     if (rs != MSM_OK) return rs;
-    auto kern = mean ? kmeans_filter_kernel<T, NM, NF, ACCUM, true> : kmeans_filter_kernel<T, NM, NF, ACCUM, false>;
+    auto kern = mean ? kmeans_filter_kernel<T, DP, NF, ACCUM, true> : kmeans_filter_kernel<T, DP, NF, ACCUM, false>;
     if (lds > 48 * 1024)
         MSM_HIP(ctx, hipFuncSetAttribute((const void*)kern, hipFuncAttributeMaxDynamicSharedMemorySize, (int)lds));
     hipLaunchKernelGGL(kern, dim3(grid), dim3(64 * kWaves), lds, ctx->stream, x, n, d, ld, k, mean, stdv, image, centers,
@@ -842,11 +869,11 @@
 msm_status launch_filter(msm_ctx* ctx, const T* x, int64_t n, int d, int64_t ld, const double* centers, int k,
                          const double* mean, const double* stdv, const uint4* image, int32_t* labels, double* mindist,
                          const FitState* st, unsigned long long* sums, unsigned long long* counts, double* upd_centers) {
-    if (filter_nm(d) == 1)
-        return launch_filter_nm<T, 1, ACCUM>(ctx, x, n, d, ld, centers, k, mean, stdv, image, labels, mindist, st, sums,
+    if (filter_dp(d) == 4)
+        return launch_filter_dp<T, 4, ACCUM>(ctx, x, n, d, ld, centers, k, mean, stdv, image, labels, mindist, st, sums,
                                              counts, upd_centers);
-    return launch_filter_nm<T, 2, ACCUM>(ctx, x, n, d, ld, centers, k, mean, stdv, image, labels, mindist, st, sums, counts,
-                                         upd_centers);
+    return launch_filter_dp<T, 10, ACCUM>(ctx, x, n, d, ld, centers, k, mean, stdv, image, labels, mindist, st, sums, counts,
+                                          upd_centers);
 }
 
 bool filter_fits(int k, int d, bool accum) { return filter_enabled() && d <= kFilterMaxD && filter_lds_bytes(k, d, accum) != 0; }
@@ -861,7 +888,7 @@
         if (!image) {
             msm_status rs = msm_reserve_km_image(ctx, filter_image_bytes(n, d));
             if (rs != MSM_OK) return rs;
-            rs = launch_pack<T>(ctx, x, n, d, ld, mean, stdv, (uint4*)ctx->km_image);
+            rs = launch_pack<T>(ctx, x, n, d, ld, mean, stdv, nullptr, (uint4*)ctx->km_image);
             if (rs != MSM_OK) return rs;
             image = ctx->km_image;
         }
@@ -889,6 +916,31 @@
     return msm_fail(ctx, MSM_ERR_UNSUPPORTED, "k-means: d=%d > 256 not supported", d);
 }
 
+msm_status mfma_probe(msm_ctx* ctx, bool f16, const uint16_t* h_a, const uint16_t* h_b, const float* h_c, float* h_d,
+                      int n_tiles) {
+    if (!ctx) return MSM_ERR_INVALID;
+    MSM_REQUIRE(ctx, n_tiles >= 1 && h_a && h_b && h_c && h_d, "msm_mfma_probe: bad arguments");
+    const size_t na = (size_t)n_tiles * 512 * sizeof(uint16_t), nc = (size_t)n_tiles * 256 * sizeof(float);
+    msm_status rs = msm_reserve_scratch(ctx, 2 * na + 2 * nc);
+    if (rs != MSM_OK) return rs;
+    unsigned char* base = (unsigned char*)ctx->scratch;
+    uint16_t* d_a = (uint16_t*)base;
+    uint16_t* d_b = (uint16_t*)(base + na);
+    float* d_c = (float*)(base + 2 * na);
+    float* d_d = (float*)(base + 2 * na + nc);
+    MSM_HIP(ctx, hipMemcpyAsync(d_a, h_a, na, hipMemcpyHostToDevice, ctx->stream));
+    MSM_HIP(ctx, hipMemcpyAsync(d_b, h_b, na, hipMemcpyHostToDevice, ctx->stream));
+    MSM_HIP(ctx, hipMemcpyAsync(d_c, h_c, nc, hipMemcpyHostToDevice, ctx->stream));
+    if (f16)
+        hipLaunchKernelGGL(mfma_f16_probe_kernel, dim3((unsigned)n_tiles), dim3(64), 0, ctx->stream, d_a, d_b, d_c, d_d);
+    else
+        hipLaunchKernelGGL(mfma_bf16_probe_kernel, dim3((unsigned)n_tiles), dim3(64), 0, ctx->stream, d_a, d_b, d_c, d_d);
+    MSM_CHECK_LAUNCH(ctx);
+    MSM_HIP(ctx, hipMemcpyAsync(h_d, d_d, nc, hipMemcpyDeviceToHost, ctx->stream));
+    MSM_HIP(ctx, hipStreamSynchronize(ctx->stream));
+    return MSM_OK;
+}
+
 }
 
 extern "C" {
@@ -931,6 +983,11 @@
 
 msm_status msm_kmeans_pack(msm_ctx* ctx, const void* d_x, msm_dtype dtype, int64_t n, int d, int64_t ld,
                            const double* d_mean, const double* d_std, void* d_image) {
+    return msm_kmeans_pack_bounded(ctx, d_x, dtype, n, d, ld, d_mean, d_std, nullptr, d_image);
+}
+
+msm_status msm_kmeans_pack_bounded(msm_ctx* ctx, const void* d_x, msm_dtype dtype, int64_t n, int d, int64_t ld,
+                                   const double* d_mean, const double* d_std, const double* d_absmax, void* d_image) {
     if (!ctx) return MSM_ERR_INVALID;
     MSM_REQUIRE(ctx, n >= 0 && d >= 1 && d <= kFilterMaxD && ld >= d, "msm_kmeans_pack: need 1 <= d <= %d, ld >= d",
                 kFilterMaxD);
@@ -939,8 +996,9 @@
     if (n == 0) return MSM_OK;
     MSM_REQUIRE(ctx, d_x && d_image, "msm_kmeans_pack: NULL pointer");
     MSM_REQUIRE(ctx, ((uintptr_t)d_image & 15) == 0, "msm_kmeans_pack: the image must be 16-byte aligned");
-    if (dtype == MSM_F32) return launch_pack<float>(ctx, (const float*)d_x, n, d, ld, d_mean, d_std, (uint4*)d_image);
-    return launch_pack<double>(ctx, (const double*)d_x, n, d, ld, d_mean, d_std, (uint4*)d_image);
+    if (dtype == MSM_F32)
+        return launch_pack<float>(ctx, (const float*)d_x, n, d, ld, d_mean, d_std, d_absmax, (uint4*)d_image);
+    return launch_pack<double>(ctx, (const double*)d_x, n, d, ld, d_mean, d_std, d_absmax, (uint4*)d_image);
 }
 
 msm_status msm_kmeans_filter_scanned(msm_ctx* ctx, uint64_t* h_out, int reset) {
@@ -955,24 +1013,12 @@
 
 msm_status msm_mfma_bf16_probe(msm_ctx* ctx, const uint16_t* h_a, const uint16_t* h_b, const float* h_c, float* h_d,
                                int n_tiles) {
-    if (!ctx) return MSM_ERR_INVALID;
-    MSM_REQUIRE(ctx, n_tiles >= 1 && h_a && h_b && h_c && h_d, "msm_mfma_bf16_probe: bad arguments");
-    const size_t na = (size_t)n_tiles * 512 * sizeof(uint16_t), nc = (size_t)n_tiles * 256 * sizeof(float);
-    msm_status rs = msm_reserve_scratch(ctx, 2 * na + 2 * nc);
-    if (rs != MSM_OK) return rs;
-    unsigned char* base = (unsigned char*)ctx->scratch;
-    uint16_t* d_a = (uint16_t*)base;
-    uint16_t* d_b = (uint16_t*)(base + na);
-    float* d_c = (float*)(base + 2 * na);
-    float* d_d = (float*)(base + 2 * na + nc);
-    MSM_HIP(ctx, hipMemcpyAsync(d_a, h_a, na, hipMemcpyHostToDevice, ctx->stream));
-    MSM_HIP(ctx, hipMemcpyAsync(d_b, h_b, na, hipMemcpyHostToDevice, ctx->stream));
-    MSM_HIP(ctx, hipMemcpyAsync(d_c, h_c, nc, hipMemcpyHostToDevice, ctx->stream));
-    hipLaunchKernelGGL(mfma_bf16_probe_kernel, dim3((unsigned)n_tiles), dim3(64), 0, ctx->stream, d_a, d_b, d_c, d_d);
-    MSM_CHECK_LAUNCH(ctx);
-    MSM_HIP(ctx, hipMemcpyAsync(h_d, d_d, nc, hipMemcpyDeviceToHost, ctx->stream));
-    MSM_HIP(ctx, hipStreamSynchronize(ctx->stream));
-    return MSM_OK;
+    return mfma_probe(ctx, false, h_a, h_b, h_c, h_d, n_tiles);
+}
+
+msm_status msm_mfma_f16_probe(msm_ctx* ctx, const uint16_t* h_a, const uint16_t* h_b, const float* h_c, float* h_d,
+                              int n_tiles) {
+    return mfma_probe(ctx, true, h_a, h_b, h_c, h_d, n_tiles);
 }
 
 msm_status msm_kmeans_fit_begin(msm_ctx* ctx, const void* d_x, msm_dtype dtype, int64_t n, int d, int64_t ld,
diff --git a/pmarlo_amd/csrc/kmeans_filter.h b/pmarlo_amd/csrc/kmeans_filter.h
--- a/pmarlo_amd/csrc/kmeans_filter.h
+++ b/pmarlo_amd/csrc/kmeans_filter.h
@@ -1,61 +1,68 @@
 #pragma once
 
 typedef __bf16 v8bf __attribute__((ext_vector_type(8)));
+typedef _Float16 v8h __attribute__((ext_vector_type(8)));
 typedef float v4f32 __attribute__((ext_vector_type(4)));
 
 #ifdef MSM_KMF_WAVES
-__host__ __device__ constexpr int filter_waves(int) { return MSM_KMF_WAVES; }
+__host__ __device__ constexpr int filter_waves(int, bool) { return MSM_KMF_WAVES; }
 #else
-__host__ __device__ constexpr int filter_waves(int nm) { return nm == 1 ? 16 : 12; }
+__host__ __device__ constexpr int filter_waves(int dp, bool heavy) { return dp == 10 && heavy ? 12 : 16; }
 #endif
 constexpr int kFilterMaxD = 10;
-constexpr double kFilterTiny = 1e-14, kFilterHi = 1e18;
+constexpr int kFilterRowQ = 3;
+constexpr double kFilterHi = 1e18;
+constexpr double kFilterScaledHi = 16384.0;
+constexpr double kF16MinNormal = 6.103515625e-05;
+constexpr int kFilterScaleTop = 13;
+constexpr double kFilterKappa = 52.0 * 5.9604644775390625e-08;
 constexpr float kPickEps = 20.0f * 5.9604644775390625e-08f;
 constexpr float kPickFloor = 1e-30f;
 constexpr float kUp20 = 1.0f + 9.5367431640625e-07f;
-
-__host__ __device__ constexpr int filter_nm(int d) { return 6 * d + 4 <= 32 ? 1 : 2; }
-__host__ __device__ constexpr int filter_rowq(int nm) { return nm == 1 ? 4 : 5; }
-__host__ __device__ constexpr double filter_kappa(int nm) { return (nm == 1 ? 44.0 : 80.0) * 5.9604644775390625e-08; }
-
-__device__ __forceinline__ unsigned bf16_rn(float f) {
-    unsigned u = __float_as_uint(f);
-    u += 0x7FFFu + ((u >> 16) & 1u);
-    return u >> 16;
-}
-__device__ __forceinline__ float bf16_f32(unsigned h) { return __uint_as_float(h << 16); }
-__device__ __forceinline__ unsigned bf16_up(float f) {
-    unsigned h = bf16_rn(f);
-    if (bf16_f32(h) < f) ++h;
-    return h;
-}
-__device__ __forceinline__ void bf16_split3(double v, unsigned (&out)[3]) {
-    float r = (float)v;
-#pragma unroll
-    for (int t = 0; t < 3; ++t) {
-        out[t] = bf16_rn(r);
-        r -= bf16_f32(out[t]);
-    }
-}
-__device__ __forceinline__ int filter_part_c(int t) { return t == 1 || t == 3 ? 1 : (t == 4 ? 2 : 0); }
-__device__ __forceinline__ int filter_part_x(int t) { return t == 2 || t == 3 ? 1 : (t == 5 ? 2 : 0); }
-
-template <int NM>
-__host__ __device__ constexpr int filter_slot(int t, int f, int d) {
-    if (NM == 1) return t * d + f;
-    constexpr int lo8[6] = {0, 8, 24, 32, 16, 40};
-    constexpr int hi2[6] = {48, 50, 54, 56, 52, 58};
-    return f < 8 ? lo8[t] + f : hi2[t] + (f - 8);
-}
-template <int NM>
-__host__ __device__ constexpr int filter_slot_h(int d) { return NM == 1 ? 6 * d : 60; }
-template <int NM>
-__host__ __device__ constexpr int filter_slot_norm() { return 32 * NM - 1; }
-template <int NM>
-__device__ __forceinline__ int filter_piece(int q, int m) {
-    if (NM == 1) return q;
-    return m == 0 ? (q < 3 ? 0 : 1) : q + 1;
-}
+constexpr double kUp20d = 1.0 + 9.5367431640625e-07;
+
+__host__ __device__ inline int filter_scale_exp(double amax) {
+    if (!(amax > 0.0) || !(amax <= 1.7976931348623157e308)) return 0;
+    const int q = ilogb(amax) + 1;
+    const int e = kFilterScaleTop - q;
+    return e < -60 ? -60 : (e > 60 ? 60 : e);
+}
+
+__device__ __forceinline__ double f16_round(double v) {
+    const int q = ilogb(v) + 1;
+    return ldexp(rint(ldexp(v, 11 - q)), q - 11);
+}
+__device__ __forceinline__ double f16_ceil(double v) {
+    const int q = ilogb(v) + 1;
+    return ldexp(ceil(ldexp(v, 11 - q)), q - 11);
+}
+__device__ __forceinline__ unsigned short f16_bits(double v) {
+    return __builtin_bit_cast(unsigned short, (_Float16)(float)v);
+}
+__device__ __forceinline__ void f16_split2(double v, unsigned short& hi, unsigned short& lo, double& tiny) {
+    hi = lo = 0;
+    if (!(fabs(v) >= kF16MinNormal)) {
+        tiny += fabs(v);
+        return;
+    }
+    const double h = f16_round(v);
+    const double r = v - h;
+    hi = f16_bits(h);
+    if (!(fabs(r) >= kF16MinNormal)) {
+        tiny += fabs(r);
+        return;
+    }
+    lo = f16_bits(f16_round(r));
+}
+__device__ __forceinline__ float f32_up(double v) {
+    float f = (float)v;
+    if ((double)f < v) f = __uint_as_float(__float_as_uint(f) + (f >= 0.0f ? 1u : ~0u));
+    return f;
+}
+
+__host__ __device__ constexpr int filter_slot(int t, int f) { return f < 8 ? 8 * t + f : 24 + 2 * t + (f - 8); }
+constexpr int kFilterSlotNorm = 31;
+__device__ __forceinline__ int filter_piece(int q) { return q == 3 ? 2 : (q & 1); }
 
 __device__ __forceinline__ float max3_f32(float a, float b, float c) { return __builtin_fmaxf(__builtin_fmaxf(a, b), c); }
 __device__ __forceinline__ float med3_f32(float a, float b, float c) { return __builtin_amdgcn_fmed3f(a, b, c); }
@@ -68,11 +75,10 @@
 template <typename T, int D>
 __global__ __launch_bounds__(256) void kmeans_pack_kernel(const T* __restrict__ x, int64_t n, int64_t ld,
                                                          const double* __restrict__ mean,
-                                                         const double* __restrict__ stdv, uint4* __restrict__ image,
-                                                         int dense) {
-    constexpr int NM = filter_nm(D);
-    constexpr int RQ = filter_rowq(NM);
-    constexpr int kOutStride = 5;
+                                                         const double* __restrict__ stdv, const double* absmax,
+                                                         uint4* __restrict__ image, int dense) {
+    constexpr int RQ = kFilterRowQ;
+    constexpr int kOutStride = RQ;
     constexpr int kInBytes = 256 * D * (int)sizeof(T);
     constexpr int kOutBytes = 256 * kOutStride * 16;
     __shared__ __attribute__((aligned(16))) unsigned char stage[kOutBytes > kInBytes ? kOutBytes : kInBytes];
@@ -81,6 +87,8 @@
     const int rows = (int)(n - t0 < 256 ? n - t0 : 256);
     const int64_t n_pad = (n + 63) & ~(int64_t)63;
     const int rows_out = (int)(n_pad - t0 < 256 ? n_pad - t0 : 256);
+    const int ex = filter_scale_exp(*absmax);
+    if (blockIdx.x == 0 && threadIdx.x == 0) reinterpret_cast<int*>(image + n_pad * RQ)[2] = ex;
     double v[D];
     if (dense) {
         const unsigned char* src = reinterpret_cast<const unsigned char*>(x + t0 * D);
@@ -101,69 +109,57 @@
 #pragma unroll
         for (int f = 0; f < D; ++f) v[f] = load_as_f64(row + f);
     }
-    unsigned part[D][3];
-    double q = 0.0, tiny = 0.0;
     bool ok = t < n;
 #pragma unroll
     for (int f = 0; f < D; ++f) {
         if (mean) v[f] = (v[f] - mean[f]) / stdv[f];
         ok = ok && fabs(v[f]) <= kFilterHi;
-    }
+        v[f] = ldexp(v[f], ex);
+        ok = ok && fabs(v[f]) <= kFilterScaledHi;
+    }
+    unsigned short hi[D], lo[D];
+    double q = 0.0, tiny = 0.0;
 #pragma unroll
     for (int f = 0; f < D; ++f) {
-        const double a = fabs(v[f]);
-        const bool keep = ok && a >= kFilterTiny;
-        if (ok && !keep) tiny += a;
-        const double w = keep ? v[f] : 0.0;
-        q = fma(w, w, q);
-        bf16_split3(w, part[f]);
-    }
-    const unsigned xn = ok ? bf16_up((float)((sqrt(q) + tiny / filter_kappa(NM)) * (1.0 + 9.5367431640625e-07))) : 0x7F80u;
-    unsigned slots[8 * RQ];
-#pragma unroll
-    for (int s = 0; s < 8 * RQ; ++s) slots[s] = 0;
-    if constexpr (NM == 1) {
-#pragma unroll
-        for (int tt = 0; tt < 6; ++tt)
-#pragma unroll
-            for (int f = 0; f < D; ++f) slots[tt * D + f] = part[f][tt == 2 || tt == 3 ? 1 : (tt == 5 ? 2 : 0)];
-        slots[6 * D] = slots[6 * D + 1] = slots[6 * D + 2] = 0x3F80u;
-        slots[31] = xn;
-    } else {
-#pragma unroll
-        for (int f = 0; f < D; ++f) {
-            if (f < 8) {
-                slots[f] = part[f][0];
-                slots[8 + f] = part[f][1];
-                slots[16 + f] = part[f][2];
-            } else {
-                const int g = f - 8;
-                slots[24 + g] = slots[26 + g] = slots[28 + g] = part[f][0];
-                slots[30 + g] = part[f][1];
-                slots[32 + g] = part[f][1];
-                slots[34 + g] = part[f][2];
-            }
-        }
-        slots[36] = slots[37] = slots[38] = 0x3F80u;
-        slots[39] = xn;
-    }
+        hi[f] = lo[f] = 0;
+        if (ok) {
+            q = fma(v[f], v[f], q);
+            f16_split2(v[f], hi[f], lo[f], tiny);
+        }
+    }
+    const unsigned short xn =
+        ok ? f16_bits(f16_ceil(fmax((sqrt(q) + 2.0 * tiny / kFilterKappa) * kUp20d, kF16MinNormal))) : 0x7C00;
+    unsigned short s[8 * RQ];
+#pragma unroll
+    for (int i = 0; i < 8 * RQ; ++i) s[i] = 0;
+#pragma unroll
+    for (int f = 0; f < D; ++f) {
+        if (f < 8) {
+            s[f] = hi[f];
+            s[8 + f] = lo[f];
+        } else {
+            s[16 + f - 8] = s[20 + f - 8] = hi[f];
+            s[18 + f - 8] = lo[f];
+        }
+    }
+    s[23] = xn;
     uint4* mine = reinterpret_cast<uint4*>(stage) + threadIdx.x * kOutStride;
 #pragma unroll
     for (int c = 0; c < RQ; ++c)
-        mine[c] = make_uint4(slots[8 * c + 0] | (slots[8 * c + 1] << 16), slots[8 * c + 2] | (slots[8 * c + 3] << 16),
-                             slots[8 * c + 4] | (slots[8 * c + 5] << 16), slots[8 * c + 6] | (slots[8 * c + 7] << 16));
+        mine[c] = make_uint4(s[8 * c + 0] | ((unsigned)s[8 * c + 1] << 16), s[8 * c + 2] | ((unsigned)s[8 * c + 3] << 16),
+                             s[8 * c + 4] | ((unsigned)s[8 * c + 5] << 16), s[8 * c + 6] | ((unsigned)s[8 * c + 7] << 16));
     __syncthreads();
     uint4* dst = image + t0 * RQ;
     for (int c = threadIdx.x; c < rows_out * RQ; c += 256)
         dst[c] = reinterpret_cast<const uint4*>(stage)[(c / RQ) * kOutStride + (c % RQ)];
 }
 
-template <int NM>
+template <int DP>
 struct FilterShape {
-    static constexpr int DP = NM == 1 ? 4 : 10;
-    static constexpr int RF = NM == 1 ? 8 : 12;
-    static constexpr int kTileBytes = NM * 1024 + 16 * RF * 4 + 16 * 8;
+    static constexpr int RF = DP == 4 ? 8 : 12;
+    static constexpr int kTileBytes = 1024 + 16 * RF * 4 + 16 * 4 + 16 * 8;
 };
+__host__ __device__ constexpr int filter_dp(int d) { return d <= 4 ? 4 : 10; }
 
 constexpr int kStageRegs = (16 * kFilterMaxD + 63) / 64;
 __device__ __forceinline__ int stage_row(int i, int d) { return (int)(((float)i + 0.5f) * (1.0f / (float)d)); }
@@ -180,30 +176,30 @@
 #pragma unroll
     for (int f = 0; f < DP; ++f) rc[f] = (lane < 16 && jr < k && f < d) ? centers[(size_t)jr * d + f] : 0.0;
 }
-template <int NM>
+template <int DP>
 __device__ __forceinline__ void filter_stage_build(int tile, int lane, unsigned short* simg, const double (&c)[kStageRegs],
-                                                   const double (&rc)[FilterShape<NM>::DP], int k, int d,
-                                                   float* __restrict__ tab, double* __restrict__ hs, int* __restrict__ any_bad) {
-    using S = FilterShape<NM>;
-    constexpr double kappa = filter_kappa(NM);
-    for (int i = lane; i < NM * 64 * 4; i += 64) reinterpret_cast<unsigned*>(simg)[i] = 0u;
+                                                   const double (&rc)[DP], int k, int d, int ec, int exc,
+                                                   float* __restrict__ tab, float* __restrict__ cz, double* __restrict__ hs,
+                                                   int* __restrict__ any_bad) {
+    using S = FilterShape<DP>;
+    for (int i = lane; i < 64 * 4; i += 64) reinterpret_cast<unsigned*>(simg)[i] = 0u;
     for (int i = lane; i < 16 * S::RF; i += 64) tab[(size_t)tile * 16 * S::RF + i] = 0.0f;
     __builtin_amdgcn_fence(__ATOMIC_ACQ_REL, "wavefront");
-    auto slot_addr = [&](int i, int sl) {
-        const int m = sl >> 5, qq = (sl & 31) >> 3, e = sl & 7;
-        return ((m * 64) + qq * 16 + i) * 8 + e;
-    };
+    auto slot_addr = [&](int i, int sl) { return ((sl >> 3) * 16 + i) * 8 + (sl & 7); };
 #pragma unroll
     for (int u = 0; u < kStageRegs; ++u) {
         const int i = lane + 64 * u;
         const int r = stage_row(i, d), f = i - r * d, j = tile * 16 + r;
         if (i < 16 * d && j < k) {
             tab[(size_t)j * S::RF + f] = (float)c[u];
-            if (fabs(c[u]) >= kFilterTiny) {
-                unsigned cp[3];
-                bf16_split3(c[u], cp);
-#pragma unroll
-                for (int t = 0; t < 6; ++t) simg[slot_addr(r, filter_slot<NM>(t, f, d))] = (unsigned short)cp[filter_part_c(t)];
+            const double w = ldexp(c[u], ec);
+            if (fabs(w) <= kFilterScaledHi) {
+                unsigned short ch, cl;
+                double tiny = 0.0;
+                f16_split2(w, ch, cl, tiny);
+                simg[slot_addr(r, filter_slot(0, f))] = ch;
+                simg[slot_addr(r, filter_slot(1, f))] = ch;
+                simg[slot_addr(r, filter_slot(2, f))] = cl;
             }
         }
     }
@@ -214,33 +210,34 @@
         float* row = tab + (size_t)j * S::RF;
         double h = __builtin_inf();
         if (j < k) {
-            double a = 0.0, akeep = 0.0, tiny = 0.0;
+            double a = 0.0, aw = 0.0, tiny = 0.0;
             bool ok = true;
 #pragma unroll
-            for (int f = 0; f < S::DP; ++f) {
+            for (int f = 0; f < DP; ++f) {
                 const double cf = rc[f];
                 a = fma(cf, cf, a);
-                const double ac = fabs(cf);
-                ok = ok && ac <= kFilterHi;
-                if (ac >= kFilterTiny) akeep = fma(cf, cf, akeep);
-                else tiny += ac;
+                const double w = ldexp(cf, ec);
+                ok = ok && fabs(cf) <= kFilterHi && fabs(w) <= kFilterScaledHi;
+                if (ok) {
+                    aw = fma(w, w, aw);
+                    const double r = fabs(w) >= kF16MinNormal ? fabs(w - f16_round(w)) : fabs(w);
+                    if (!(r >= kF16MinNormal) || !(fabs(w) >= kF16MinNormal)) tiny += r;
+                }
             }
             h = 0.5 * a;
+            const double cval = ldexp(-(h - kFilterKappa * h), exc);
+            ok = ok && fabs(cval) <= 0x1p100;
             if (!ok) bad_row = 1;
-            unsigned hsp[3];
-            bf16_split3(-(h - kappa * h), hsp);
-            const int sh = filter_slot_h<NM>(d);
-            simg[slot_addr(lane, sh)] = (unsigned short)hsp[0];
-            simg[slot_addr(lane, sh + 1)] = (unsigned short)hsp[1];
-            simg[slot_addr(lane, sh + 2)] = (unsigned short)hsp[2];
-            simg[slot_addr(lane, filter_slot_norm<NM>())] =
-                (unsigned short)bf16_up((float)((kappa * sqrt(akeep) + tiny) * (1.0 + 9.5367431640625e-07)));
-            row[S::DP] = (float)h;
-            row[S::DP + 1] = (float)(sqrt(a) * (1.0 + 9.5367431640625e-07));
+            cz[j] = ok ? f32_up(cval) : 0.0f;
+            if (ok)
+                simg[slot_addr(lane, kFilterSlotNorm)] =
+                    f16_bits(f16_ceil(fmax((kFilterKappa * sqrt(aw) + 2.0 * tiny) * kUp20d, kF16MinNormal)));
+            row[DP] = (float)h;
+            row[DP + 1] = (float)(sqrt(a) * kUp20d);
         } else {
-            simg[slot_addr(lane, filter_slot_h<NM>(d))] = 0xFF7F;
-            row[S::DP] = 3.0e38f;
-            row[S::DP + 1] = -3.0e38f;
+            cz[j] = -3.0e38f;
+            row[DP] = 3.0e38f;
+            row[DP + 1] = -3.0e38f;
         }
         hs[j] = h;
     }
@@ -314,6 +311,28 @@
     return x;
 }
 
+template <typename T>
+__global__ __launch_bounds__(256) void filter_absmax_kernel(const T* __restrict__ x, int64_t n, int d, int64_t ld,
+                                                           const double* __restrict__ mean, const double* __restrict__ stdv,
+                                                           unsigned long long* __restrict__ out_bits) {
+    double m = 0.0;
+    for (int64_t i = (int64_t)blockIdx.x * 256 + threadIdx.x; i < n * d; i += (int64_t)gridDim.x * 256) {
+        const int64_t r = i / d;
+        const int f = (int)(i - r * d);
+        double v = load_as_f64(x + r * ld + f);
+        if (mean) v = (v - mean[f]) / stdv[f];
+        if (fabs(v) <= kFilterHi) m = fmax(m, fabs(v));
+    }
+    m = wave_max_f64(m);
+    __shared__ double wm[4];
+    if ((threadIdx.x & 63) == 0) wm[threadIdx.x >> 6] = m;
+    __syncthreads();
+    if (threadIdx.x == 0) {
+        m = fmax(fmax(wm[0], wm[1]), fmax(wm[2], wm[3]));
+        if (m > 0.0) atomicMax(out_bits, (unsigned long long)__double_as_longlong(m));
+    }
+}
+
 template <typename T, int DP, bool WHITEN>
 __device__ __forceinline__ void filter_load_frame(const T* __restrict__ x, int64_t ld, int d, bool vec_rows,
                                                   const double* __restrict__ mean, const double* __restrict__ stdv,
@@ -391,17 +410,17 @@
     }
 }
 
-template <typename T, int NM, int NF, bool ACCUM, bool WHITEN>
-__global__ __launch_bounds__(64 * filter_waves(NM)) void kmeans_filter_kernel(
+template <typename T, int DP, int NF, bool ACCUM, bool WHITEN>
+__global__ __launch_bounds__(64 * filter_waves(DP, ACCUM)) void kmeans_filter_kernel(
     const T* __restrict__ x, int64_t n, int d, int64_t ld, int k, const double* __restrict__ mean,
     const double* __restrict__ stdv, const uint4* __restrict__ image, const double* __restrict__ centers,
     int32_t* __restrict__ labels,
     double* __restrict__ mindist, const FitState* __restrict__ st, unsigned long long* __restrict__ sums,
     unsigned long long* __restrict__ counts, unsigned long long* __restrict__ n_scanned, double* upd_centers,
     unsigned int* __restrict__ ticket) {
-    using S = FilterShape<NM>;
-    constexpr int kFilterWaves = filter_waves(NM);
-    constexpr int kMT = 64 * kFilterWaves, DP = S::DP, RF = S::RF, RQ = filter_rowq(NM);
+    using S = FilterShape<DP>;
+    constexpr int kFilterWaves = filter_waves(DP, ACCUM);
+    constexpr int kMT = 64 * kFilterWaves, RF = S::RF, RQ = kFilterRowQ;
     static_assert(NF == 4, "one frame group per lane quarter: a unit is 64 frames, one per lane in the candidate pick");
     extern __shared__ __attribute__((aligned(16))) unsigned char smem_raw[];
     if constexpr (ACCUM) {
@@ -410,18 +429,21 @@
     const int k16 = (k + 15) & ~15;
     const int n_tiles = ((k16 / 16) + 1) & ~1;
     uint4* img = reinterpret_cast<uint4*>(smem_raw);
-    float* tab = reinterpret_cast<float*>(img + (size_t)n_tiles * NM * 64);
-    double* hs = reinterpret_cast<double*>(tab + (size_t)n_tiles * 16 * RF);
+    float* tab = reinterpret_cast<float*>(img + (size_t)n_tiles * 64);
+    float* cz = tab + (size_t)n_tiles * 16 * RF;
+    double* hs = reinterpret_cast<double*>(cz + (size_t)n_tiles * 16);
     unsigned long long* lsum = reinterpret_cast<unsigned long long*>(hs + (size_t)n_tiles * 16);
     unsigned long long* lcnt = lsum + (ACCUM ? (size_t)k * d : 0);
     __shared__ int unit_ctr;
     __shared__ int any_bad;
+    __shared__ unsigned long long cmax_bits;
     const int tid = threadIdx.x, lane = tid & 63, wave = __builtin_amdgcn_readfirstlane(tid >> 6);
     const int j16 = lane & 15, q = lane >> 4;
     const double scale = ACCUM ? st->scale : 0.0;
     if (tid == 0) {
         unit_ctr = kFilterWaves;
         any_bad = 0;
+        cmax_bits = 0ull;
     }
     KSTAMP_INIT
     if constexpr (ACCUM) {
@@ -433,34 +455,41 @@
     const int64_t units_per_block = (n_units + gridDim.x - 1) / gridDim.x;
     const int64_t u_begin = (int64_t)blockIdx.x * units_per_block;
     const int64_t u_end = min(n_units, u_begin + units_per_block);
-    int voff[NM];
-#pragma unroll
-    for (int m = 0; m < NM; ++m) voff[m] = j16 * RQ + filter_piece<NM>(q, m);
+    const int voff = j16 * RQ + filter_piece(q);
+    const int ex = reinterpret_cast<const int*>(image + (size_t)((n + 63) & ~(int64_t)63) * RQ)[2];
 
     int64_t unit = u_begin + wave;
-    v8bf b[NF][NM];
+    v8h b[NF];
     auto load_images = [&](int64_t un) {
         const uint4* ub = image + un * (kUnit * RQ);
 #pragma unroll
-        for (int u = 0; u < NF; ++u)
-#pragma unroll
-            for (int m = 0; m < NM; ++m) b[u][m] = __builtin_bit_cast(v8bf, ub[voff[m] + u * 16 * RQ]);
+        for (int u = 0; u < NF; ++u) b[u] = __builtin_bit_cast(v8h, ub[voff + u * 16 * RQ]);
     };
     if (unit < u_end) load_images(unit);
 
+    {
+        double cm = 0.0;
+        for (int i = tid; i < k * d; i += kMT) cm = fmax(cm, fabs(centers[i]));
+        cm = wave_max_f64(cm);
+        if (lane == 0 && cm > 0.0) atomicMax(&cmax_bits, (unsigned long long)__double_as_longlong(cm));
+    }
+    __syncthreads();
+    const int ec = __builtin_amdgcn_readfirstlane(filter_scale_exp(__longlong_as_double((long long)cmax_bits)));
+    const int exc = ex + ec;
     for (int t = wave; t < n_tiles; t += 2 * kFilterWaves) {
         const int t2 = t + kFilterWaves;
         double c0[kStageRegs], c1[kStageRegs], r0[DP], r1[DP];
         filter_stage_fetch<DP>(t, lane, centers, k, d, c0, r0);
         if (t2 < n_tiles) filter_stage_fetch<DP>(t2, lane, centers, k, d, c1, r1);
-        filter_stage_build<NM>(t, lane, reinterpret_cast<unsigned short*>(img + (size_t)t * NM * 64), c0, r0, k, d, tab, hs,
-                               &any_bad);
+        filter_stage_build<DP>(t, lane, reinterpret_cast<unsigned short*>(img + (size_t)t * 64), c0, r0, k, d, ec, exc, tab, cz,
+                               hs, &any_bad);
         if (t2 < n_tiles)
-            filter_stage_build<NM>(t2, lane, reinterpret_cast<unsigned short*>(img + (size_t)t2 * NM * 64), c1, r1, k, d, tab, hs,
-                                   &any_bad);
+            filter_stage_build<DP>(t2, lane, reinterpret_cast<unsigned short*>(img + (size_t)t2 * 64), c1, r1, k, d, ec, exc, tab,
+                                   cz, hs, &any_bad);
     }
     __syncthreads();
-    const bool all_scan = any_bad != 0;
+    const float inv_scale_u = __int_as_float((127 - exc) << 23);
+    const bool all_scan = __builtin_amdgcn_readfirstlane(any_bad) != 0;
     KSTAMP(0);
 
     unsigned long long my_scans = 0;
@@ -550,24 +579,15 @@
         for (int it = 0; it < iters; ++it) {
 #endif
             const int jt = 2 * it;
-            v8bf aa[NM], ab[NM];
-#pragma unroll
-            for (int m = 0; m < NM; ++m) {
-                aa[m] = __builtin_bit_cast(v8bf, img[((jt + 0) * NM + m) * 64 + lane]);
-                ab[m] = __builtin_bit_cast(v8bf, img[((jt + 1) * NM + m) * 64 + lane]);
-            }
+            const v8h aa = __builtin_bit_cast(v8h, img[(jt + 0) * 64 + lane]);
+            const v8h ab = __builtin_bit_cast(v8h, img[(jt + 1) * 64 + lane]);
+            const v4f32 ca = *reinterpret_cast<const v4f32*>(cz + (jt + 0) * 16 + 4 * q);
+            const v4f32 cb = *reinterpret_cast<const v4f32*>(cz + (jt + 1) * 16 + 4 * q);
             v4f32 acca[NF], accb[NF];
 #pragma unroll
             for (int u = 0; u < NF; ++u) {
-                acca[u] = __builtin_amdgcn_mfma_f32_16x16x32_bf16(aa[0], b[u][0], (v4f32){0.f, 0.f, 0.f, 0.f}, 0, 0, 0);
-                accb[u] = __builtin_amdgcn_mfma_f32_16x16x32_bf16(ab[0], b[u][0], (v4f32){0.f, 0.f, 0.f, 0.f}, 0, 0, 0);
-            }
-            if constexpr (NM == 2) {
-#pragma unroll
-                for (int u = 0; u < NF; ++u) {
-                    acca[u] = __builtin_amdgcn_mfma_f32_16x16x32_bf16(aa[1], b[u][1], acca[u], 0, 0, 0);
-                    accb[u] = __builtin_amdgcn_mfma_f32_16x16x32_bf16(ab[1], b[u][1], accb[u], 0, 0, 0);
-                }
+                acca[u] = __builtin_amdgcn_mfma_f32_16x16x32_f16(aa, b[u], ca, 0, 0, 0);
+                accb[u] = __builtin_amdgcn_mfma_f32_16x16x32_f16(ab, b[u], cb, 0, 0, 0);
             }
 #pragma unroll
             for (int u = 0; u < NF; ++u) {
@@ -584,7 +604,7 @@
         KSTAMP(2);
         bool guard[NF];
 #pragma unroll
-        for (int u = 0; u < NF; ++u) guard[u] = q == 3 && __builtin_bit_cast(unsigned short, b[u][NM - 1][7]) == 0x7F80;
+        for (int u = 0; u < NF; ++u) guard[u] = q == 3 && __builtin_bit_cast(unsigned short, b[u][7]) == 0x7C00;
         if (nxt < u_end) load_images(nxt);
         const int64_t f0 = unit * kUnit + lane;
         const bool fok = f0 < n;
@@ -613,6 +633,7 @@
             Ru = q == u ? R_u : Ru;
         }
 #endif
+        Ru = __builtin_fmaf(Ru, inv_scale_u, 1.40129846e-45f);
         KSTAMP(3);
         const int gs = cd >> 16, pstar = cd & 0xffff;
         const int base = min(pstar * 16 + 4 * gs, n_tiles * 16 - 20);
@@ -633,7 +654,7 @@
         for (int c = 0; c < 8; ++c) {
             const float4* r4 = reinterpret_cast<const float4*>(p_row + ((c & 3) + 16 * (c >> 2)) * RF);
             float a = 0.f, h, cn;
-            if constexpr (NM == 1) {
+            if constexpr (DP == 4) {
                 const float4 r0 = r4[0], r1 = r4[1];
                 a = __builtin_fmaf(r0.x, pz[0], a);
                 a = __builtin_fmaf(r0.y, pz[1], a);
@@ -718,7 +739,7 @@
             for (int c = lane; c < n_tiles * 16; c += 64) {
                 const float4* r4 = reinterpret_cast<const float4*>(tab + (size_t)c * RF);
                 float a = 0.f, h, cn;
-                if constexpr (NM == 1) {
+                if constexpr (DP == 4) {
                     const float4 r0 = r4[0], r1 = r4[1];
                     a = __builtin_fmaf(r0.x, zf[0], a);
                     a = __builtin_fmaf(r0.y, zf[1], a);
@@ -834,10 +855,9 @@
 
 static inline size_t filter_lds_bytes(int k, int d, bool accum) {
     if (d > kFilterMaxD) return 0;
-    const int nm = filter_nm(d);
     const int k16 = (k + 15) & ~15;
     const int n_tiles = ((k16 / 16) + 1) & ~1;
-    const size_t tile_bytes = nm == 1 ? FilterShape<1>::kTileBytes : FilterShape<2>::kTileBytes;
+    const size_t tile_bytes = filter_dp(d) == 4 ? FilterShape<4>::kTileBytes : FilterShape<10>::kTileBytes;
     const size_t total = (size_t)n_tiles * tile_bytes + (accum ? (size_t)k * (d + 1) * sizeof(unsigned long long) : 0);
     const size_t cap = 160 * 1024 - 64;
     return total <= cap ? total : 0;
diff --git a/pmarlo_amd/device.py b/pmarlo_amd/device.py
--- a/pmarlo_amd/device.py
+++ b/pmarlo_amd/device.py
@@ -609,7 +609,7 @@
         return int(out.value)
 
     def kmeans_pack(self, x: DeviceArray, *, mean: DeviceArray | None = None, std: DeviceArray | None = None,
-                    image: DeviceArray | None = None) -> DeviceArray | None:
+                    image: DeviceArray | None = None, absmax: DeviceArray | None = None) -> DeviceArray | None:
         n, d = x.shape
         nbytes = self.kmeans_image_bytes(n, d)
         if nbytes == 0:
@@ -617,9 +617,9 @@
         image = image if image is not None else self.empty((nbytes,), np.uint8)
         if image.nbytes < nbytes:
             raise ValueError(f"image buffer holds {image.nbytes} bytes, {nbytes} needed")
-        check(lib.msm_kmeans_pack(self.handle, x.ptr, _dtype_code(x.dtype), n, d, d,
-                                  mean.ptr if mean is not None else None, std.ptr if std is not None else None,
-                                  image.ptr), self.handle)
+        check(lib.msm_kmeans_pack_bounded(self.handle, x.ptr, _dtype_code(x.dtype), n, d, d,
+                                          mean.ptr if mean is not None else None, std.ptr if std is not None else None,
+                                          absmax.ptr if absmax is not None else None, image.ptr), self.handle)
         return image
 
     def kmeans_filter_scanned(self, reset: bool = False) -> int:
@@ -628,15 +628,20 @@
         return int(out.value)
 
     def mfma_bf16_probe(self, a_bits: np.ndarray, b_bits: np.ndarray, c: np.ndarray) -> np.ndarray:
+        return self._mfma_probe(lib.msm_mfma_bf16_probe, a_bits, b_bits, c)
+
+    def mfma_f16_probe(self, a_bits: np.ndarray, b_bits: np.ndarray, c: np.ndarray) -> np.ndarray:
+        return self._mfma_probe(lib.msm_mfma_f16_probe, a_bits, b_bits, c)
+
+    def _mfma_probe(self, fn, a_bits: np.ndarray, b_bits: np.ndarray, c: np.ndarray) -> np.ndarray:
         a = np.ascontiguousarray(a_bits, np.uint16)
         b = np.ascontiguousarray(b_bits, np.uint16)
         cc = np.ascontiguousarray(c, np.float32)
         t = a.shape[0]
         if a.shape != (t, 16, 32) or b.shape != (t, 32, 16) or cc.shape != (t, 16, 16):
-            raise ValueError("mfma_bf16_probe: shapes must be [t,16,32], [t,32,16], [t,16,16]")
+            raise ValueError("mfma probe: shapes must be [t,16,32], [t,32,16], [t,16,16]")
         out = np.empty((t, 16, 16), np.float32)
-        check(lib.msm_mfma_bf16_probe(self.handle, a.ctypes.data, b.ctypes.data, cc.ctypes.data, out.ctypes.data, t),
-              self.handle)
+        check(fn(self.handle, a.ctypes.data, b.ctypes.data, cc.ctypes.data, out.ctypes.data, t), self.handle)
         return out
 
     def kmeans_lloyd_pass(self, x: DeviceArray, centers: DeviceArray, state: DeviceArray, sums: DeviceArray,
diff --git a/pmarlo_amd/dist.py b/pmarlo_amd/dist.py
--- a/pmarlo_amd/dist.py
+++ b/pmarlo_amd/dist.py
@@ -378,7 +378,7 @@
         acc_sums, acc_counts = acc.view((k * d,), np.int64), acc.view((k,), np.int64, offset_elems=k * d)
         self.labels.fill_bytes_(0xFF)
         if self.km_image is not None:
-            eng.kmeans_pack(self.Y, image=self.km_image)
+            eng.kmeans_pack(self.Y, image=self.km_image, absmax=b["fit_state"].view((1,), offset_elems=2))
         for _ in range(cfg.kmeans_iters):
             if self.time_accum:
                 e0, e1 = eng.event(), eng.event()
```

Measured after the change: 702.0 million frames/s (median of 6 runs). 1.06x the previous value.
